# cbs228/sameold

Hardware: AMD Instinct MI355X
Metric: Msamples/s demodulated (batched 22.05 kHz channels) + % HBM roofline, 1/8 GPU (higher is better)
Workload: dtype f32

## Files before the change

sameold_amd/csrc/same_batch.cpp:

```cpp
#include <hip/hip_runtime.h>

#include <algorithm>
#include <chrono>
#include <cstdio>
#include <cstdlib>
#include <cstring>
#include <deque>
#include <new>
#include <string>
#include <type_traits>
#include <utility>
#include <vector>

#include "../../include/same_rx.h"
#include "same_config.h"
#include "same_device.h"
#include "same_harvest.h"
#include "same_hipmem.h"
#include "same_launch.h"
#include "same_resets.h"
#include "same_tp_plan.h"
#include "same_transport.h"

using same::fail;
static_assert(sizeof(same::cap::Span) == same::kSpanBytes, "same_tp_plan.h sizes the span list");

namespace {

#define HIP_TRY(expr)                                                                     \
    do {                                                                                   \
        hipError_t _e = (expr);                                                            \
        if (_e != hipSuccess)                                                              \
            return fail(SAME_EHIP, "%s failed: %s (%s:%d)", #expr, hipGetErrorString(_e),  \
                        __FILE__, __LINE__);                                               \
    } while (0)

}

struct same_batch {
    same_rx_builder builder{};
    same::Params P{};
    same::State S{};
    int device = 0;
    uint32_t flags = 0;
    uint64_t counter = 0;
    hipStream_t own_stream = nullptr;
    hipStream_t last_stream = nullptr;
    same::DevBuf<float4> d_taps;
    same::DevBuf<void> d_state_blob;
    struct Slot {
        same::DevBuf<same::DevEvent> d_events;
        uint32_t event_cap() const { return (uint32_t)d_events.size(); }
        same::DevBuf<uint32_t> d_sort;
        same::PinnedBuf<uint32_t> h_sort;
        same::DevBuf<same::DevEvent> d_sorted;
        uint32_t sort_bins = 0;
        same::DevBuf<uint8_t> d_bursts;
        uint32_t burst_cap() const { return (uint32_t)(d_bursts.size() / same::kBurstCap); }
        same::DevBuf<uint32_t> d_counters;
        same::MappedBuf<uint32_t> h_counters;
        same::Event ev_start, ev_stop, ev_done, ev_planned;
        same::Event ev_k0, ev_k1;
        bool have_k = false;
        bool timed = false;
        same::PinnedBuf<void> h_events, h_bursts;
        bool in_flight = false;
        uint64_t seq = 0;
        uint64_t end_counter = 0;
        bool chunked = false;
        same::ChunkGeom geom{};
        uint32_t columns(uint32_t n_channels) const { return chunked ? geom.n_chunks * n_channels : n_channels; }
        uint64_t end_blocks = 0;
        same::DevBuf<uint64_t> d_handover;
        same::PinnedBuf<uint64_t> h_handover;
        bool per_channel = false;
        same::TpGeomWords words;
        same::DevBuf<uint32_t> d_geom;
        same::PinnedBuf<uint32_t> h_geom;
        same::TpPlan plan{};
        uint64_t plan_counter0 = 0;
        bool plan_sorted = false, plan_lpt = false, plan_pairs = false;
        same::CoherentBuf<uint32_t> h_reset;
        same::CoherentBuf<uint32_t> h_counts;
        same::PinnedBuf<uint64_t> h_wake_up;
        bool dev_transport = false;
        same::CoherentBuf<same::DevMessage> h_near;
        uint32_t near_cap() const { return (uint32_t)h_near.size(); }
        same::DevBuf<same::DevMessage> d_msgs;
        uint32_t msg_cap() const { return (uint32_t)d_msgs.size(); }
        same::PinnedBuf<void> h_msgs;
        bool captured = false;
        same::DevBuf<same::cap::Span> d_spans;
        uint32_t span_cap() const { return (uint32_t)d_spans.size(); }
        same::DevBuf<float> d_pool;
        same::DevBuf<same::cap::Cursors> d_cap_cur;
        same::MappedBuf<same::cap::Cursors> h_cap_cur;
        same::PinnedBuf<void> h_spans, h_pool;
    } slot[2];
    struct TimePar {
        bool enabled = false;
        same::TpConfig cfg;
        uint32_t cap_columns = 0;
        uint32_t carved_columns = 0;
        int carved_family = -1;
        same::Params Pv{};
        same::State Sv{};
        same::DevBuf<void> blob;
        same::DevBuf<void> blob_fresh;
        size_t fresh_bytes = 0;
        same::DevBuf<same::StateArrayDesc> d_desc_in, d_desc_out;
        uint32_t n_desc = 0;
        same::DevBuf<uint32_t> d_final_col;
        same::DevBuf<float> d_energy;
        same::DevBuf<float> d_hist;
        same::Event ev_plan_prev; bool plan_recorded = false;
        uint32_t last_chunks = 1;
        bool last_per_channel = false;
        same::Family family = same::Family::kPipe;
    } tp;
    uint64_t launch_seq = 0;
    hipStream_t copy_stream = nullptr;
    struct Windowed {
        bool on = false;
        uint32_t window = 0;
        uint32_t fill = 0;
        same::DevBuf<void> d_buf;
        same::Event ev_buf;
        hipStream_t buf_stream = nullptr; bool buf_used = false;
        same::Event ev_read[2];
        uint64_t n_reads = 0;
        hipStream_t read_stream = nullptr;
    } inv;
    hipStream_t plan_stream = nullptr;
    float last_ms = 0.0f;
    bool overflowed = false;
    std::string record_path;
    bool kernel_fault = false;
    same::Request want;
    same::Mode mode;
    same::Choice plain;
    same::Params Pfm{};
    same::Family last_family = same::Family::kGeneric;
    bool sym_launched = false;
    bool debug = false;
    same::DevBuf<void> d_stage, d_stage2;
    same::DevBuf<void> d_upload;
    same::DevBuf<void> d_zero;
    same::Event ev_order;
    bool timing = false;
    bool have_timing = false;
    float last_demod_ms = 0.0f;
    same::PinnedBuf<uint64_t> h_wake;
    bool wake_ordered = false;
    std::vector<uint32_t> ragged_by;
    bool messages_only = false;
    bool dev_transport = false;
    bool last_dev_transport = false;
    same::DevBuf<void> d_thot, d_tcold;
    same::ResetLedger resets;
    std::vector<uint32_t> reset_list, reset_now, reset_cols;
    same::EventLog events;
    same::Replay replay{resets, events};
    struct Audio {
        size_t per_launch = 0;
        same::DevBuf<same::cap::Rec> d_rec;
        uint64_t flush_at = UINT64_MAX;
        same::AudioLog log;
    } audio;
};

namespace {

struct Carver {
    size_t off = 0;
    template <typename T> size_t take(size_t n)
    {
        off = (off + 255) & ~size_t(255);
        size_t o = off;
        off += n * sizeof(T);
        return o;
    }
};

#define SAME_STATE_ARRAYS(X, P)                                                                            \
    X(dc_ff_ring, float, (P).dc_len) X(dc_fb_ring, float, (P).dc_len)                                        \
    X(dc_sum0, float, 1) X(dc_sum1, float, 1) X(agc_gain, float, 1)                                          \
    X(win_ring, float, (P).win_ring)                                                                         \
    X(ted_clock, uint32_t, 1) X(until_next_ted, float, 1)                                                    \
    X(ted_h0, float, 1) X(ted_h1, float, 1) X(ted_h2, float, 1)                                              \
    X(period_avg, float, 1) X(period_inst, float, 1)                                                         \
    X(sq_data, uint32_t, 1) X(sq_power, float, 1) X(sq_phist, uint32_t, 1)                                   \
    X(sq_fill, uint32_t, 1) X(sq_clock, int32_t, 1) X(sq_symbols, uint64_t, 1)                               \
    X(sq_hist, float, same::kSquelchHist)                                                                    \
    X(eq_ffc, float, (P).eq_nff) X(eq_fbc, float, (P).eq_nfb)                                                \
    X(eq_ffw, float, (P).eq_nff) X(eq_fbw, float, (P).eq_nfb)                                                \
    X(eq_word, uint32_t, 1) X(eq_count, uint32_t, 1)                                                         \
    X(eq_snap_ffc, float, (P).eq_nff) X(eq_snap_fbc, float, (P).eq_nfb)                                      \
    X(eq_snap_ffw, float, (P).eq_nff) X(eq_snap_fbw, float, (P).eq_nfb)                                      \
    X(fr_word, uint32_t, 1) X(fr_count, uint32_t, 1) X(fr_invalid, uint32_t, 1) X(fr_len, uint32_t, 1)       \
    X(flags, uint32_t, 1)                                                                                    \
    X(tk_next, uint64_t, 1) X(tk_last, uint64_t, 1) X(tk_ring, uint64_t, same::kTickRing)                    \
    X(tk_n, uint32_t, 1) X(wake_sample, uint64_t, 1) X(wake_fired, uint64_t, 1)

size_t carve_state(const same::Params &P, char *base, same::State &S)
{
    const size_t C = P.n_channels;
    Carver cv;
#define CARVE(field, type, count) \
    do { size_t o = cv.take<type>(count); if (base) S.field = reinterpret_cast<type *>(base + o); } while (0)
#define CARVE_ROWS(field, type, rows) CARVE(field, type, (size_t)(rows) * C);
    SAME_STATE_ARRAYS(CARVE_ROWS, P)
#undef CARVE_ROWS
    CARVE(fr_msg, uint8_t, (size_t)same::kBurstCap * C);
    if (P.trace_cap) {
        CARVE(trace_n, uint32_t, C);
        CARVE(trace, float, (size_t)P.trace_cap * 4 * C);
        CARVE(trace_idx, uint64_t, (size_t)P.trace_cap * C);
    }
#undef CARVE
    return (cv.off + 255) & ~size_t(255);
}

void list_state_arrays(const same::Params &P, const same::State &src, const same::State &dst,
                       std::vector<same::StateArrayDesc> &out)
{
    out.clear();
#define DESC_ROWS(field, type, rows)                                                                     \
    out.push_back(same::StateArrayDesc{reinterpret_cast<char *>(src.field), reinterpret_cast<char *>(dst.field), \
                                       (uint32_t)(rows), (uint32_t)(sizeof(type) / 4)});
    SAME_STATE_ARRAYS(DESC_ROWS, P)
#undef DESC_ROWS
    static_assert(same::kBurstCap % 4 == 0, "framer rows are copied in words");
    out.push_back(same::StateArrayDesc{reinterpret_cast<char *>(src.fr_msg), reinterpret_cast<char *>(dst.fr_msg), 1u,
                                       (uint32_t)(same::kBurstCap / 4)});
}

void read_knobs(same_batch *rx)
{
    auto num = [](const char *name, int unset) { const char *e = std::getenv(name); return e ? std::atoi(e) : unset; };
    auto tri = [](const char *name) { const char *e = std::getenv(name); return e ? (std::atoi(e) ? 1 : -1) : 0; };
    rx->P.knob_pipe = tri("SAME_PIPE");
    rx->P.knob_pipe_lanes = num("SAME_PIPE_LANES", 0);
    rx->P.knob_pipe_split = tri("SAME_PIPE_SPLIT");
#ifdef SAME_PROFILE
    rx->P.knob_mirror = tri("SAME_MIRROR");
    rx->P.knob_pipe_share = tri("SAME_PIPE_SHARE");
    rx->P.knob_prio = num("SAME_PIPE_PRIO", 0);
#endif
    rx->P.knob_fast_dense = tri("SAME_FAST_DENSE");
    rx->P.knob_sym = tri("SAME_SYM");
    rx->want.sym_max_channels = (uint32_t)std::max(0, num("SAME_SYM_MAX", 1 << 30));
    rx->debug = rx->replay.debug = std::getenv("SAME_DEBUG") != nullptr;
    { const char *e = std::getenv("SAME_RECORD_HARVEST"); rx->record_path = e ? e : ""; }
    rx->replay.host_threads = std::max(0, num("SAME_HOST_THREADS", 0));
    rx->tp.cfg.sort_mode = num("SAME_TP_SORT", -1);
    rx->tp.cfg.knob_plan_stream = tri("SAME_TP_PLAN_STREAM");
    rx->tp.cfg.knob_prologue = tri("SAME_TP_PROLOGUE");
    rx->want.knob_relaxed = tri("SAME_RELAXED");
    { const char *e = std::getenv("SAME_RELAXED_KERNEL"); rx->P.knob_relaxed_kernel = !e ? 0 : (std::strcmp(e, "solo") == 0 ? 1 : (std::strcmp(e, "duo") == 0 ? 2 : 0)); }
    { const char *e = std::getenv("SAME_TP_KERNEL"); rx->want.knob_tp_kernel = !e ? 0 : (std::strcmp(e, "wave") == 0 ? 2 : (std::strcmp(e, "pipe") == 0 ? 1 : 0)); }
}

int ensure_output(same_batch *rx, same_batch::Slot &sl, size_t n_samples, same::Output &O, size_t n_columns = 0)
{
    const same::OutputCaps caps = same::output_caps(rx->P, n_samples, n_columns, rx->dev_transport, rx->audio.per_launch != 0, sl.near_cap(), sl.msg_cap());
    HIP_TRY(sl.d_events.ensure(caps.events));
    HIP_TRY(sl.d_bursts.ensure(caps.bursts * same::kBurstCap));
    if (caps.messages) HIP_TRY(sl.d_msgs.ensure(caps.messages));
    if (caps.near) HIP_TRY(sl.h_near.ensure(caps.near));
    if (caps.spans) HIP_TRY(sl.d_spans.ensure(caps.spans));
    HIP_TRY(sl.d_sorted.ensure(sl.d_events.size()));
    HIP_TRY(sl.d_sort.ensure(caps.sort_words));
    HIP_TRY(sl.h_sort.ensure(caps.bins + 1));
    sl.sort_bins = (uint32_t)caps.bins;
    O.events = sl.d_events; O.event_cap = sl.event_cap();
    O.bursts = sl.d_bursts; O.burst_cap = sl.burst_cap();
    O.n_events = sl.d_counters; O.n_bursts = sl.d_counters + 1; O.overflow = sl.d_counters + 2;
    return SAME_OK;
}

template <typename SampleT>
hipError_t launch_family(same::Family f, const same::Params &P, const same::State &S, const same::Output &O, const float4 *taps, const SampleT *x,
                         uint32_t n_blocks, uint64_t counter0, hipStream_t stream, const same::PipeChunks &pc = same::PipeChunks{})
{
    switch (f) {
    case same::Family::kSym: return same::launch_demod_sym(P, S, O, taps, x, n_blocks, counter0, stream, pc);
    case same::Family::kPipeFastmath: return same::launch_demod_pipe(P, S, O, taps, x, n_blocks, counter0, stream, pc, true);
    case same::Family::kPipe: return same::launch_demod_pipe(P, S, O, taps, x, n_blocks, counter0, stream, pc, false);
    case same::Family::kWaveRelaxed: return same::launch_demod_relaxed(P, S, O, taps, x, n_blocks, counter0, stream, pc);
    case same::Family::kFast: return same::launch_demod_fast(P, S, O, taps, x, n_blocks, counter0, stream);
    case same::Family::kGeneric: break;
    }
    return hipErrorInvalidValue;
}

void reset_channel_host(same_batch *rx, uint32_t c, uint64_t pos)
{
    rx->replay.reset_channel(c, pos);
    if (rx->h_wake) rx->h_wake[c] = 0;
}

int launch_pending_resets(same_batch *rx, same_batch::Slot &sl, hipStream_t stream)
{
    if (rx->resets.device.empty()) return SAME_OK;
    std::vector<uint32_t> &cols = rx->reset_cols;
    rx->resets.take_device(cols);
    const uint32_t n = (uint32_t)cols.size();
    if (n > sl.h_reset.size()) HIP_TRY(sl.h_reset.ensure(std::max<uint32_t>(256u, n + n / 2u)));
    std::memcpy(sl.h_reset, cols.data(), (size_t)n * sizeof(uint32_t));
    hipError_t e = same::launch_reset_columns(rx->P, rx->S, sl.h_reset.dev(), n, stream);
    if (e == hipSuccess && rx->dev_transport)
        e = same::launch_transport_reset(rx->d_thot, rx->d_tcold, rx->P.n_channels, sl.h_reset.dev(), n, 0, stream, rx->audio.d_rec);
    if (e != hipSuccess) return fail(SAME_EHIP, "channel reset launch failed: %s", hipGetErrorString(e));
    return SAME_OK;
}

int record_harvest(same_batch *rx, same_batch::Slot &sl, const same::HarvestInput &in, uint32_t n_events, uint32_t n_bursts, const char *path)
{
    if (sl.seq != 3u) return SAME_OK;
    const uint32_t n_ch = rx->P.n_channels, n_bins = sl.columns(n_ch);
    same::HarvestFileHeader h{};
    h.n_channels = n_ch; h.n_bins = n_bins; h.n_events = n_events; h.n_bursts = n_bursts;
    h.chunked = sl.chunked; h.per_channel = sl.per_channel; h.flags = rx->flags; h.input_rate = rx->P.input_rate; h.tp_enabled = rx->tp.enabled;
    h.geom = sl.geom; h.end_blocks = sl.end_blocks; h.end_counter = sl.end_counter;
    return same::write_harvest_file(path, h, in);
}

hipError_t grow_pinned(same::PinnedBuf<void> &b, size_t need)
{
    return need <= b.size() ? hipSuccess : b.ensure(need + need / 2 + 4096);
}

int harvest_audio(same_batch *rx, same_batch::Slot &sl)
{
    sl.captured = false;
    same_batch::Audio &A = rx->audio;
    const same::cap::Cursors cur = *sl.h_cap_cur.get();
    if (cur.overflow) rx->overflowed = true;
    const uint32_t n_spans = std::min(cur.n_spans, sl.span_cap());
    if (!n_spans) return SAME_OK;
    const size_t used = (size_t)std::min<unsigned long long>(cur.pool_used, (unsigned long long)A.per_launch);
    HIP_TRY(grow_pinned(sl.h_spans, (size_t)n_spans * sizeof(same::cap::Span)));
    HIP_TRY(hipMemcpyAsync(sl.h_spans, sl.d_spans, (size_t)n_spans * sizeof(same::cap::Span), hipMemcpyDeviceToHost, rx->copy_stream));
    if (used) {
        HIP_TRY(grow_pinned(sl.h_pool, used * sizeof(float)));
        HIP_TRY(hipMemcpyAsync(sl.h_pool, sl.d_pool, used * sizeof(float), hipMemcpyDeviceToHost, rx->copy_stream));
    }
    HIP_TRY(hipStreamSynchronize(rx->copy_stream));
    const same::cap::Span *sp = static_cast<const same::cap::Span *>(sl.h_spans.get());
    const float *pool = static_cast<const float *>(sl.h_pool.get());
    size_t n_samples = 0;
    if (const int arc = A.log.append_spans(sp, n_spans, pool, used, rx->resets, &n_samples)) return arc;
    if (rx->debug)
        std::fprintf(stderr, "[same] audio: %u chunks, %zu samples (pool %zu of %zu)%s\n", n_spans, n_samples, used, A.per_launch,
                     cur.overflow ? ", truncated" : "");
    return SAME_OK;
}

int harvest_messages(same_batch *rx, same_batch::Slot &sl, std::chrono::steady_clock::time_point t_begin,
                     std::chrono::steady_clock::time_point t_waited)
{
    const uint32_t n_msgs = std::min(sl.h_counters[3], sl.near_cap() + sl.msg_cap());
    const uint32_t n_near = std::min(n_msgs, sl.near_cap()), n_far = n_msgs - n_near;
    const size_t far_bytes = (size_t)n_far * sizeof(same::DevMessage);
    if (n_far) {
        HIP_TRY(grow_pinned(sl.h_msgs, far_bytes));
        HIP_TRY(hipMemcpyAsync(sl.h_msgs, sl.d_msgs, far_bytes, hipMemcpyDeviceToHost, rx->copy_stream));
        HIP_TRY(hipStreamSynchronize(rx->copy_stream));
    }
    auto t_copied = std::chrono::steady_clock::now();
    const same::DevMessage *far = static_cast<const same::DevMessage *>(sl.h_msgs.get());
    if (const int mrc = rx->replay.append_messages(sl.h_near.get(), n_near, far, n_far)) return mrc;
    if (sl.captured) {
        const int arc = harvest_audio(rx, sl);
        if (arc) return arc;
    }
    const int si = (int)(&sl - rx->slot);
    rx->resets.shift_due(si);
    rx->resets.done_shift(si);
    if (const int arc = rx->audio.log.end_reset(rx->resets.slot[si & 1].channels, rx->resets.rec_pos(si), rx->resets)) return arc;
    for (uint32_t c : rx->resets.host_due(si)) reset_channel_host(rx, c, rx->resets.rec_pos(si));
    rx->resets.done_host(si);
    if (rx->debug) {
        auto t_end = std::chrono::steady_clock::now();
        auto ms = [](auto a, auto b) { return std::chrono::duration<double, std::milli>(b - a).count(); };
        std::fprintf(stderr, "[same] harvest timing: wait %.2f ms, copy %.2f ms, %u messages queued in %.2f ms (transport layer on the device)\n",
                     ms(t_begin, t_waited), ms(t_waited, t_copied), n_msgs, ms(t_copied, t_end));
    }
    return SAME_OK;
}

int upload_wake_ordered(same_batch *rx, same_batch::Slot &sl)
{
    const uint32_t C = rx->P.n_channels;
    HIP_TRY(sl.h_wake_up.ensure(C));
    same_batch::Slot &other = rx->slot[(&sl - rx->slot) ^ 1];
    const int oi = (int)(&other - rx->slot);
    for (uint32_t c = 0; c < C; ++c) {
        const uint64_t w = rx->h_wake[c];
        sl.h_wake_up[c] = w && other.in_flight ? w + rx->resets.pending_shift(oi, c) : w;
    }
    if (other.in_flight) {
        HIP_TRY(hipMemcpyAsync(rx->S.wake_sample, sl.h_wake_up, (size_t)C * sizeof(uint64_t), hipMemcpyHostToDevice, rx->last_stream));
        HIP_TRY(hipEventRecord(other.ev_done, rx->last_stream));
    } else {
        HIP_TRY(hipMemcpyAsync(rx->S.wake_sample, sl.h_wake_up, (size_t)C * sizeof(uint64_t), hipMemcpyHostToDevice, rx->copy_stream));
        HIP_TRY(hipStreamSynchronize(rx->copy_stream));
    }
    return SAME_OK;
}

int harvest_slot(same_batch *rx, same_batch::Slot &sl)
{
    if (!sl.in_flight) return SAME_OK;
    const bool dbg = rx->debug;
    auto t_begin = std::chrono::steady_clock::now();
    HIP_TRY(hipEventSynchronize(sl.ev_done));
    sl.in_flight = false;
    if (sl.timed) {
        HIP_TRY(hipEventElapsedTime(&rx->last_ms, sl.ev_start, sl.ev_stop));
        rx->last_demod_ms = rx->last_ms;
        if (sl.have_k) HIP_TRY(hipEventElapsedTime(&rx->last_demod_ms, sl.ev_k0, sl.ev_k1));
        rx->have_timing = true;
    }
    auto t_waited = std::chrono::steady_clock::now();
    const uint32_t n_events = std::min(sl.h_counters[0], sl.event_cap());
    if (dbg)
        std::fprintf(stderr, "[same] harvest: %u device events (%u bursts), cap %u/%u\n", sl.h_counters[0],
                     sl.h_counters[1], sl.event_cap(), sl.burst_cap());
    const uint32_t n_bursts = std::min(sl.h_counters[1], sl.burst_cap());
    if (sl.h_counters[2] & (3u | same::kMessageLogOverflow)) rx->overflowed = true;
    if (sl.h_counters[2] & 4u) rx->kernel_fault = true;
    if (sl.dev_transport) return harvest_messages(rx, sl, t_begin, t_waited);
    const size_t ev_bytes = (size_t)n_events * sizeof(same::DevEvent), bu_bytes = (size_t)n_bursts * same::kBurstCap;
    HIP_TRY(grow_pinned(sl.h_events, ev_bytes));
    HIP_TRY(grow_pinned(sl.h_bursts, bu_bytes));
    const uint32_t n_bins = sl.columns(rx->P.n_channels);
    if (n_bins != sl.sort_bins) return fail(SAME_EINVAL, "internal: event sort made for %u columns, launch has %u", sl.sort_bins, n_bins);
    HIP_TRY(hipMemcpyAsync(sl.h_sort, sl.d_sort + n_bins, ((size_t)n_bins + 1) * sizeof(uint32_t), hipMemcpyDeviceToHost, rx->copy_stream));
    if (n_events) HIP_TRY(hipMemcpyAsync(sl.h_events, sl.d_sorted, ev_bytes, hipMemcpyDeviceToHost, rx->copy_stream));
    HIP_TRY(hipStreamSynchronize(rx->copy_stream));
    if (n_bursts) HIP_TRY(hipMemcpyAsync(sl.h_bursts, sl.d_bursts, bu_bytes, hipMemcpyDeviceToHost, rx->copy_stream));
    if (sl.chunked) {
        HIP_TRY(hipMemcpyAsync(sl.h_handover, sl.d_handover, (size_t)n_bins * sizeof(uint64_t), hipMemcpyDeviceToHost, rx->copy_stream));
        if (sl.per_channel)
            HIP_TRY(hipMemcpyAsync(sl.h_geom, sl.d_geom + sl.words.own_start, sl.words.harvest * sizeof(uint32_t), hipMemcpyDeviceToHost, rx->copy_stream));
    }
    if (n_bursts || sl.chunked) HIP_TRY(hipStreamSynchronize(rx->copy_stream));
    auto t_copied = std::chrono::steady_clock::now();
    const same::HarvestInput in{sl.h_sort, static_cast<same::DevEvent *>(sl.h_events.get()), static_cast<const uint8_t *>(sl.h_bursts.get()),
                                sl.h_handover, sl.h_geom};
    if (!rx->record_path.empty()) { const int rrc = record_harvest(rx, sl, in, n_events, n_bursts, rx->record_path.c_str()); if (rrc != SAME_OK) return rrc; }
    std::vector<uint32_t> rearm;
    same::HarvestTimes times;
    same::HarvestLaunch launch;
    launch.chunked = sl.chunked; launch.per_channel = sl.per_channel; launch.geom = sl.geom;
    launch.end_blocks = sl.end_blocks; launch.end_counter = sl.end_counter;
    int rc = rx->replay.replay(launch, in, n_events, n_bursts, rearm, times);
    if (rc) return rc;
    {
        const int si = (int)(&sl - rx->slot);
        const same::ResetLedger::SlotShift &sh = rx->resets.shift_due(si);
        if (!rx->replay.thot.empty())
            for (size_t i = 0; i < sh.channels.size(); ++i)
                if (rx->replay.tr(sh.channels[i]).shift_force_eom(sh.by[i])) rearm.push_back(sh.channels[i]);
        rx->resets.done_shift(si);
    }
    {
        const int si = (int)(&sl - rx->slot);
        const std::vector<uint32_t> &due = rx->resets.host_due(si);
        for (uint32_t c : due) reset_channel_host(rx, c, rx->resets.rec_pos(si));
        rx->resets.done_host(si);
    }
    if (!rearm.empty()) {
        if (!rx->h_wake) {
            HIP_TRY(rx->h_wake.ensure(rx->P.n_channels));
            std::memset(rx->h_wake, 0, (size_t)rx->P.n_channels * sizeof(uint64_t));
        }
        for (uint32_t c : rearm) rx->h_wake[c] = rx->replay.tr(c).force_eom_at();
        if (rx->wake_ordered) {
            int rc2 = upload_wake_ordered(rx, sl);
            if (rc2) return rc2;
        } else {
        HIP_TRY(hipMemcpyAsync(rx->S.wake_sample, rx->h_wake, (size_t)rx->P.n_channels * sizeof(uint64_t), hipMemcpyHostToDevice, rx->copy_stream));
        HIP_TRY(hipStreamSynchronize(rx->copy_stream));
        }
    }
    if (dbg) {
        auto t_end = std::chrono::steady_clock::now();
        auto ms = [](auto a, auto b) { return std::chrono::duration<double, std::milli>(b - a).count(); };
        std::fprintf(stderr, "[same] harvest timing: wait %.2f ms, copy %.2f ms, sort %.2f ms, replay on %u threads %.2f ms, "
                             "queue %.2f ms\n",
                     ms(t_begin, t_waited), ms(t_waited, t_copied), ms(t_copied, times.sorted), times.n_threads,
                     ms(times.sorted, times.replayed), ms(times.replayed, t_end));
    }
    return SAME_OK;
}

int harvest(same_batch *rx)
{
    same_batch::Slot *order[2] = {&rx->slot[0], &rx->slot[1]};
    if (order[0]->seq > order[1]->seq) std::swap(order[0], order[1]);
    for (same_batch::Slot *sl : order) {
        int rc = harvest_slot(rx, *sl);
        if (rc) return rc;
    }
    return SAME_OK;
}

int ensure_wide_state(same_batch *rx, uint32_t columns)
{
    same_batch::TimePar &tp = rx->tp;
    if (tp.carved_columns == columns && tp.carved_family == (int)tp.family) return SAME_OK;
    int rc = harvest(rx);
    if (rc) return rc;
    HIP_TRY(hipDeviceSynchronize());
    tp.Pv = same::wide_params(rx->P, columns, same::is_fastmath(tp.family), same::tp_more_than_one_round(columns));
    if (columns > tp.cap_columns) {
        tp.cap_columns = 0;
        HIP_TRY(tp.blob.reset());
        HIP_TRY(tp.blob_fresh.reset());
        const size_t bytes = carve_state(tp.Pv, nullptr, tp.Sv);
        HIP_TRY(tp.blob.ensure(bytes));
        HIP_TRY(hipMemset(tp.blob, 0, bytes));
        HIP_TRY(tp.blob_fresh.ensure(bytes));
        tp.cap_columns = columns;
    }
    const size_t blob_bytes = carve_state(tp.Pv, (char *)tp.blob.get(), tp.Sv);
    {
        same::State Sf{};
        carve_state(tp.Pv, (char *)tp.blob_fresh.get(), Sf);
        HIP_TRY(hipMemset(tp.blob_fresh, 0, blob_bytes));
        HIP_TRY(same::launch_init_state(tp.Pv, Sf, 0, nullptr, 0));
        HIP_TRY(hipDeviceSynchronize());
        tp.fresh_bytes = (size_t)(reinterpret_cast<char *>(tp.Sv.fr_msg) - static_cast<char *>(tp.blob.get()));
    }
    std::vector<same::StateArrayDesc> in, out;
    list_state_arrays(rx->P, rx->S, tp.Sv, in);
    list_state_arrays(rx->P, tp.Sv, rx->S, out);
    tp.n_desc = (uint32_t)in.size();
    HIP_TRY(tp.d_desc_in.ensure(in.size()));
    HIP_TRY(tp.d_desc_out.ensure(out.size()));
    HIP_TRY(tp.d_final_col.ensure(rx->P.n_channels));
    HIP_TRY(hipMemcpy(tp.d_desc_in, in.data(), in.size() * sizeof(same::StateArrayDesc), hipMemcpyHostToDevice));
    HIP_TRY(hipMemcpy(tp.d_desc_out, out.data(), out.size() * sizeof(same::StateArrayDesc), hipMemcpyHostToDevice));
    tp.carved_columns = columns;
    tp.carved_family = (int)tp.family;
    return SAME_OK;
}

struct Ragged {
    const uint32_t *counts = nullptr;
    uint32_t m = 0;
    uint32_t row_off = 0;
};

struct RaggedLaunch {
    uint32_t row0 = 0;
    size_t n_lock = 0;
};


int begin_launch(same_batch *rx, same_batch::Slot &sl, const same_batch::Slot &prev, hipStream_t stream)
{
    int rc = harvest_slot(rx, sl);
    if (rc) return rc;
    if (prev.in_flight && rx->last_stream != stream) HIP_TRY(hipStreamWaitEvent(stream, prev.ev_done, 0));
    return launch_pending_resets(rx, sl, stream);
}

int begin_timing(same_batch *rx, same_batch::Slot &sl, hipStream_t stream)
{
    sl.timed = rx->timing;
    if (sl.timed) HIP_TRY(hipEventRecord(sl.ev_start, stream));
    return SAME_OK;
}

int tp_start(same_batch *rx, same_batch::Slot &sl, uint32_t columns, const char *layout, hipStream_t stream, bool *sort_bins_empty)
{
    same_batch::TimePar &tp = rx->tp;
    const uint32_t C = rx->P.n_channels;
    *sort_bins_empty = false;
    if (tp.cfg.knob_prologue >= 0) {
        HIP_TRY(same::launch_tp_prologue(tp.blob, tp.blob_fresh, tp.fresh_bytes, sl.d_handover, sl.d_sort, columns, sl.d_counters, stream));
        *sort_bins_empty = sl.sort_bins == columns;
    } else {
        HIP_TRY(same::launch_counters(sl.d_counters, sl.h_counters.dev(), 0, stream));
        HIP_TRY(same::launch_init_state(tp.Pv, tp.Sv, 0, stream, C));
        HIP_TRY(same::launch_fill_u64(sl.d_handover, columns, same::kNoHandover, stream));
    }
    if (rx->debug) std::fprintf(stderr, "[same] time-parallel launch: %u columns (%s), start-up: %s\n", columns, layout,
                                tp.cfg.knob_prologue >= 0 ? "prologue kernel" : "separate launches");
    HIP_TRY(same::launch_copy_state_columns(tp.d_desc_in, tp.n_desc, C, columns, nullptr, C, stream));
    return SAME_OK;
}

template <typename SampleT>
int demod_tail(same_batch *rx, const same::Output &O, const SampleT *rows, size_t n, uint64_t counter0, hipStream_t stream)
{
    const hipError_t e = same::launch_demod(rx->P, rx->S, O, rx->d_taps, rows, (uint32_t)n, counter0, stream);
    if (e != hipSuccess) return fail(SAME_EHIP, "demod kernel launch failed: %s", hipGetErrorString(e));
    return SAME_OK;
}
int demod_tail_corner(same_batch *rx, const same::Output &O, const float *corner, size_t pitch, size_t r, uint64_t counter0, hipStream_t stream)
{
    const uint32_t C = rx->P.n_channels;
    HIP_TRY(rx->d_stage.ensure(r * C * sizeof(float)));
    HIP_TRY(rx->d_stage2.ensure(r * C * sizeof(float)));
    float *staged = static_cast<float *>(rx->d_stage.get()), *rows = static_cast<float *>(rx->d_stage2.get());
    HIP_TRY(hipMemcpy2DAsync(staged, r * sizeof(float), corner, pitch * sizeof(float), r * sizeof(float), C, hipMemcpyDeviceToDevice, stream));
    const hipError_t e = same::launch_transpose(staged, rows, C, (uint32_t)r, stream);
    if (e != hipSuccess) return fail(SAME_EHIP, "demod kernel launch failed: %s", hipGetErrorString(e));
    return demod_tail(rx, O, rows, r, counter0, stream);
}

int tp_plan_boundaries(same_batch *rx, same_batch::Slot &sl, const same::TpCut &cut, const same::TpNative &np, const float *d_x,
                       hipStream_t stream, same::PipeChunks &pc)
{
    same_batch::TimePar &tp = rx->tp;
    const same::TpGeomWords &w = np.words;
    same::TpPlan plan{};
    plan.channels = rx->P.n_channels; plan.n_chunks = cut.n_chunks; plan.block_len = cut.geom.block_len;
    plan.warmup_samples = np.warmup_samples; plan.whole_samples = np.whole_samples; plan.in_samples = np.in_samples;
    plan.scout_blocks = np.scout_blocks;
    sl.plan = plan; sl.plan_counter0 = rx->counter;
    sl.plan_sorted = np.sort_mode != 0; sl.plan_lpt = np.lpt; sl.plan_pairs = np.pair_groups;
    uint32_t *g = sl.d_geom;
    const bool side = same::tp_plan_beside(tp.cfg, stream == rx->own_stream);
    hipStream_t ps = side ? rx->plan_stream : stream;
    if (tp.plan_recorded) HIP_TRY(hipStreamWaitEvent(ps, tp.ev_plan_prev, 0));
    HIP_TRY(same::launch_tp_plan(d_x, plan, tp.d_energy, g + w.own_start, g + w.row0, g + w.nominal, g + w.perm, g + w.wg, np.sort_mode != 0, ps,
                                 np.lpt ? g + w.perm2 : nullptr, np.lpt ? g + w.wg2 : nullptr, np.pair_groups));
    HIP_TRY(tp.ev_plan_prev.ensure());
    HIP_TRY(hipEventRecord(tp.ev_plan_prev, ps));
    tp.plan_recorded = true;
    if (side) {
        HIP_TRY(hipEventRecord(sl.ev_planned, ps));
        HIP_TRY(hipStreamWaitEvent(stream, sl.ev_planned, 0));
    }
    pc.col_row0 = g + w.row0; pc.col_nominal = g + w.nominal;
    pc.wg_blocks = g + (np.lpt ? w.wg2 : w.wg); pc.col_perm = np.lpt ? g + w.perm2 : nullptr;
    pc.in_samples = np.in_samples; pc.whole_samples = np.whole_samples;
    pc.hist_scratch = np.need_hist ? tp.d_hist.get() : nullptr;
    return SAME_OK;
}

template <typename SampleT>
int launch_time_parallel(same_batch *rx, same_batch::Slot &sl, hipStream_t stream, const same::TpCut &cut, const same::TpNative *np,
                         const SampleT *x, size_t n_call, bool *sort_bins_empty)
{
    same_batch::TimePar &tp = rx->tp;
    const same::ChunkGeom &geom = cut.geom;
    const uint32_t C = rx->P.n_channels, columns = cut.n_chunks * C, fb = geom.block_len;
    const uint32_t total_blocks = (uint32_t)(n_call / fb);
    const size_t n_whole = (size_t)total_blocks * fb;
    tp.family = cut.choice.family;
    same::Output O{};
    int rc = ensure_wide_state(rx, columns);
    if (rc == SAME_OK) rc = ensure_output(rx, sl, same::tp_output_samples(np ? n_whole : n_call, cut.pc, fb), O, columns);
    if (rc) return rc;
    HIP_TRY(sl.d_handover.ensure(columns));
    HIP_TRY(sl.h_handover.ensure(columns));
    same::PipeChunks pc = cut.pc;
    pc.handover = sl.d_handover;
    if (np) {
        HIP_TRY(sl.d_geom.ensure(np->words.total));
        HIP_TRY(sl.h_geom.ensure(np->words.harvest));
        HIP_TRY(tp.d_energy.ensure(np->energy_floats));
        if (np->need_hist) HIP_TRY(tp.d_hist.ensure(np->hist_floats));
        sl.words = np->words;
    }
    rc = begin_timing(rx, sl, stream);
    if (rc) return rc;
    const float *xf = nullptr;
    if constexpr (std::is_same_v<SampleT, float>) xf = x;
    if (np && (rc = tp_plan_boundaries(rx, sl, cut, *np, xf, stream, pc)) != SAME_OK) return rc;
    rc = tp_start(rx, sl, columns, np ? "channel-major" : "time-major", stream, sort_bins_empty);
    if (rc) return rc;
    sl.have_k = np && sl.timed;
    if (sl.have_k) HIP_TRY(hipEventRecord(sl.ev_k0, stream));
    const hipError_t e = launch_family(tp.family, tp.Pv, tp.Sv, O, rx->d_taps, x, total_blocks, rx->counter, stream, pc);
    rx->last_family = tp.family;
    if (e != hipSuccess) return fail(SAME_EHIP, "time-parallel demod kernel launch failed: %s", hipGetErrorString(e));
    if (sl.have_k) HIP_TRY(hipEventRecord(sl.ev_k1, stream));
    if (np) HIP_TRY(same::launch_chunk_final_column_pc(sl.d_handover, sl.d_geom + np->words.own_start, C, geom.n_chunks, rx->counter, tp.d_final_col, stream));
    else HIP_TRY(same::launch_chunk_final_column(sl.d_handover, C, geom, tp.d_final_col, stream));
    HIP_TRY(same::launch_copy_state_columns(tp.d_desc_out, tp.n_desc, columns, C, tp.d_final_col, C, stream));
    if (n_whole < n_call) {
        rc = np ? demod_tail_corner(rx, O, xf + n_whole, n_call, n_call - n_whole, rx->counter + n_whole, stream)
                : demod_tail(rx, O, x + n_whole * C, n_call - n_whole, rx->counter + n_whole, stream);
        if (rc) return rc;
    }
    sl.chunked = true; sl.per_channel = np != nullptr;
    sl.geom = geom;
    sl.end_blocks = rx->counter + n_whole;
    tp.last_chunks = cut.n_chunks; tp.last_per_channel = sl.per_channel;
    return SAME_OK;
}

template <typename SampleT>
int end_launch(same_batch *rx, same_batch::Slot &sl, same_batch::Slot &prev, hipStream_t stream, const SampleT *rows, size_t n,
               bool sort_bins_empty, const RaggedLaunch *rl = nullptr)
{
    if (sl.timed) HIP_TRY(hipEventRecord(sl.ev_stop, stream));
    HIP_TRY(same::launch_event_sort(sl.d_events, sl.d_counters, sl.event_cap(), sl.sort_bins, sl.d_sort, sl.d_sort + sl.sort_bins,
                                    sl.d_sorted, stream, sort_bins_empty));
    sl.dev_transport = rx->dev_transport && !sl.chunked;
    rx->last_dev_transport = sl.dev_transport;
    if (sl.dev_transport) {
        same::TransportLaunch T{};
        T.n_channels = rx->P.n_channels; T.input_rate = rx->P.input_rate;
        T.first = sl.d_sort + sl.sort_bins; T.sorted = sl.d_sorted; T.counters = sl.d_counters;
        T.bursts = sl.d_bursts; T.burst_cap = sl.burst_cap();
        T.hot = rx->d_thot; T.cold = rx->d_tcold; T.wake_sample = rx->S.wake_sample;
        T.near = sl.h_near.dev(); T.near_cap = sl.near_cap();
        T.log = sl.d_msgs; T.log_cap = sl.msg_cap(); T.log_cursor = sl.d_counters + 3; T.overflow = sl.d_counters + 2;
        sl.captured = rx->audio.per_launch != 0;
        if (sl.captured) {
            same::cap::Launch &K = T.cap;
            const uint64_t fa = rx->audio.flush_at;
            K.start = rx->counter; K.n_rows = (uint32_t)n;
            K.flush_row = fa >= rx->counter + n ? same::cap::kNoFlush : (uint32_t)(fa > rx->counter ? fa - rx->counter : 0);
            K.rec = rx->audio.d_rec; K.spans = sl.d_spans; K.span_cap = sl.span_cap();
            K.n_spans = &sl.d_cap_cur->n_spans; K.pool_used = &sl.d_cap_cur->pool_used; K.pool_cap = rx->audio.per_launch;
            K.overflow = &sl.d_cap_cur->overflow;
        }
        if (rl && rl->n_lock < n)
            HIP_TRY(same::launch_transport_ragged(T, sl.h_counts.dev(), rl->row0, (uint32_t)n, stream));
        else
            HIP_TRY(same::launch_transport(T, stream));
        if (sl.captured) {
            const hipError_t e = same::launch_capture(sl.d_spans, sl.d_cap_cur, sl.span_cap(), sl.d_pool, rx->audio.per_launch, rows,
                                                      rx->P.n_channels, (uint32_t)n, sl.h_cap_cur.dev(), stream);
            if (e != hipSuccess) return fail(SAME_EHIP, "capture kernel launch failed: %s", hipGetErrorString(e));
        }
    }
    HIP_TRY(same::launch_counters(sl.d_counters, sl.h_counters.dev(), 1, stream));
    HIP_TRY(hipEventRecord(sl.ev_done, stream));
    sl.in_flight = true;
    sl.seq = ++rx->launch_seq;
    rx->last_stream = stream;
    if (rl) rx->resets.shift(rx->ragged_by.data(), rx->counter + n, (int)(&sl - rx->slot));
    rx->counter += n;
    sl.end_counter = rx->counter;
    return harvest_slot(rx, prev);
}

template <typename SampleT>
int process_time_major_launches(same_batch *rx, const SampleT *d_x, size_t n_samples, hipStream_t stream, const Ragged *rg = nullptr)
{
    const size_t kMaxChunk = same::max_launch_samples(rx->P.input_rate);
    size_t done = 0;
    while (done < n_samples) {
        const size_t n = std::min(kMaxChunk, n_samples - done);
        same_batch::Slot &sl = rx->slot[rx->launch_seq & 1];
        same_batch::Slot &prev = rx->slot[(rx->launch_seq & 1) ^ 1];
        int rc = begin_launch(rx, sl, prev, stream);
        if (rc) return rc;
        size_t n_lock = n;
        if (rg) {
            const size_t row0 = (size_t)rg->row_off + done;
            const uint32_t C = rx->P.n_channels;
            HIP_TRY(sl.h_counts.ensure(C));
            std::memcpy(sl.h_counts, rg->counts, (size_t)C * sizeof(uint32_t));
            rx->ragged_by.resize(C);
            n_lock = same::ragged_launch_split(rg->counts, C, rg->m, row0, n, rx->ragged_by.data());
        }
        const same::TpCut cut = rg ? same::TpCut{} : same::tp_uniform_cut(rx->P, rx->mode, rx->want, rx->tp.cfg, n, rx->counter);
        rx->tp.last_chunks = cut.n_chunks;
        sl.have_k = false;
        bool sort_bins_empty = false;
        if (cut.n_chunks > 1u) {
            rc = launch_time_parallel(rx, sl, stream, cut, nullptr, d_x + done * rx->P.n_channels, n, &sort_bins_empty);
            if (rc) return rc;
        } else {
        same::Output O{};
        sl.chunked = false; sl.per_channel = false;
        rc = ensure_output(rx, sl, n, O);
        if (rc) return rc;
        HIP_TRY(same::launch_counters(sl.d_counters, sl.h_counters.dev(), 0, stream));
        rc = begin_timing(rx, sl, stream);
        if (rc) return rc;
        const SampleT *xp = d_x + done * rx->P.n_channels;
        hipError_t e = hipSuccess;
        const same::Choice &plain = rx->plain;
        const size_t fb = plain.block_len;
        const size_t n_fast = fb ? (n_lock / fb) * fb : 0;
        if (n_fast) {
            e = launch_family(plain.family, same::is_fastmath(plain.family) ? rx->Pfm : rx->P, rx->S, O, rx->d_taps, xp, (uint32_t)(n_fast / fb), rx->counter, stream);
            if (e != hipSuccess) return fail(SAME_EHIP, "%s launch failed: %s", same::family_name(plain.family, rx->P.block_len), hipGetErrorString(e));
            rx->sym_launched |= plain.family == same::Family::kSym;
        }
        rx->last_family = plain.family == same::Family::kSym && !rx->sym_launched ? same::Family::kPipeFastmath : plain.family;
        if (n_fast < n_lock &&
            (rc = demod_tail(rx, O, xp + n_fast * rx->P.n_channels, n_lock - n_fast, rx->counter + n_fast, stream)) != SAME_OK) return rc;
        if (n_lock < n) {
            e = same::launch_demod_ragged(rx->P, rx->S, O, rx->d_taps, xp + n_lock * rx->P.n_channels, (uint32_t)(n - n_lock), sl.h_counts.dev(),
                                          (uint32_t)(rg->row_off + done + n_lock), rx->counter + n_lock, stream);
            if (e != hipSuccess) return fail(SAME_EHIP, "ragged demod kernel launch failed: %s", hipGetErrorString(e));
        }
        }
        const RaggedLaunch rl{rg ? (uint32_t)(rg->row_off + done) : 0u, n_lock};
        rc = end_launch(rx, sl, prev, stream, d_x + done * rx->P.n_channels, n, sort_bins_empty, rg ? &rl : nullptr);
        if (rc) return rc;
        done += n;
    }
    return SAME_OK;
}

constexpr uint32_t kInvWindow = 18432;
constexpr uint32_t kInvWindowTimeParallel = 73728;
static int inv_buffer_wait(same_batch *rx, hipStream_t stream)
{
    same_batch::Windowed &iv = rx->inv;
    if (iv.buf_used && iv.buf_stream != stream) HIP_TRY(hipStreamWaitEvent(stream, iv.ev_buf, 0));
    return SAME_OK;
}
static int inv_buffer_done(same_batch *rx, hipStream_t stream)
{
    same_batch::Windowed &iv = rx->inv;
    HIP_TRY(iv.ev_buf.ensure());
    HIP_TRY(hipEventRecord(iv.ev_buf, stream));
    iv.buf_stream = stream; iv.buf_used = true;
    return SAME_OK;
}
static int inv_copy(const float *d_x, float *dst, size_t n, hipStream_t stream)
{
    HIP_TRY(hipMemcpyAsync(dst, d_x, n * sizeof(float), hipMemcpyDeviceToDevice, stream));
    return SAME_OK;
}
static int inv_copy(const int16_t *d_x, float *dst, size_t n, hipStream_t stream)
{
    const hipError_t e = same::launch_cast_i16_f32(d_x, dst, n, stream);
    if (e != hipSuccess) return fail(SAME_EHIP, "cast launch failed: %s", hipGetErrorString(e));
    return SAME_OK;
}
template <typename SampleT>
static int inv_append(same_batch *rx, const SampleT *d_x, size_t n, hipStream_t stream)
{
    same_batch::Windowed &iv = rx->inv;
    const size_t C = rx->P.n_channels;
    HIP_TRY(iv.d_buf.ensure((size_t)iv.window * C * sizeof(float)));
    int rc = inv_buffer_wait(rx, stream);
    if (rc) return rc;
    rc = inv_copy(d_x, static_cast<float *>(iv.d_buf.get()) + (size_t)iv.fill * C, n * C, stream);
    if (rc) return rc;
    iv.fill += (uint32_t)n;
    return inv_buffer_done(rx, stream);
}
static int inv_launch_waiting(same_batch *rx, hipStream_t stream)
{
    same_batch::Windowed &iv = rx->inv;
    if (!iv.fill) return SAME_OK;
    int rc = inv_buffer_wait(rx, stream);
    if (rc) return rc;
    const uint32_t n = iv.fill;
    iv.fill = 0;
// ... 145 lines not shown
template <typename SampleT>
int process_host_any(same_batch *rx, const SampleT *h_x, size_t n_samples, uint32_t layout)
{
    if (!rx || (!h_x && n_samples)) return fail(SAME_EINVAL, "null argument");
    if (n_samples == 0) return SAME_OK;
    HIP_TRY(hipSetDevice(rx->device));
    return upload_in_slabs(rx, h_x, n_samples, n_samples, layout, [&](const SampleT *d_in, size_t n, size_t) {
        return process_device_any(rx, d_in, n, layout, SAME_STREAM_OWN);
    });
}

int ragged_check(same_batch *rx, size_t n_rows, const uint32_t *counts, uint32_t layout, uint32_t *m_out, uint32_t *M_out)
{
    if (!rx) return fail(SAME_EINVAL, "null handle");
    if (!counts) return fail(SAME_EINVAL, "null counts");
    if (layout != SAME_LAYOUT_TIME_MAJOR && layout != SAME_LAYOUT_CHANNEL_MAJOR) return fail(SAME_EINVAL, "unknown layout %u", layout);
    if (rx->tp.enabled) return fail(SAME_EINVAL, "ragged calls: a SAME_BATCH_TIME_PARALLEL batch plans its cuts over one common row range");
    if (rx->inv.on) return fail(SAME_EINVAL, "ragged calls: SAME_BATCH_CALL_INVARIANT windows begin at positions of one common stream");
    if (rx->P.trace_cap) return fail(SAME_EINVAL, "ragged calls: SAME_BATCH_TRACE_SYMBOLS records batch sample positions");
    if (n_rows > 0xffffffffull) return fail(SAME_EINVAL, "ragged calls: n_rows beyond 2^32 - 1");
    uint32_t m = UINT32_MAX, M = 0;
    for (uint32_t c = 0; c < rx->P.n_channels; ++c) {
        if (counts[c] > n_rows) return fail(SAME_EINVAL, "counts[%u] = %u exceeds n_rows = %zu; nothing was consumed", c, counts[c], n_rows);
        m = std::min(m, counts[c]); M = std::max(M, counts[c]);
    }
    *m_out = m; *M_out = M;
    return SAME_OK;
}

template <typename SampleT>
int process_ragged_on(same_batch *rx, const SampleT *d_x, size_t pitch, size_t n_buf, size_t row_base, const uint32_t *counts,
                      uint32_t m, uint32_t M, uint32_t layout, hipStream_t stream)
{
    const size_t n_p = std::min<size_t>(M, row_base + n_buf) - row_base;
    Ragged rg; rg.counts = counts; rg.m = m;
    if (layout == SAME_LAYOUT_TIME_MAJOR) {
        if (m == M) return process_time_major_launches(rx, d_x, n_p, stream);
        rg.row_off = (uint32_t)row_base;
        return process_time_major_launches(rx, d_x, n_p, stream, &rg);
    }
    return transpose_in_slabs(rx, d_x, pitch, n_p, stream, [&](const SampleT *rows, size_t n, size_t t0) {
        if (m == M) return process_time_major_launches(rx, rows, n, stream);
        rg.row_off = (uint32_t)(row_base + t0);
        return process_time_major_launches(rx, rows, n, stream, &rg);
    });
}

template <typename SampleT>
int process_ragged_device(same_batch *rx, const SampleT *d_x, size_t n_rows, const uint32_t *counts, uint32_t layout, void *hip_stream)
{
    uint32_t m = 0, M = 0;
    int rc = ragged_check(rx, n_rows, counts, layout, &m, &M);
    if (rc) return rc;
    if (M == 0) return SAME_OK;
    if (!d_x) return fail(SAME_EINVAL, "null argument");
    if (m == M && M == n_rows) return process_device_any(rx, d_x, n_rows, layout, hip_stream);
    HIP_TRY(hipSetDevice(rx->device));
    hipStream_t stream = hip_stream == SAME_STREAM_OWN ? rx->own_stream : (hipStream_t)hip_stream;
    if (m != M) rx->wake_ordered = true;
    return process_ragged_on(rx, d_x, n_rows, n_rows, 0, counts, m, M, layout, stream);
}

template <typename SampleT>
int process_ragged_host(same_batch *rx, const SampleT *h_x, size_t n_rows, const uint32_t *counts, uint32_t layout)
{
    uint32_t m = 0, M = 0;
    int rc = ragged_check(rx, n_rows, counts, layout, &m, &M);
    if (rc) return rc;
    if (M == 0) return SAME_OK;
    if (!h_x) return fail(SAME_EINVAL, "null argument");
    if (m == M && M == n_rows) return process_host_any(rx, h_x, n_rows, layout);
    HIP_TRY(hipSetDevice(rx->device));
    if (m != M) rx->wake_ordered = true;
    rc = harvest(rx);
    if (rc) return rc;
    return upload_in_slabs(rx, h_x, n_rows, M, layout, [&](const SampleT *d_in, size_t n, size_t t0) {
        return process_ragged_on(rx, d_in, n, n, t0, counts, m, M, layout, rx->own_stream);
    });
}

}

extern "C" {

const char *same_last_error(void) { return same::last_error(); }

#ifndef SAME_SOURCE_HASH
#define SAME_SOURCE_HASH "unknown"
#endif
const char *same_rx_source_hash(void) { return "SAME_SOURCE_HASH=" SAME_SOURCE_HASH; }

int same_batch_new(const same_rx_builder *b, uint32_t n_channels, int device, uint32_t flags,
                   same_batch **out)
{
    if (!b || !out || n_channels == 0) return fail(SAME_EINVAL, "null builder/out or zero channels");
    *out = nullptr;
    int ndev = 0;
    if (hipGetDeviceCount(&ndev) != hipSuccess || ndev <= 0)
        return fail(SAME_ENODEVICE, "no HIP device visible (this library has no CPU path)");
    if (device < 0 || device >= ndev) return fail(SAME_ENODEVICE, "device %d out of range (%d visible)", device, ndev);
    same_batch *rx = new (std::nothrow) same_batch;
    if (!rx) return fail(SAME_ENOMEM, "out of memory");
    rx->builder = *b;
    rx->device = device;
    rx->flags = flags;
    rx->inv.on = (flags & SAME_BATCH_CALL_INVARIANT) != 0;
    rx->inv.window = (flags & SAME_BATCH_TIME_PARALLEL) ? kInvWindowTimeParallel : kInvWindow;
    if (const char *e = std::getenv("SAME_INV_WINDOW")) { const long v = std::atol(e); if (v >= 64 && v <= (1 << 22)) rx->inv.window = (uint32_t)v; }
    std::vector<float> taps;
    int rc = same::derive_params(*b, n_channels, rx->P, taps);
    if (rc) { delete rx; return fail(rc, "builder rejected (code %d)", rc); }
    read_knobs(rx);
    rx->P.trace_cap = (flags & SAME_BATCH_TRACE_SYMBOLS) ? 4096u : 0u;
    if ((flags & SAME_BATCH_TIME_PARALLEL) && (flags & SAME_BATCH_TRACE_SYMBOLS)) {
        delete rx;
        return fail(SAME_EINVAL, "SAME_BATCH_TIME_PARALLEL cannot record a symbol trace");
    }
    if ((flags & SAME_BATCH_MESSAGES_ONLY) && (flags & SAME_BATCH_LINK_ONLY)) {
        delete rx;
        return fail(SAME_EINVAL, "SAME_BATCH_MESSAGES_ONLY needs the transport layer that SAME_BATCH_LINK_ONLY skips");
    }
    rx->tp.enabled = (flags & SAME_BATCH_TIME_PARALLEL) != 0;
    rx->messages_only = (flags & SAME_BATCH_MESSAGES_ONLY) != 0;
    rx->dev_transport = rx->messages_only && !rx->tp.enabled;
    rx->P.ticks = ((flags & SAME_BATCH_LINK_ONLY) || rx->tp.enabled) ? 0u : 1u;
    rx->P.tick_interburst = (uint32_t)same::max_interburst_symbols();
    rx->P.tick_history = (uint32_t)same::max_history_duration();

    auto cleanup = [&](int code) { same_batch_free(rx); return code; };
#define TRY_OR_CLEAN(expr)                                                                     \
    do {                                                                                       \
        hipError_t _e = (expr);                                                                \
        if (_e != hipSuccess)                                                                  \
            return cleanup(fail(SAME_EHIP, "%s failed: %s", #expr, hipGetErrorString(_e)));    \
    } while (0)
    TRY_OR_CLEAN(hipSetDevice(device));
    hipDeviceProp_t prop;
    TRY_OR_CLEAN(hipGetDeviceProperties(&prop, device));
    if (std::strncmp(prop.gcnArchName, "gfx950", 6) != 0)
        return cleanup(fail(SAME_ENODEVICE, "device %d is %s; this build carries gfx950 code only", device, prop.gcnArchName));
    rx->want.relaxed = (flags & SAME_BATCH_RELAXED) != 0;
    rx->want.time_parallel = rx->tp.enabled;
    rx->want.generic = (flags & SAME_BATCH_GENERIC_KERNEL) != 0;
    rx->mode = same::select_mode(rx->P, rx->want);
    rx->plain = same::select_plain(rx->P, rx->mode, rx->want);
    rx->Pfm = same::fm_params(rx->P);
    rx->last_family = same::strict_family(rx->P, rx->mode);
    if (same::demod_lds_bytes(rx->P) > 160 * 1024)
        return cleanup(fail(SAME_EINVAL, "configuration needs %zu bytes of LDS per wavefront (limit 160 KiB)", same::demod_lds_bytes(rx->P)));
    TRY_OR_CLEAN(hipStreamCreateWithFlags(&rx->own_stream, hipStreamNonBlocking));
    TRY_OR_CLEAN(hipStreamCreateWithFlags(&rx->copy_stream, hipStreamNonBlocking));
    TRY_OR_CLEAN(hipStreamCreateWithFlags(&rx->plan_stream, hipStreamNonBlocking));
    TRY_OR_CLEAN(rx->ev_order.ensure());
    for (auto &sl : rx->slot) {
        TRY_OR_CLEAN(sl.ev_start.ensure(hipEventDefault));
        TRY_OR_CLEAN(sl.ev_stop.ensure(hipEventDefault));
        TRY_OR_CLEAN(sl.ev_k0.ensure(hipEventDefault));
        TRY_OR_CLEAN(sl.ev_k1.ensure(hipEventDefault));
        TRY_OR_CLEAN(sl.ev_done.ensure());
        TRY_OR_CLEAN(sl.ev_planned.ensure());
        TRY_OR_CLEAN(sl.d_counters.ensure(4));
        TRY_OR_CLEAN(sl.h_counters.ensure(4));
    }
    static_assert(sizeof(float4) == 4 * sizeof(float), "the taps are uploaded in fours");
    TRY_OR_CLEAN(rx->d_taps.ensure(taps.size() / 4));
    TRY_OR_CLEAN(hipMemcpy(rx->d_taps, taps.data(), taps.size() * sizeof(float), hipMemcpyHostToDevice));
    const size_t state_bytes = carve_state(rx->P, nullptr, rx->S);
    TRY_OR_CLEAN(rx->d_state_blob.ensure(state_bytes));
    TRY_OR_CLEAN(hipMemset(rx->d_state_blob, 0, state_bytes));
    carve_state(rx->P, (char *)rx->d_state_blob.get(), rx->S);
    TRY_OR_CLEAN(same::launch_init_state(rx->P, rx->S, 0, rx->own_stream));
    if (rx->dev_transport) {
        TRY_OR_CLEAN(rx->d_thot.ensure((size_t)n_channels * same::transport_hot_bytes()));
        TRY_OR_CLEAN(rx->d_tcold.ensure((size_t)n_channels * same::transport_cold_bytes()));
        TRY_OR_CLEAN(hipMemsetAsync(rx->d_tcold, 0, (size_t)n_channels * same::transport_cold_bytes(), rx->own_stream));
        TRY_OR_CLEAN(same::launch_transport_reset(rx->d_thot, rx->d_tcold, n_channels, nullptr, 0, 1, rx->own_stream));
    }
    TRY_OR_CLEAN(hipStreamSynchronize(rx->own_stream));
#undef TRY_OR_CLEAN
    rx->replay.link_only = (flags & SAME_BATCH_LINK_ONLY) != 0;
    rx->replay.messages_only = rx->messages_only;
    rx->replay.time_parallel = rx->tp.enabled;
    rx->replay.init(n_channels, rx->P.input_rate, !(flags & SAME_BATCH_LINK_ONLY) && !rx->dev_transport);
    rx->resets.init(n_channels);
    *out = rx;
    return SAME_OK;
}

void same_batch_free(same_batch *rx)
{
    if (!rx) return;
    (void)hipSetDevice(rx->device);
    if (rx->last_stream) (void)hipStreamSynchronize(rx->last_stream);
    const hipStream_t streams[3] = {rx->copy_stream, rx->plan_stream, rx->own_stream};
    delete rx;
    for (hipStream_t st : streams)
        if (st) (void)hipStreamDestroy(st);
}

int same_batch_reset(same_batch *rx)
{
    if (!rx) return fail(SAME_EINVAL, "null handle");
    HIP_TRY(hipSetDevice(rx->device));
    int rc = harvest(rx);
    if (rc) return rc;
    hipError_t e = same::launch_init_state(rx->P, rx->S, 1, rx->own_stream);
    if (e == hipSuccess && rx->dev_transport)
        e = same::launch_transport_reset(rx->d_thot, rx->d_tcold, rx->P.n_channels, nullptr, 0, 0, rx->own_stream, rx->audio.d_rec);
    if (e != hipSuccess) return fail(SAME_EHIP, "reset launch failed: %s", hipGetErrorString(e));
    HIP_TRY(hipStreamSynchronize(rx->own_stream));
    rx->counter = 0;
    rx->inv.fill = 0;
    rx->events.clear();
    rx->replay.reset();
    if (rx->h_wake) std::memset(rx->h_wake, 0, (size_t)rx->P.n_channels * sizeof(uint64_t));
    rx->resets.clear();
    rx->overflowed = false;
    rx->kernel_fault = false;
    rx->audio.log.clear();
    rx->audio.flush_at = UINT64_MAX;
    return SAME_OK;
}

int same_batch_reset_channels(same_batch *rx, const uint32_t *channels, size_t n)
{
    if (!rx) return fail(SAME_EINVAL, "null handle");
    if (n && !channels) return fail(SAME_EINVAL, "null channel list");
    if (!same::ResetLedger::normalise(channels, n, rx->P.n_channels, rx->reset_list))
        return fail(SAME_EINVAL, "a channel of the list is out of range (the batch has %u); nothing was reset", rx->P.n_channels);
    if (rx->reset_list.empty()) return SAME_OK;
    HIP_TRY(hipSetDevice(rx->device));
    if (rx->inv.on && rx->inv.fill) {
        const int rc = inv_launch_waiting(rx, rx->own_stream);
        if (rc) return rc;
    }
    int newest = -1;
    for (int s = 0; s < 2; ++s)
        if (rx->slot[s].in_flight && (newest < 0 || rx->slot[s].seq > rx->slot[newest].seq)) newest = s;
    if (newest < 0) {
        const int arc = rx->audio.log.end_reset(rx->reset_list, rx->counter, rx->resets);
        if (arc) return arc;
    }
    rx->resets.request(rx->reset_list, rx->counter, newest, rx->reset_now);
    for (uint32_t c : rx->reset_now) reset_channel_host(rx, c, rx->counter);
    return SAME_OK;
}

uint64_t same_batch_channel_input_sample_counter(const same_batch *rx, uint32_t channel)
{
    if (!rx || channel >= rx->P.n_channels) return 0;
    return rx->counter + rx->inv.fill - rx->resets.api_base[channel];
}

uint32_t same_batch_input_rate(const same_batch *rx) { return rx ? rx->P.input_rate : 0; }
uint32_t same_batch_n_channels(const same_batch *rx) { return rx ? rx->P.n_channels : 0; }
uint64_t same_batch_input_sample_counter(const same_batch *rx) { return rx ? rx->counter + rx->inv.fill : 0; }
int same_batch_device(const same_batch *rx) { return rx ? rx->device : -1; }

int same_batch_process_device(same_batch *rx, const float *d_x, size_t n_samples, uint32_t layout, void *hip_stream)
{ return process_device_any<float>(rx, d_x, n_samples, layout, hip_stream); }
int same_batch_process_device_i16(same_batch *rx, const int16_t *d_x, size_t n_samples, uint32_t layout, void *hip_stream)
{ return process_device_any<int16_t>(rx, d_x, n_samples, layout, hip_stream); }
int same_batch_process_host(same_batch *rx, const float *h_x, size_t n_samples, uint32_t layout)
{ return process_host_any<float>(rx, h_x, n_samples, layout); }
int same_batch_process_host_i16(same_batch *rx, const int16_t *h_x, size_t n_samples, uint32_t layout)
{ return process_host_any<int16_t>(rx, h_x, n_samples, layout); }

int same_batch_process_device_ragged(same_batch *rx, const float *d_x, size_t n_rows, const uint32_t *counts, uint32_t layout, void *hip_stream)
{ return process_ragged_device<float>(rx, d_x, n_rows, counts, layout, hip_stream); }
int same_batch_process_device_ragged_i16(same_batch *rx, const int16_t *d_x, size_t n_rows, const uint32_t *counts, uint32_t layout,
                                         void *hip_stream)
{ return process_ragged_device<int16_t>(rx, d_x, n_rows, counts, layout, hip_stream); }
int same_batch_process_host_ragged(same_batch *rx, const float *h_x, size_t n_rows, const uint32_t *counts, uint32_t layout)
{ return process_ragged_host<float>(rx, h_x, n_rows, counts, layout); }
int same_batch_process_host_ragged_i16(same_batch *rx, const int16_t *h_x, size_t n_rows, const uint32_t *counts, uint32_t layout)
{ return process_ragged_host<int16_t>(rx, h_x, n_rows, counts, layout); }

int same_batch_flush(same_batch *rx)
{
    if (!rx) return fail(SAME_EINVAL, "null handle");
    HIP_TRY(hipSetDevice(rx->device));
    const size_t n = (size_t)rx->P.input_rate * 4;
    const size_t slab = std::max<size_t>(1, std::min<size_t>(n, ((size_t)256 << 20) / ((size_t)rx->P.n_channels * sizeof(float))));
    if (slab * rx->P.n_channels * sizeof(float) > rx->d_zero.size()) {
        HIP_TRY(rx->d_zero.ensure(slab * rx->P.n_channels * sizeof(float)));
        HIP_TRY(hipMemset(rx->d_zero, 0, rx->d_zero.size()));
    }
    int rc = SAME_OK;
    rx->audio.flush_at = rx->counter + rx->inv.fill;
    for (size_t t0 = 0; t0 < n && rc == SAME_OK; t0 += slab) {
        rc = process_device_any<float>(rx, static_cast<const float *>(rx->d_zero.get()), std::min(slab, n - t0), SAME_LAYOUT_TIME_MAJOR, SAME_STREAM_OWN);
        if (rc == SAME_OK) rc = harvest(rx);
    }
    if (rc == SAME_OK && rx->inv.on) {
        rc = inv_launch_waiting(rx, rx->own_stream);
        if (rc == SAME_OK) rc = harvest(rx);
    }
    rx->audio.flush_at = UINT64_MAX;
    return rc;
}

int same_batch_set_call_window(same_batch *rx, uint32_t samples)
{
    if (!rx) return fail(SAME_EINVAL, "null handle");
    if (!rx->inv.on) return fail(SAME_EINVAL, "the batch was not made with SAME_BATCH_CALL_INVARIANT");
    if (samples < 64u || samples > (1u << 22)) return fail(SAME_EINVAL, "window of %u samples (64 .. 4 194 304)", samples);
    if (rx->counter || rx->inv.fill) return fail(SAME_EINVAL, "the window is set before the first sample (or right behind a reset)");
    rx->inv.window = samples;
    return SAME_OK;
}

int same_batch_order_after(same_batch *rx, void *producer_stream)
{
    if (!rx) return fail(SAME_EINVAL, "null handle");
    if (producer_stream == SAME_STREAM_OWN) return SAME_OK;
    HIP_TRY(hipSetDevice(rx->device));
    HIP_TRY(hipEventRecord(rx->ev_order, (hipStream_t)producer_stream));
    HIP_TRY(hipStreamWaitEvent(rx->own_stream, rx->ev_order, 0));
    HIP_TRY(hipStreamWaitEvent(rx->plan_stream, rx->ev_order, 0));
    return SAME_OK;
}

int same_batch_sync(same_batch *rx)
{
    if (!rx) return fail(SAME_EINVAL, "null handle");
    HIP_TRY(hipSetDevice(rx->device));
    int rc = harvest(rx);
    if (rc == SAME_OK && rx->inv.on) rc = inv_reads_wait(rx);
    if (rc) return rc;
    if (rx->kernel_fault) return fail(SAME_EKERNEL, "a demodulation kernel's wavefronts lost step (internal hand-over timed out)");
    if (rx->overflowed) return fail(SAME_EOVERFLOW, "event/burst pool overflow");
    return SAME_OK;
}

size_t same_batch_pending_events(same_batch *rx)
{
    if (!rx) return 0;
    return rx->events.pending();
}

int same_batch_poll_events(same_batch *rx, same_rx_event *out, size_t cap, size_t *n_out, size_t *n_left)
{
    if (!rx || (!out && cap)) return fail(SAME_EINVAL, "null argument");
    return rx->events.poll(rx->replay.workers, out, cap, n_out, n_left);
}

int same_batch_peek_events(same_batch *rx, const same_rx_event **events, size_t *n)
{
    if (!rx || !events || !n) return fail(SAME_EINVAL, "null argument");
    return rx->events.peek(rx->replay.workers, events, n);
}

int same_batch_drop_events(same_batch *rx, size_t n)
{
    if (!rx) return fail(SAME_EINVAL, "null argument");
    return rx->events.drop(n);
}

int same_batch_set_audio_capture(same_batch *rx, size_t samples_per_launch)
{
    if (!rx) return fail(SAME_EINVAL, "null handle");
    if (!rx->messages_only) return fail(SAME_EINVAL, "audio capture needs SAME_BATCH_MESSAGES_ONLY (the transport layer on the device)");
    if (rx->tp.enabled) return fail(SAME_EINVAL, "audio capture is not available in SAME_BATCH_TIME_PARALLEL batches");
    if (rx->counter || rx->inv.fill) return fail(SAME_EINVAL, "audio capture is set before the first sample (or right behind a reset)");
    HIP_TRY(hipSetDevice(rx->device));
    int rc = harvest(rx);
    if (rc) return rc;
    same_batch::Audio &A = rx->audio;
    auto release = [&]() {
        for (same_batch::Slot &sl : rx->slot) { (void)sl.d_pool.reset(); (void)sl.d_spans.reset(); }
        (void)A.d_rec.reset();
        A.per_launch = 0;
        A.log.open.clear();
    };
    release();
    if (!samples_per_launch) return SAME_OK;
    if (samples_per_launch > ((size_t)1 << 40)) return fail(SAME_EINVAL, "%zu samples per launch", samples_per_launch);
    auto oom = [&](const char *what) {
        (void)hipGetLastError();
        release();
        return fail(SAME_ENOMEM, "audio capture: %s (%zu samples per launch)", what, samples_per_launch);
    };
    for (same_batch::Slot &sl : rx->slot) {
        if (sl.d_pool.ensure(samples_per_launch) != hipSuccess) return oom("sample pool");
        if (!sl.d_cap_cur) {
            if (sl.d_cap_cur.ensure(1) != hipSuccess) return oom("cursors");
            HIP_TRY(hipMemset(sl.d_cap_cur, 0, sizeof(same::cap::Cursors)));
            if (sl.h_cap_cur.ensure(1) != hipSuccess) return oom("cursors");
        }
    }
    if (A.d_rec.ensure(rx->P.n_channels) != hipSuccess) return oom("capture records");
    HIP_TRY(hipMemset(A.d_rec, 0, (size_t)rx->P.n_channels * sizeof(same::cap::Rec)));
    A.log.open.assign(rx->P.n_channels, 0);
    A.per_launch = samples_per_launch;
    return SAME_OK;
}

int same_batch_peek_audio(same_batch *rx, const same_audio_chunk **chunks, size_t *n)
{
    if (!rx || !chunks || !n) return fail(SAME_EINVAL, "null argument");
    return rx->audio.log.peek(chunks, n);
}

int same_batch_drop_audio(same_batch *rx, size_t n)
{
    if (!rx) return fail(SAME_EINVAL, "null argument");
    return rx->audio.log.drop(n);
}

int same_batch_pack_bursts(same_batch *rx, uint32_t first_channel, uint8_t *out, size_t cap, size_t *n_records)
{
    if (!rx || !n_records) return fail(SAME_EINVAL, "null argument");
    return rx->events.pack_bursts(rx->replay.workers, first_channel, out, cap, n_records);
}

int same_batch_read_trace(same_batch *rx, uint32_t channel, same_symbol_trace *out, size_t cap, size_t *n_out)
{
    if (!rx || !n_out) return fail(SAME_EINVAL, "null argument");
    if (!rx->P.trace_cap) return fail(SAME_EINVAL, "batch was not created with SAME_BATCH_TRACE_SYMBOLS");
    if (channel >= rx->P.n_channels) return fail(SAME_EINVAL, "channel out of range");
    HIP_TRY(hipSetDevice(rx->device));
    int rc = harvest(rx);
    if (rc) return rc;
    uint32_t n = 0;
    HIP_TRY(hipMemcpy(&n, rx->S.trace_n + channel, sizeof(n), hipMemcpyDeviceToHost));
    n = std::min(n, rx->P.trace_cap);
    n = (uint32_t)std::min<size_t>(n, cap);
    std::vector<float> f((size_t)n * 4);
    std::vector<uint64_t> idx(n);
    if (n) {
        HIP_TRY(hipMemcpy(f.data(), rx->S.trace + (size_t)channel * rx->P.trace_cap * 4, f.size() * sizeof(float), hipMemcpyDeviceToHost));
        HIP_TRY(hipMemcpy(idx.data(), rx->S.trace_idx + (size_t)channel * rx->P.trace_cap, n * sizeof(uint64_t), hipMemcpyDeviceToHost));
    }
    for (uint32_t i = 0; i < n; ++i) {
        out[i].sample_counter = idx[i];
        out[i].zero = f[4 * i]; out[i].sym = f[4 * i + 1]; out[i].err = f[4 * i + 2];
        out[i].samples_until_next_ted = f[4 * i + 3];
    }
    *n_out = n;
    return SAME_OK;
}

void same_batch_set_kernel_timing(same_batch *rx, int enable) { if (rx) { rx->timing = enable != 0; rx->have_timing = false; } }
int same_batch_last_kernel_ms(same_batch *rx, float *ms)
{
    if (!rx || !ms) return fail(SAME_EINVAL, "null argument");
    if (!rx->have_timing) return fail(SAME_EINVAL, "no timed launch yet");
    *ms = rx->last_ms;
    return SAME_OK;
}
int same_batch_last_demod_kernel_ms(same_batch *rx, float *ms)
{
    if (!rx || !ms) return fail(SAME_EINVAL, "null argument");
    if (!rx->have_timing) return fail(SAME_EINVAL, "no timed launch yet");
    *ms = rx->last_demod_ms;
    return SAME_OK;
}
int same_batch_time_parallel_config(same_batch *rx, uint32_t max_chunks, uint32_t min_own_samples, uint32_t warmup_samples)
{
    if (!rx) return fail(SAME_EINVAL, "null handle");
    if (!rx->tp.enabled) return fail(SAME_EINVAL, "batch was not created with SAME_BATCH_TIME_PARALLEL");
    rx->tp.cfg.max_chunks = max_chunks; rx->tp.cfg.min_own = min_own_samples; rx->tp.cfg.warmup = warmup_samples;
    return SAME_OK;
}
uint32_t same_batch_time_parallel_chunks(const same_batch *rx) { return rx ? rx->tp.last_chunks : 0; }
int same_batch_transport_on_device(const same_batch *rx) { return rx && rx->last_dev_transport ? 1 : 0; }
int same_batch_time_parallel_per_channel(const same_batch *rx) { return rx && rx->tp.last_chunks > 1u && rx->tp.last_per_channel ? 1 : 0; }

int same_batch_debug_tp_plan(same_batch *rx, same_tp_plan_info *info, float *energy, size_t energy_cap, uint32_t *geom,
                             size_t geom_cap, uint64_t *handover, size_t handover_cap, uint32_t *final_col, size_t final_col_cap)
{
    if (!rx || !info) return fail(SAME_EINVAL, "null argument");
// ... 172 lines not shown
```

sameold_amd/csrc/same_device.h:

```cpp
#pragma once

#include <stddef.h>
#include <stdint.h>

namespace same {

constexpr int kWave = 64;
constexpr int kMaxEqTaps = 16;
constexpr int kBurstCap = 288;
constexpr int kSquelchHist = 64;
constexpr int kMaxTaps = 512;

struct Params {
    uint32_t n_channels;
    uint32_t input_rate;
    uint32_t dc_len;
    float dc_inv_len;
    float dc_k;
    float agc_bw, agc_min, agc_max, agc_gain0;
    uint32_t ntaps;
    uint32_t win_ring;
    float samples_per_ted, period_min, period_max;
    float alpha_unlocked, beta_unlocked, alpha_locked, beta_locked;
    uint32_t sync_word, sq_max_errors;
    float sq_power_open, sq_power_close, sq_bw;
    uint32_t eq_nff, eq_nfb;
    float eq_relaxation, eq_regularization;
    uint32_t fr_max_prefix_errors, fr_max_invalid;
    uint32_t block_len;
    uint32_t trace_cap;
    uint32_t ticks;
    uint32_t tick_interburst;
    uint32_t tick_history;
    int32_t knob_pipe;
    int32_t knob_pipe_lanes;
    int32_t knob_pipe_split;
    int32_t knob_mirror;
    int32_t knob_fast_dense;
    int32_t knob_pipe_share;
    int32_t knob_relaxed_kernel;
    int32_t knob_sym;
    int32_t knob_prio;
};

enum : uint32_t {
    F_AGC_LOCKED = 1u << 0,
    F_TED_PHASE = 1u << 1,
    F_BW_LOCKED = 1u << 2,
    F_SQ_LOCK = 1u << 3,
    F_EQ_MODE_SHIFT = 4,
    F_EQ_MODE_MASK = 3u << 4,
    F_FR_STATE_SHIFT = 6,
    F_FR_STATE_MASK = 3u << 6,
    F_LINK_SHIFT = 8,
    F_LINK_MASK = 3u << 8,
    F_TICK_AGAIN = 1u << 10,
    F_EQ_BITS_SHIFT = 16,
    F_EQ_BITS_MASK = 0xffu << 16,
};
constexpr int kTickRing = 8;

struct State {
    float *dc_ff_ring;
    float *dc_fb_ring;
    float *dc_sum0, *dc_sum1;
    float *agc_gain;
    float *win_ring;
    uint32_t *ted_clock;
    float *until_next_ted;
    float *ted_h0, *ted_h1, *ted_h2;
    float *period_avg, *period_inst;
    uint32_t *sq_data;
    float *sq_power;
    uint32_t *sq_phist;
    uint32_t *sq_fill;
    int32_t *sq_clock;
    uint64_t *sq_symbols;
    float *sq_hist;
    float *eq_ffc, *eq_fbc;
    float *eq_ffw, *eq_fbw;
    uint32_t *eq_word, *eq_count;
    float *eq_snap_ffc, *eq_snap_fbc, *eq_snap_ffw, *eq_snap_fbw;
    uint32_t *fr_word, *fr_count, *fr_invalid, *fr_len;
    uint8_t *fr_msg;
    uint32_t *flags;
    uint64_t *tk_next;
    uint64_t *tk_last;
    uint64_t *tk_ring;
    uint32_t *tk_n;
    uint64_t *wake_sample;
    uint64_t *wake_fired;
    uint32_t *trace_n;
    float *trace;
    uint64_t *trace_idx;
};

struct PipeChunks {
    uint32_t n_chunks;
    uint32_t in_channels;
    uint32_t stride_blocks;
    uint32_t nominal_blocks;
    uint64_t *handover;
    const uint32_t *col_row0;
    const uint32_t *col_nominal;
    const uint32_t *wg_blocks;
    const uint32_t *col_perm;
    float *hist_scratch;
    uint64_t in_samples;
    uint32_t whole_samples;
};

struct ChunkGeom {
    uint64_t counter0;
    uint32_t n_chunks, block_len, stride_blocks, warmup_blocks;
#if defined(__HIPCC__)
    __host__ __device__
#endif
    uint32_t owner_of(uint64_t h) const
    {
        const uint64_t blocks = (h - counter0) / block_len;
        if (blocks < warmup_blocks) return 0u;
        const uint64_t k = (blocks - warmup_blocks) / stride_blocks;
        return k >= n_chunks ? n_chunks - 1u : (uint32_t)k;
    }
#if defined(__HIPCC__)
    __host__ __device__
#endif
    uint64_t own_start(uint32_t k) const
    { return k == 0u ? counter0 : counter0 + ((uint64_t)k * stride_blocks + warmup_blocks) * block_len; }
};
constexpr uint64_t kNoHandover = ~0ull;

struct StateArrayDesc { char *src; char *dst; uint32_t rows; uint32_t elem_words; };

constexpr uint32_t kDevEventNone = 0xffffffffu;
struct DevEvent {
    uint32_t channel;
    uint32_t kind;
    uint64_t sample_counter;
    uint64_t symbol_count;
    uint32_t burst_len;
    uint32_t burst_slot;
};

constexpr uint32_t kDevMessageText = 272;
struct DevMessage {
    uint32_t channel;
    uint32_t kind;
    uint64_t sample_counter;
    uint64_t symbol_count;
    uint32_t len, aux, aux2;
    uint32_t seq;
    uint8_t text[kDevMessageText];
};

struct Output {
    DevEvent *events;
    uint32_t *n_events;
    uint32_t event_cap;
    uint8_t *bursts;
    uint32_t *n_bursts;
    uint32_t burst_cap;
    uint32_t *overflow;
};

}
```

sameold_amd/csrc/same_kernels.hip:

```cpp
#include <hip/hip_runtime.h>

#include <algorithm>

#include "same_dev_common.h"
#include "same_device.h"
#include "same_launch.h"
#include "same_tp_plan.h"

namespace same {

template <int B, typename SampleT>
__global__ __launch_bounds__(kWave) void demod_kernel(Params P, State S, Output O,
                                                      const float4 *__restrict__ taps,
                                                      const SampleT *__restrict__ x,
                                                      uint32_t n_samples, uint64_t counter0)
{
    extern __shared__ float lds[];
    const uint32_t lane = threadIdx.x;
    const uint32_t C = P.n_channels;
    const uint32_t c_raw = blockIdx.x * kWave + lane;
    if (c_raw >= C) return;
    const uint32_t c = c_raw;
    const uint32_t DL = P.dc_len;
    float *ff = lds;
// ... 553 lines not shown
        return n;
    };
    const bool forced = plan(NB - 1, false, false) > K;
    int lo = (NB + K - 1) / K, hi = NB;
    while (lo < hi) {
        const int step = (hi - lo + (int)kWave - 1) / (int)kWave;
        const int cand = lo + step * (int)lane;
        const bool ok = cand >= hi || plan(cand, false, forced) <= K;
        const unsigned long long okm = __builtin_amdgcn_ballot_w64(ok);
        if (okm == 0ull) { lo += step * ((int)kWave - 1) + 1; continue; }
        const int first = __builtin_ctzll(okm);
        hi = min(lo + step * first, hi);
        if (first > 0) lo += step * (first - 1) + 1;
    }
    int used = 0;
    if (lane == 0) used = plan(lo, true, forced);
    used = __shfl(used, 0);
    __syncthreads();
    auto own = [&](int k) __attribute__((always_inline)) -> uint32_t {
        const int i = k < used ? k : used - 1;
        uint32_t p = (k >= 1 && i >= 1) ? (uint32_t)cut[i] * kScoutBlock : 0u;
        return p - p % kB;
    };
    for (int k = (int)lane; k < K; k += (int)kWave) {
        const uint32_t p = own(k);
        const uint32_t r = (k == 0 || p < g.warmup_samples) ? 0u : p - g.warmup_samples;
        const size_t v = (size_t)k * g.channels + c;
        own_start[v] = p;
        row0[v] = r;
        nominal[v] = k + 1 < K ? (own(k + 1) - r + kB - 1u) / kB : 0xffffffffu;
    }
}
constexpr uint32_t kSortBuckets = 4096, kSortBucketBlocks = 4;
__device__ __forceinline__ void tp_sort_key(const TpPlan &g, const uint32_t *row0, const uint32_t *nominal, uint32_t v,
                                            uint32_t *group, uint32_t *bucket)
{
    const uint32_t chunk = v / g.channels;
    const uint32_t avail = (g.whole_samples - row0[v]) / g.block_len;
    *group = chunk + 1u == g.n_chunks ? 0u : (chunk == 0u ? 1u : 2u);
    const uint32_t len = *group == 0u ? avail : min(nominal[v], avail);
    *bucket = kSortBuckets - 1u - min(len / kSortBucketBlocks, kSortBuckets - 1u);
}
constexpr uint32_t kSortThreads = 1024;
__global__ __launch_bounds__(kSortThreads) void tp_sort_kernel(TpPlan g, const uint32_t *__restrict__ row0, const uint32_t *__restrict__ nominal,
                                                                uint32_t *__restrict__ perm)
{
    __shared__ uint32_t hist[3u * kSortBuckets];
    __shared__ uint32_t wave_sum[kSortThreads / kWave];
    const uint32_t tid = threadIdx.x, lane = tid & (kWave - 1u), wave = tid / kWave, n = g.n_chunks * g.channels;
    for (uint32_t i = tid; i < 3u * kSortBuckets; i += kSortThreads) hist[i] = 0u;
    __syncthreads();
    for (uint32_t v = tid; v < n; v += kSortThreads) {
        uint32_t grp, b;
        tp_sort_key(g, row0, nominal, v, &grp, &b);
        if (grp != 0u) atomicAdd(&hist[grp * kSortBuckets + b], 1u);
    }
    __syncthreads();
    constexpr uint32_t PER = kSortBuckets / kSortThreads;
    static_assert(PER * kSortThreads == kSortBuckets, "buckets per thread");
    const uint32_t base[3] = {0u, g.channels, 2u * g.channels};
    for (uint32_t grp = 0; grp < 3u; ++grp) {
        uint32_t *h = hist + grp * kSortBuckets + tid * PER;
        uint32_t mine = 0;
        for (uint32_t i = 0; i < PER; ++i) mine += h[i];
        uint32_t incl = mine;
        for (int off = 1; off < (int)kWave; off <<= 1) { const uint32_t t = (uint32_t)__shfl_up((int)incl, off); if ((int)lane >= off) incl += t; }
        if (lane == kWave - 1u) wave_sum[wave] = incl;
        __syncthreads();
        uint32_t before = base[grp] + incl - mine;
        for (uint32_t w = 0; w < wave; ++w) before += wave_sum[w];
        for (uint32_t i = 0; i < PER; ++i) { const uint32_t c = h[i]; h[i] = before; before += c; }
        __syncthreads();
    }
    for (uint32_t v = tid; v < n; v += kSortThreads) {
        uint32_t grp, b;
        tp_sort_key(g, row0, nominal, v, &grp, &b);
        if (grp == 0u) perm[v - (g.n_chunks - 1u) * g.channels] = v;
        else perm[atomicAdd(&hist[grp * kSortBuckets + b], 1u)] = v;
    }
}
__global__ void tp_iota_kernel(uint32_t *perm, uint32_t n)
{
    const uint32_t i = blockIdx.x * blockDim.x + threadIdx.x;
    if (i < n) perm[i] = i;
}
__global__ void tp_align_kernel(TpPlan g, const uint32_t *__restrict__ perm, uint32_t *__restrict__ row0, const uint32_t *__restrict__ nominal,
                                uint32_t *__restrict__ wg_blocks, uint32_t *__restrict__ wg_len)
{
    const uint32_t v = perm[blockIdx.x * kWave + threadIdx.x];
    const uint32_t chunk = v / g.channels;
    uint32_t avail = (g.whole_samples - row0[v]) / g.block_len;
    uint32_t m = avail;
    for (int off = 32; off > 0; off >>= 1) m = max(m, (uint32_t)__shfl_xor((int)m, off));
    if (chunk + 1u == g.n_chunks) row0[v] = g.whole_samples - m * g.block_len;
    if (threadIdx.x == 0) wg_blocks[blockIdx.x] = m;
    if (wg_len) {
        uint32_t len = chunk + 1u == g.n_chunks ? m : min(nominal[v], avail);
        for (int off = 32; off > 0; off >>= 1) len = max(len, (uint32_t)__shfl_xor((int)len, off));
        if (threadIdx.x == 0) wg_len[blockIdx.x] = len;
    }
}
__global__ void tp_wg_order_kernel(uint32_t n_wg, const uint32_t *__restrict__ perm, const uint32_t *__restrict__ wg_blocks,
                                   const uint32_t *__restrict__ wg_len, uint32_t *__restrict__ perm_out, uint32_t *__restrict__ wg_blocks_out,
                                   uint32_t pairs)
{
    const uint32_t w = blockIdx.x, lane = threadIdx.x;
    const uint32_t mine = wg_len[w];
    uint32_t rank = 0;
    for (uint32_t j = lane; j < n_wg; j += kWave) { const uint32_t b = wg_len[j]; rank += (b > mine || (b == mine && j < w)) ? 1u : 0u; }
    for (int off = 32; off > 0; off >>= 1) rank += (uint32_t)__shfl_xor((int)rank, off);
    const uint32_t pos = (pairs && (n_wg & 1u) == 0u) ? (rank < n_wg / 2u ? 2u * rank : 2u * (n_wg - 1u - rank) + 1u) : rank;
    perm_out[pos * kWave + lane] = perm[w * kWave + lane];
    if (lane == 0) wg_blocks_out[pos] = wg_blocks[w];
}
hipError_t launch_tp_plan(const float *x, const TpPlan &g, float *energy, uint32_t *own_start, uint32_t *row0,
                          uint32_t *nominal, uint32_t *perm, uint32_t *wg_blocks, bool sorted, hipStream_t stream,
                          uint32_t *perm_out, uint32_t *wg_blocks_out, bool pairs)
{
    const size_t n = (size_t)g.channels * g.scout_blocks;
    const uint32_t columns = g.n_chunks * g.channels;
    hipLaunchKernelGGL(tp_scout_kernel, dim3((unsigned)((4 * n + 255) / 256)), dim3(256), 0, stream, x, g, energy);
    hipLaunchKernelGGL(tp_boundaries_kernel, dim3(g.channels), dim3(kWave), (size_t)g.scout_blocks * 8 + 64 * sizeof(int), stream, energy, g, own_start, row0, nominal);
    if (sorted) {
        hipLaunchKernelGGL(tp_sort_kernel, dim3(1), dim3(kSortThreads), 0, stream, g, row0, nominal, perm);
    } else {
        hipLaunchKernelGGL(tp_iota_kernel, dim3((columns + 255) / 256), dim3(256), 0, stream, perm, columns);
    }
    uint32_t *wg_len = perm_out ? wg_blocks_out + columns / kWave : nullptr;
    hipLaunchKernelGGL(tp_align_kernel, dim3(columns / kWave), dim3(kWave), 0, stream, g, perm, row0, nominal, wg_blocks, wg_len);
    if (perm_out)
        hipLaunchKernelGGL(tp_wg_order_kernel, dim3(columns / kWave), dim3(kWave), 0, stream, columns / kWave, perm, wg_blocks, wg_len,
                           perm_out, wg_blocks_out, pairs ? 1u : 0u);
    return hipGetLastError();
}

__global__ __launch_bounds__(256) void tp_prologue_kernel(uint4 *__restrict__ dst, const uint4 *__restrict__ src, size_t n16,
                                                          uint64_t *__restrict__ handover, uint32_t *__restrict__ sort_cnt, uint32_t n_cols,
                                                          uint32_t *__restrict__ counters)
{
    const size_t t = (size_t)blockIdx.x * blockDim.x + threadIdx.x, stride = (size_t)gridDim.x * blockDim.x;
    for (size_t i = t; i < n16; i += stride) dst[i] = src[i];
    for (size_t i = t; i < n_cols; i += stride) { handover[i] = kNoHandover; if (sort_cnt) sort_cnt[i] = 0u; }
    if (t < 3 && counters) counters[t] = 0u;
}
hipError_t launch_tp_prologue(void *blob, const void *fresh, size_t bytes, uint64_t *handover, uint32_t *sort_cnt, uint32_t n_cols,
                              uint32_t *counters, hipStream_t stream)
{
    const size_t n16 = bytes / 16;
    const unsigned grid = (unsigned)std::min<size_t>((n16 + 255) / 256, 256 * 16);
    hipLaunchKernelGGL(tp_prologue_kernel, dim3(grid ? grid : 1u), dim3(256), 0, stream, reinterpret_cast<uint4 *>(blob),
                       reinterpret_cast<const uint4 *>(fresh), n16, handover, sort_cnt, n_cols, counters);
    return hipGetLastError();
}
__global__ void cast_i16_f32_kernel(const int16_t *__restrict__ in, float *__restrict__ out, size_t n)
{
    for (size_t i = (size_t)blockIdx.x * blockDim.x + threadIdx.x; i < n; i += (size_t)gridDim.x * blockDim.x) out[i] = (float)in[i];
}
hipError_t launch_cast_i16_f32(const int16_t *in, float *out, size_t n, hipStream_t stream)
{
    if (!n) return hipSuccess;
    hipLaunchKernelGGL(cast_i16_f32_kernel, dim3((unsigned)std::min<size_t>((n + 255) / 256, 65536)), dim3(256), 0, stream, in, out, n);
    return hipGetLastError();
}
__global__ void fill_u64_kernel(uint64_t *p, size_t n, uint64_t v)
{
    const size_t i = (size_t)blockIdx.x * blockDim.x + threadIdx.x;
    if (i < n) p[i] = v;
}
hipError_t launch_fill_u64(uint64_t *p, size_t n, uint64_t v, hipStream_t stream)
{
    hipLaunchKernelGGL(fill_u64_kernel, dim3((unsigned)((n + 255) / 256)), dim3(256), 0, stream, p, n, v);
    return hipGetLastError();
}

hipError_t launch_transpose(const float *in, float *out, uint32_t n_channels, uint32_t n_samples,
                            hipStream_t stream)
{
    dim3 grid((n_samples + 63) / 64, (n_channels + 63) / 64);
    hipLaunchKernelGGL(transpose_to_time_major<float>, grid, dim3(256), 0, stream, in, out, n_channels, n_samples);
    return hipGetLastError();
}
hipError_t launch_transpose(const int16_t *in, int16_t *out, uint32_t n_channels, uint32_t n_samples,
                            hipStream_t stream)
{
    dim3 grid((n_samples + 63) / 64, (n_channels + 63) / 64);
    hipLaunchKernelGGL(transpose_to_time_major<int16_t>, grid, dim3(256), 0, stream, in, out, n_channels, n_samples);
    return hipGetLastError();
}

}
```

sameold_amd/csrc/same_kernels_sym.hip:

```cpp
#include <hip/hip_runtime.h>

#include <cmath>
#include <cstdlib>
#include <mutex>
#include <set>
#include <type_traits>
#include <utility>

#include "same_dev_common.h"
#include "same_device.h"
#include "same_fast_common.h"
#include "same_launch.h"
#include "same_pipe_common.h"
#include "same_profile.h"
#include "same_relaxed_common.h"

namespace same {

constexpr int kSymSub = 36;
constexpr uint32_t kSymDrain = 5u;
constexpr uint32_t kSymOffMask = 255u;
template <int NT> struct SymGeom;
template <> struct SymGeom<42> { static constexpr int DCL = 16, NSUB = 1, HALVES = 2; };
template <> struct SymGeom<92> { static constexpr int DCL = 35, NSUB = 2, HALVES = 1; };
// ... 705 lines not shown
            for (int i = 0; i < 16; ++i) samples[i] = *hptr((head + (uint32_t)i) & 63u);
            uint32_t tb = 0u;
#pragma unroll 1
            for (int b = 0; b < 8; ++b) tb |= eq_step_masked(P, train, samples[2 * b], samples[2 * b + 1]) << b;
            byte = train ? tb : byte;
        }
        const bool snap = ready & ((L.flags & F_SQ_LOCK) == 0u);
        if (__builtin_amdgcn_ballot_w64(snap) != 0ull) {
#pragma unroll
            for (int i = 0; i < NFF; ++i) { sffc[i] = snap ? ffc[i] : sffc[i]; sffw[i] = snap ? ffw[i] : sffw[i]; }
#pragma unroll
            for (int i = 0; i < NFB; ++i) { sfbc[i] = snap ? fbc[i] : sfbc[i]; sfbw[i] = snap ? fbw[i] : sfbw[i]; }
        }
        if (__builtin_expect(__builtin_amdgcn_ballot_w64(drop) != 0ull, 0)) end_masked(drop);
        const uint32_t after = L.flags & (F_AGC_LOCKED | F_BW_LOCKED);
        *fb = (valid & ((after != before) | drop)) ? (FB_VALID | ((after & F_AGC_LOCKED) ? FB_AGC : 0u) | ((after & F_BW_LOCKED) ? FB_BW : 0u) | (drop ? FB_END : 0u) | (off << 8)) : 0u;
        return valid ? (YM_VALID | (ready ? YM_READY : 0u) | (adjusted ? YM_ADJUSTED : 0u) | (reading ? YM_READING : 0u) | (drop ? YM_DROP : 0u) |
                        (byte << YM_BYTE_SHIFT) | (off << YM_OFF_SHIFT)) : 0u;
    }
    __device__ __forceinline__ uint32_t symbol(const Params &P, float zero, float sym, uint32_t off, uint32_t *fb)
    {
        const uint32_t before = L.flags & (F_AGC_LOCKED | F_BW_LOCKED);
        const uint32_t slot = (2u * nsym) & 63u;
        const float eq_in0 = nxt0, eq_in1 = nxt1;
        {
            float *pn = hptr((slot + 18u) & 63u), *pw = hptr(slot);
            nxt0 = pn[0]; nxt1 = *reinterpret_cast<float *>(reinterpret_cast<char *>(pn) + hrow4);
            pw[0] = zero; *reinterpret_cast<float *>(reinterpret_cast<char *>(pw) + hrow4) = sym;
        }
        const uint32_t fill = min(64u, L.sq_fill + 2u);
        L.sq_fill = fill;
        L.sq_data = (L.sq_data >> 1) | ((sym >= 0.0f) ? 0x80000000u : 0u);
        const uint32_t nerr = __popc(P.sync_word ^ L.sq_data);
        const float pwr = fmaxf(__builtin_fmaf(__builtin_fmaf(sym, sym, -L.sq_power), P.sq_bw, L.sq_power), 0.0f);
        L.sq_power = pwr;
        L.sq_phist = (L.sq_phist << 1) | ((pwr >= P.sq_power_close) ? 1u : 0u);
        nsym += 1u;
        const int32_t clock_before = L.sq_clock;
        const bool full = fill >= 64u;
        const bool locked = (L.flags & F_SQ_LOCK) != 0u;
        const bool sync_now = full & !locked & (nerr <= P.sq_max_errors) & (pwr >= P.sq_power_open);
        const bool adjusted = sync_now & (clock_before != 0);
        const bool drop = full & !sync_now & (clock_before >= 0) & ((L.sq_phist & 0x80000000u) == 0u);
        int32_t clk = sync_now ? 0 : clock_before;
        clk = drop ? -1 : clk;
        const bool ready = full & (clk == 0);
        const bool reading = full & (clk > 0);
        clk = ready ? 1 : (reading ? ((clk + 1) & 7) : clk);
        L.sq_clock = clk;
        if ((clock_before >= 0) & !adjusted & (ready | reading)) {
            const uint32_t j = (uint32_t)(clock_before + 7) & 7u;
            const uint32_t ebit = eq_symbol_relaxed<NFF, NFB>(P, L, ffc, ffw, fbc, fbw, eq_in0, eq_in1);
            uint32_t bits = (j == 0u) ? 0u : ((L.flags & F_EQ_BITS_MASK) >> F_EQ_BITS_SHIFT);
            bits |= ebit << j;
            L.flags = (L.flags & ~F_EQ_BITS_MASK) | (bits << F_EQ_BITS_SHIFT);
        }
        uint32_t byte = (L.flags & F_EQ_BITS_MASK) >> F_EQ_BITS_SHIFT;
        if (ready & adjusted) {
            if (clock_before >= 0) {
#pragma unroll
                for (int i = 0; i < NFF; ++i) { ffc[i] = sffc[i]; ffw[i] = sffw[i]; }
#pragma unroll
                for (int i = 0; i < NFB; ++i) { fbc[i] = sfbc[i]; fbw[i] = sfbw[i]; }
            }
            L.flags |= F_AGC_LOCKED | F_BW_LOCKED;
            L.flags = (L.flags & ~F_EQ_MODE_MASK) | (2u << F_EQ_MODE_SHIFT);
            L.eq_word = P.sync_word; L.eq_count = 0;
            const uint32_t head = (2u * nsym) & 63u;
            float samples[16];
#pragma unroll
            for (int i = 0; i < 16; ++i) samples[i] = *hptr((head + (uint32_t)i) & 63u);
            byte = 0u;
#pragma unroll 1
            for (int b = 0; b < 8; ++b) byte |= eq_symbol_relaxed<NFF, NFB>(P, L, ffc, ffw, fbc, fbw, samples[2 * b], samples[2 * b + 1]) << b;
        }
        if (ready & !(L.flags & F_SQ_LOCK)) {
#pragma unroll
            for (int i = 0; i < NFF; ++i) { sffc[i] = ffc[i]; sffw[i] = ffw[i]; }
#pragma unroll
            for (int i = 0; i < NFB; ++i) { sfbc[i] = fbc[i]; sfbw[i] = fbw[i]; }
        }
        if (drop) end();
        const uint32_t after = L.flags & (F_AGC_LOCKED | F_BW_LOCKED);
        *fb = (after != before || drop) ? (FB_VALID | ((after & F_AGC_LOCKED) ? FB_AGC : 0u) | ((after & F_BW_LOCKED) ? FB_BW : 0u) | (drop ? FB_END : 0u) | (off << 8)) : 0u;
        return YM_VALID | (ready ? YM_READY : 0u) | (adjusted ? YM_ADJUSTED : 0u) | (reading ? YM_READING : 0u) | (drop ? YM_DROP : 0u) |
               (byte << YM_BYTE_SHIFT) | (off << YM_OFF_SHIFT);
    }
};

struct SymFramer { uint32_t st, last, word, count, invalid, len; };
__device__ __forceinline__ uint32_t sym_framer_step(const Params &P, SymFramer &F, uint8_t *row, uint32_t m, uint32_t *burst_len, uint32_t *fb2, bool *emit)
{
    const bool valid = (m & YM_VALID) != 0u, ready = (m & YM_READY) != 0u, reading = (m & YM_READING) != 0u;
    const uint32_t byte = (m >> YM_BYTE_SHIFT) & 0xffu;
    const bool restart = (m & (YM_READY | YM_ADJUSTED)) == (YM_READY | YM_ADJUSTED);
    const uint32_t st = F.st;
    const bool burst_at_restart = restart & (st == 2u);
    const uint32_t st1 = restart ? 1u : st;
    const uint32_t word0 = restart ? 0u : F.word, count0 = restart ? 0u : F.count;
    const bool searching = ready & (st1 == 1u), rd = ready & (st1 == 2u);
    const uint32_t word = (word0 << 8) | byte, count = count0 + 1u;
    const uint32_t e0 = __popc(word ^ 0x5a435a43u);
    const uint32_t e1 = __popc(word ^ 0x4e4e4e4eu);
    const bool found = searching & (min(e0, e1) <= P.fr_max_prefix_errors);
    const bool give_up = searching & !found & (count > 21u);
    const uint32_t invalid = F.invalid + (is_allowed_byte(byte) ? 0u : 1u);
    const bool over = rd & (invalid > P.fr_max_invalid);
    const bool keep = rd & !over;
    F.word = searching ? word : word0;
    F.count = searching ? count : count0;
    F.invalid = found ? 0u : (rd ? invalid : F.invalid);
    if (found) *reinterpret_cast<uint32_t *>(row) = __builtin_bswap32(word);
    if (keep && F.len < (uint32_t)kBurstCap) row[F.len] = (uint8_t)byte;
    const bool was_reading_burst = valid & !ready & !reading & (st == 2u);
    *burst_len = (over | burst_at_restart | was_reading_burst) ? F.len : 0u;
    F.len = found ? 4u : (keep ? F.len + 1u : F.len);
    const uint32_t nst = found ? 2u : ((give_up | over) ? 0u : st1);
    const uint32_t link_ready = restart ? (burst_at_restart ? 3u : 1u) : (over ? 3u : nst);
    const uint32_t link_quiet = reading ? st : (st == 2u ? 3u : 0u);
    const uint32_t link = ready ? link_ready : link_quiet;
    F.st = ready ? nst : ((valid & !reading) ? 0u : st);
    const uint32_t fb_end = FB_VALID | FB_END | (((m >> YM_OFF_SHIFT) & kSymOffMask) << 8);
    *fb2 = ready ? (link == 2u ? (uint32_t)FB_SQLOCK : ((link == 0u || link == 3u) ? fb_end : 0u)) : 0u;
    *emit = valid & ((link != F.last) | (link == 3u));
    F.last = *emit ? link : F.last;
    return link;
}

#ifndef SYM_PRIOS
#define SYM_PRIOS 0x0031322
#endif
constexpr int sym_prio_of(int k) { return (int)((SYM_PRIOS >> (4 * (6 - k))) & 3); }
#ifndef SYM_PRIOS_HI
#define SYM_PRIOS_HI 0x3321200
#endif
template <int NT> constexpr int sym_prio(int k) { return NT == 42 ? sym_prio_of(k) : (int)((SYM_PRIOS_HI >> (4 * (6 - k))) & 3); }
template <int PRIO> __device__ __forceinline__ void sym_setprio(const Params &P)
{
#ifdef SAME_PROFILE
    const uint32_t variant = ((uint32_t)P.knob_prio >> 12) & 3u;
    if (variant == 1u) return;
    if (variant == 2u) { __builtin_amdgcn_s_setprio(PRIO >= 2 ? 3 : 0); return; }
#else
    (void)P;
#endif
    __builtin_amdgcn_s_setprio(PRIO);
}

__device__ __forceinline__ float sym_next_fire(float s)
{
    return fmaxf(floorf(s - 0.5f) + 1.0f, 1.0f);
}

struct SymKernArgs { Params P; State S; Output O; const float4 *taps; const void *x; uint32_t n_blocks; uint64_t counter0; PipeChunks K; };
typedef const __attribute__((address_space(4))) char *sym_kernarg_ptr;
template <typename T> __device__ __forceinline__ T sym_fresh_arg(sym_kernarg_ptr ka, size_t off)
{
    uint64_t p = (uint64_t)(uintptr_t)ka + off;
    asm volatile("" : "+s"(p));
    T r;
    __builtin_memcpy(&r, reinterpret_cast<const __attribute__((address_space(4))) void *>(p), sizeof(T));
    return r;
}

constexpr int kSymRoles = 6;
template <int NT, int NFF, int NFB, typename SampleT, int CMODE>
__global__ __launch_bounds__(SymGeom<NT>::HALVES * kSymRoles * kWave, NT == 42 ? 3 : 2) void demod_sym_kernel(Params P, State S_arg_, Output O_arg_, const float4 *__restrict__ taps,
                                                                         const SampleT *__restrict__ x, uint32_t n_blocks, uint64_t counter0,
                                                                         PipeChunks K)
{
    (void)S_arg_; (void)O_arg_;
    const sym_kernarg_ptr ka = (sym_kernarg_ptr)__builtin_amdgcn_kernarg_segment_ptr();
    auto fresh_state = [&]() __attribute__((always_inline)) -> State { return sym_fresh_arg<State>(ka, offsetof(SymKernArgs, S)); };
    auto fresh_output = [&]() __attribute__((always_inline)) -> Output { return sym_fresh_arg<Output>(ka, offsetof(SymKernArgs, O)); };
    using LY = SymLayout<NT>;
    constexpr int kB = LY::B, RING = LY::RING, kSB = LY::SB, kNSUB = LY::NSUB;
    constexpr uint32_t kSymHalves = (uint32_t)LY::HALVES;
    constexpr uint32_t LP = kWave;
    static_assert(CMODE == 0 || std::is_same<SampleT, float>::value, "channel-major streams are f32");
    if constexpr (CMODE == 0) { K.col_row0 = nullptr; K.col_perm = nullptr; }
    extern __shared__ float lds_all[];
    const uint32_t lane = threadIdx.x & (kWave - 1u);
    const uint32_t wave = (uint32_t)__builtin_amdgcn_readfirstlane((int)(threadIdx.x >> 6));
    constexpr uint64_t kDeal0 = 0xdcba98543210ull;
#ifdef SAME_PROFILE
    const uint32_t deal = ((uint32_t)P.knob_prio >> 14) & 3u;
    constexpr uint64_t kDeal1 = 0x805d192ab3c4ull;
    constexpr uint64_t kDeal2 = 0x08d591a2b3c4ull;
    constexpr uint64_t kDeal3 = 0x2ad51908b3c4ull;
    const uint64_t tbl = deal == 0u ? kDeal0 : (deal == 1u ? kDeal1 : (deal == 2u ? kDeal2 : kDeal3));
#else
    constexpr uint64_t tbl = kDeal0;
#endif
    const uint32_t hr = LY::HALVES == 2 ? (uint32_t)(tbl >> (4u * wave)) & 15u : wave;
    const uint32_t half = LY::HALVES == 2 ? hr >> 3 : 0u;
    const uint32_t role = hr & 7u;
    const uint32_t C = P.n_channels;
    const uint32_t vwg = blockIdx.x * kSymHalves + half;
    if (vwg * kWave >= C) return;
    float *lds = lds_all + half * (uint32_t)(LY::lds_bytes / sizeof(float));
    const uint32_t c = (K.n_chunks > 1u && K.col_perm) ? K.col_perm[vwg * kWave + lane] : vwg * kWave + lane;
    uint32_t cin = c, Cin = C, n_nominal = n_blocks;
    bool may_leave = false;
    int32_t row_l = 0;
    const SampleT *xl = nullptr;
    uint32_t avail_l = 0;
    if (K.n_chunks > 1u) {
        Cin = K.in_channels;
        if (K.col_row0) {
            const uint32_t chunk_l = c / Cin;
            cin = c - chunk_l * Cin;
            may_leave = (uint32_t)__builtin_amdgcn_readfirstlane((int)chunk_l) + 1u < K.n_chunks;
            const uint32_t row_abs = K.col_row0[c];
            xl = x + (size_t)cin * K.in_samples + row_abs;
            avail_l = (K.whole_samples - row_abs) / (uint32_t)kSB;
            n_blocks = K.wg_blocks[vwg];
            n_nominal = may_leave ? K.col_nominal[c] : n_blocks;
            const uint32_t row_first = (uint32_t)__builtin_amdgcn_readfirstlane((int)row_abs);
            counter0 += (uint64_t)row_first;
            row_l = (int32_t)(row_abs - row_first);
        } else {
            const uint32_t wgs = K.in_channels / kWave;
            const uint32_t chunk = (uint32_t)__builtin_amdgcn_readfirstlane((int)(vwg / wgs));
            cin = (vwg - chunk * wgs) * kWave + lane;
            may_leave = chunk + 1u < K.n_chunks;
            const uint32_t first_block = chunk * K.stride_blocks;
            x += (size_t)first_block * kB * Cin;
            counter0 += (uint64_t)first_block * kB;
            n_blocks -= first_block;
            n_nominal = may_leave ? K.nominal_blocks : n_blocks;
        }
    }
    lds_u32 *mail = (lds_u32 *)(lds + LY::tap_floats);
    lds_u32 *symbox = mail;
    lds_u32 *ybox = symbox + 2u * LY::sym_words;
    lds_u32 *fb1box = ybox + 2u * kWave;
    lds_u32 *fb2box = fb1box + 2u * LY::fb_words;
    lds_u32 *iobox = fb2box + 2u * LY::fb_words;
    lds_u32 *phasebox = iobox + 2u * LY::io_words;
    lds_u32 *againbox = phasebox + kWave;
    lds_u32 *flagbox = againbox + kWave;
    lds_u32 *posbox = flagbox + kWave;
    lds_u32 *sabox = posbox + 2u * kWave;
    lds_u32 *tkbox = sabox + kWave;
    lds_u32 *donebox = tkbox + kIoRingWords;
    lds_u32 *chunkbox = fb1box + kWave + 2u;
    lds_u32 *seqbox = fb1box + kWave + 4u;
    static_assert((size_t)(2u * LY::sym_words + 2u * kWave + 4u * LY::fb_words + 2u * LY::io_words + 3u * kWave + 2u * kWave + kWave + kIoRingWords + kWave + kWave) <= LY::mail_words, "mailboxes");
    float *wring = lds + LY::tap_floats + LY::mail_words;
    float *wcol = wring + lane;
    const uint64_t counter1 = counter0 + (uint64_t)n_blocks * kB;
    const uint32_t last_e_step = n_blocks + kSymDrain;
    const uint32_t last_y1_step = last_e_step + 1u, last_y2_step = last_e_step + 2u, last_a_step = last_e_step + 3u;
    const uint32_t n_steps = last_e_step + 4u;
    auto sym_index = [&](uint32_t s_e, uint32_t off) __attribute__((always_inline)) -> int64_t {
        const int64_t base = s_e <= n_blocks ? (int64_t)s_e - 2 : (int64_t)n_blocks - 3;
        return (int64_t)kB * base + (int64_t)off;
    };
    lds_u32 *prog = donebox + kWave;
    lds_u32 *pos2box = prog + kWave + (SYM_TL_WORDS + 63u) / 64u * 64u;
    lds_u32 *partbox = pos2box + 2u * kWave;
#ifdef SAME_SYM_TL
    lds_u32 *tlbox = prog + kWave;
#endif
    const uint32_t prog_idx = lane < (uint32_t)kSymRoles ? lane : 0u;
    uint32_t *const err_flags = fresh_output().n_events + 2;
    uint32_t spin_limit = 1u << 22;
    auto gave_up = [&]() __attribute__((always_inline)) -> bool { return spin_limit != (1u << 22); };
    constexpr bool kPeek = NT != 42;
    uint32_t seen = 0u;
    auto peek = [&]() __attribute__((always_inline)) { if constexpr (kPeek) seen = prog[prog_idx]; };
    auto wait_for = [&](uint32_t s, uint32_t deps, uint32_t *w_y1, uint32_t *w_y2, auto nap_) __attribute__((always_inline)) {
        constexpr int NAP = decltype(nap_)::value;
        uint32_t v = seen, spins = 0;
        if constexpr (!kPeek) v = prog[prog_idx];
        for (;;) {
            const uint32_t ok = (uint32_t)__builtin_amdgcn_ballot_w64(v >= (s << 16));
            if ((ok & deps) == deps) break;
            if (!kPeek || spins != 0u) __builtin_amdgcn_s_sleep(NAP);
            if (++spins > spin_limit) { if (lane == 0u) atomicOr(err_flags, 4u); spin_limit = 8u; break; }
            v = prog[prog_idx];
        }
        if constexpr (kPeek) seen = v;
        asm volatile("" ::: "memory");
        *w_y1 = (uint32_t)__builtin_amdgcn_readlane((int)v, 4);
        *w_y2 = (uint32_t)__builtin_amdgcn_readlane((int)v, 5);
    };
    constexpr std::integral_constant<int, 1> kNapShort{};
    constexpr std::integral_constant<int, 4> kNapLong{};
    auto flags_of_last = [&](uint32_t w, uint32_t s) __attribute__((always_inline)) -> uint32_t { return s == 0u ? 0u : (w >> (8u * ((s - 1u) & 1u))) & 0xffu; };
    auto publish = [&](uint32_t s, uint32_t flags, uint32_t flags_before) __attribute__((always_inline)) {
        asm volatile("" ::: "memory");
        if (lane == 0u) prog[role] = ((s + 1u) << 16) | (flags << (8u * (s & 1u))) | (flags_before << (8u * ((s + 1u) & 1u)));
    };
    enum : uint32_t { R_S = 1u, R_T = 2u, R_A = 4u, R_E = 8u, R_Y1 = 16u, R_Y2 = 32u };
    enum : uint32_t { Y1F_ANY = 1u, Y2F_END = 1u, Y2F_LEAVE = 2u, Y2F_LOCK = 4u };
    constexpr uint32_t kDepsS = R_T | R_A | R_E | R_Y1 | R_Y2;
    if (role == 0u && lane < (uint32_t)kSymRoles) prog[lane] = 0u;

    if (role == 0u) {
        sym_setprio<sym_prio<NT>(0)>(P);
        SymAgc<NT> M;
        { const State S = fresh_state(); M.load(P, S, c, C, counter0, wcol); }
        lds_barrier();
        P3_T0();
        uint32_t stop_at = 0xffffffffu;
        bool left = false;
        for (uint32_t s = 0; s < n_steps; ++s) {
            uint32_t w1, w2;
            SYM_TRACE(0, s, 0);
            wait_for(s, kDepsS, &w1, &w2, kNapLong);
            SYM_TRACE(0, s, 1);
            P3_LAP(p3_wait);
            const uint32_t f1 = flags_of_last(w1, s), f2 = flags_of_last(w2, s);
            if (f2 & Y2F_LEAVE) stop_at = s;
            if ((f2 & Y2F_END) && s >= 1u) {
                if (fb2box[((s - 1u) & 1u) * LY::fb_words + lane] & FB_VALID) M.locked = false;
            }
            if ((f1 & Y1F_ANY) && s >= 1u) {
                const uint32_t v = fb1box[((s - 1u) & 1u) * LY::fb_words + lane];
                if (v & FB_VALID) {
                    const bool new_locked = (v & FB_AGC) != 0u;
                    if (new_locked && !M.locked) {
                        const int64_t idx = sym_index(s - 2u, v >> 8);
                        const uint32_t b = (uint32_t)(idx / kB);
                        M.gain = M.gain_at(P, wcol, b, (int)(idx - (int64_t)b * kB));
                    }
                    M.locked = new_locked;
                }
                P3_LAP(p3_fb);
            }
            if (s < n_blocks && !PROF_SKIP(P, 64)) M.block(P, wcol, s);
            SYM_TRACE(0, s, 2);
            peek();
            publish(s, 0u, 0u);
            P3_LAP(p3_work);
            if (s == stop_at) { left = true; break; }
        }
        SYM_REPORT(0);
        if (left || gave_up()) return;
        { const State S = fresh_state(); M.store(P, S, c, C, counter1, wcol); }
    } else if (role == 1u) {
        sym_setprio<sym_prio<NT>(1)>(P);
        if constexpr (NT != 42) {
            static_assert(CMODE == 0 && kNSUB == 2, "time-major rows, two sub-blocks a step");
            SymDcRot<SampleT, NT> D;
            const uint32_t n_sub = n_blocks * (uint32_t)kNSUB;
            { const State S = fresh_state(); D.load(S, x, c, C, cin, Cin, counter0, n_sub); }
            donebox[lane] = 0u;
            D.template sub<0>(P, wcol, x, 0u, n_sub, cin, Cin);
            D.template sub<1>(P, wcol, x, 1u, n_sub, cin, Cin);
            lds_barrier();
            P3_T0();
            uint32_t stop_at = 0xffffffffu;
            auto step = [&](uint32_t s, auto ph_) __attribute__((always_inline)) -> bool {
                constexpr int PH = 2 * decltype(ph_)::value;
                uint32_t w1, w2;
                SYM_TRACE(1, s, 0);
                wait_for(s, R_A | R_E, &w1, &w2, kNapLong);
                SYM_TRACE(1, s, 1);
                P3_LAP(p3_wait);
                if (s + 1u < n_blocks && !PROF_SKIP(P, 128)) {
                    D.template sub<PH>(P, wcol, x, 2u * (s + 1u), n_sub, cin, Cin);
                    D.template sub<PH + 1>(P, wcol, x, 2u * (s + 1u) + 1u, n_sub, cin, Cin);
                }
                if (may_leave) {
                    wait_for(s, R_Y2, &w1, &w2, kNapLong);
                    if (flags_of_last(w2, s) & Y2F_LEAVE) stop_at = s;
                }
                SYM_TRACE(1, s, 2);
                peek();
                publish(s, 0u, 0u);
                P3_LAP(p3_work);
                return s == stop_at;
            };
            bool left = false;
            for (uint32_t s = 0; s < n_steps && !left; s += 3u) {
                left = step(s, std::integral_constant<int, 1>{});
                if (!left && s + 1u < n_steps) left = step(s + 1u, std::integral_constant<int, 2>{});
                if (!left && s + 2u < n_steps) left = step(s + 2u, std::integral_constant<int, 0>{});
            }
            SYM_REPORT(1);
            if (left || gave_up()) return;
            { const State S = fresh_state(); D.store(S, c, C, counter1, n_sub - 1u); }
            return;
        } else {
        using Dc = SymDc<SampleT, CMODE, NT>;
        Dc D;
        D.xl = xl; D.avail = avail_l;
        const uint32_t n_sub = n_blocks * (uint32_t)kNSUB;
        { const State S = fresh_state(); D.load(S, x, c, C, cin, Cin, counter0, n_sub); }
        donebox[lane] = 0u;
        auto sub_tm = [&](uint32_t q, auto pb_) __attribute__((always_inline)) {
            typename Dc::Pairs X;
            if constexpr (decltype(pb_)::value == 0) { D.request(D.xb, x, q + 1u, n_sub, cin, Cin); D.template take<0>(D.xa, X); }
            else { D.request(D.xa, x, q + 1u, n_sub, cin, Cin); D.template take<0>(D.xb, X); }
            D.block(P, wcol, X, q);
        };
        {
            if constexpr (CMODE == 1) {
                typename Dc::Pairs X0;
                D.request(D.xb, x, 1u, n_sub, cin, Cin);
                D.template take<9>(D.xa, X0);
                D.block(P, wcol, X0, 0u);
                D.request(D.xa, x, 2u, n_sub, cin, Cin);
            } else {
                sub_tm(0u, std::integral_constant<int, 0>{});
                if constexpr (kNSUB == 2) sub_tm(1u, std::integral_constant<int, 1>{});
            }
        }
        lds_barrier();
        P3_T0();
        uint32_t stop_at = 0xffffffffu;
        auto step = [&](uint32_t s, auto buf) __attribute__((always_inline)) -> bool {
            constexpr int BUF = decltype(buf)::value;
            uint32_t w1, w2;
            SYM_TRACE(1, s, 0);
            wait_for(s, R_A | R_E, &w1, &w2, kNapLong);
            SYM_TRACE(1, s, 1);
            P3_LAP(p3_wait);
            if constexpr (CMODE == 1) D.done = donebox[lane] != 0u;
            if (s + 1u < n_blocks && !PROF_SKIP(P, 128)) {
                if constexpr (CMODE == 1) {
                    typename Dc::Pairs X;
                    if constexpr (BUF == 0) { D.template take<9>(D.xa, X); D.block(P, wcol, X, s + 1u); D.request(D.xa, x, s + 3u, n_sub, cin, Cin); }
                    else { D.template take<9>(D.xb, X); D.block(P, wcol, X, s + 1u); D.request(D.xb, x, s + 3u, n_sub, cin, Cin); }
                } else if constexpr (kNSUB == 1) {
                    sub_tm(s + 1u, buf);
                } else {
                    sub_tm(2u * (s + 1u), std::integral_constant<int, 0>{});
                    sub_tm(2u * (s + 1u) + 1u, std::integral_constant<int, 1>{});
                }
            }
            if (may_leave) {
                wait_for(s, R_Y2, &w1, &w2, kNapLong);
                if (flags_of_last(w2, s) & Y2F_LEAVE) stop_at = s;
            }
            SYM_TRACE(1, s, 2);
            peek();
            publish(s, 0u, 0u);
            P3_LAP(p3_work);
            return s == stop_at;
        };
        bool left = false;
        for (uint32_t s = 0; s < n_steps && !left; s += 2u) {
            left = step(s, std::integral_constant<int, 1>{});
            if (!left && s + 1u < n_steps) left = step(s + 1u, std::integral_constant<int, 0>{});
        }
        SYM_REPORT(1);
        if (left || gave_up()) return;
        { const State S = fresh_state(); D.store(S, c, C, counter1); }
        }
    } else if (role == 2u) {
        sym_setprio<sym_prio<NT>(2)>(P);
        const uint32_t wcol_lds = lds_addr(wcol);
        std::conditional_t<NT == 42, SymTaps<42>, SymHalfTaps<NT, 0, NT / 4>> TP;
        TP.load(taps);
        Lane L;
        IoCtxLds X;
        X.chunk = chunkbox;
        if (lane == 0u) { chunkbox[0] = 0u; chunkbox[1] = kEvChunk; seqbox[0] = 0u; }
        X.pending_slot = 0xffffffffu;
        X.tk = tkbox + lane;
        {
            const State S = fresh_state();
            lane_load(L, S, c);
            X.ring_load(P, S, c);
        }
        const State Snone{};
        Output O{};
        { const Output Of = fresh_output(); O.events = Of.events; O.n_events = Of.n_events; O.event_cap = Of.event_cap; }
        lds_barrier();
        P3_T0();
        uint32_t stop_at = 0xffffffffu;
        bool left = false;
        for (uint32_t s = 0; s < n_steps; ++s) {
            uint32_t w1, w2;
            SYM_TRACE(2, s, 0);
            wait_for(s, R_S | R_E, &w1, &w2, kNapShort);
            SYM_TRACE(2, s, 1);
            P3_LAP(p3_wait);
            if (s >= 1u && s <= last_e_step) {
                const uint32_t n1 = posbox[(s & 1u) * kWave + lane];
                if constexpr (NT == 42) {
                    if (__builtin_amdgcn_ballot_w64(n1 != 0xffffffffu) != 0ull) {
                        const float sa1 = PROF_SKIP(P, 256) ? 0.0f : TP.template demod<RING>(wcol_lds, n1 == 0xffffffffu ? 0 : (int)n1);
                        sabox[lane] = __float_as_uint(sa1);
                        if (lane == 0u) seqbox[0] = 2u * s + 1u;
                    }
                } else {
                    const uint32_t n2 = pos2box[(s & 1u) * kWave + lane];
                    if (__builtin_amdgcn_ballot_w64(n2 != 0xffffffffu) != 0ull) {
                        float2v r2 = {0.0f, 0.0f}, i2 = {0.0f, 0.0f}, r1 = {0.0f, 0.0f}, i1 = {0.0f, 0.0f};
                        if (!PROF_SKIP(P, 256)) {
                            TP.template partial<RING>(wcol_lds, n2 == 0xffffffffu ? 0 : (int)n2, r2, i2);
                            if (__builtin_amdgcn_ballot_w64(n1 != 0xffffffffu) != 0ull) TP.template partial<RING>(wcol_lds, n1 == 0xffffffffu ? 0 : (int)n1, r1, i1);
                        }
                        lds_u32 *pb = partbox + lane;
                        pb[0] = __float_as_uint(r2.x); pb[kWave] = __float_as_uint(r2.y); pb[2 * kWave] = __float_as_uint(i2.x); pb[3 * kWave] = __float_as_uint(i2.y);
                        pb[4 * kWave] = __float_as_uint(r1.x); pb[5 * kWave] = __float_as_uint(r1.y); pb[6 * kWave] = __float_as_uint(i1.x); pb[7 * kWave] = __float_as_uint(i1.y);
                        if (lane == 0u) seqbox[0] = 2u * s + 1u;
                    }
                }
            }
            SYM_TRACE(2, s, 3);
            sym_setprio<sym_prio<NT>(3)>(P);
            wait_for(s, R_Y2, &w1, &w2, kNapLong);
            if (flags_of_last(w2, s) & Y2F_LEAVE) stop_at = s;
            if (s >= 4u && s <= last_a_step && !PROF_SKIP(P, 8)) {
                const lds_u32 *io = iobox + ((s - 1u) & 1u) * LY::io_words + lane;
                const uint32_t io0 = io[0];
                if (io0 & 1u) {
                    L.sq_symbols += 1;
                    const uint32_t link = (io0 >> 1) & 3u, off = (io0 >> 4) & kSymOffMask;
                    const bool burst = (io0 & 8u) != 0u && link == 3u;
                    uint32_t burst_len = 0;
                    if (burst) { X.pending_slot = io[kWave]; burst_len = io[2 * kWave]; }
                    const uint64_t counter = counter0 + (int64_t)row_l + (uint64_t)sym_index(s - 3u, off) + 1u;
                    symbol_io(P, L, Snone, O, X, c, link, (io0 & 8u) != 0u, counter, burst_len);
                }
            }
            if (s + 1u == n_steps) againbox[lane] = L.flags & F_TICK_AGAIN;
            SYM_TRACE(2, s, 2);
            peek();
            publish(s, 0u, 0u);
            sym_setprio<sym_prio<NT>(2)>(P);
            P3_LAP(p3_work);
            if (s == stop_at) { left = true; break; }
        }
        SYM_REPORT(2);
        X.retire(O, lane, kWave);
        if (left || gave_up()) return;
        {
            const State S = fresh_state();
            S.tk_next[c] = L.tk_next; S.tk_last[c] = L.tk_last; S.wake_fired[c] = L.wake_fired;
            X.ring_store(P, S, c);
        }
    } else if (role == 3u) {
        sym_setprio<sym_prio<NT>(4)>(P);
        const uint32_t wcol_lds = lds_addr(wcol);
        std::conditional_t<NT == 42, SymTaps<42>, SymHalfTaps<NT, NT / 4, NT / 2>> TP;
        TP.load(taps);
        Lane L;
        { const State S = fresh_state(); lane_load(L, S, c); }
        const float inv_spt = 1.0f / P.samples_per_ted;
        int cstar = next_fire_count(L.until_next_ted, L.ted_clock);
        int rel = cstar - (int)L.ted_clock - 1;
        float cstar_f = (float)cstar;
        SYM_T_DECL();
        bool pl_typeA = false, pl_ready = false, pl_single = false;
        int pl_p2 = 0;
        uint32_t pl_n2 = 0, pl_n1 = 0xffffffffu;
        float pl_rem1 = 0.0f, pl_instA = 0.0f, pl_c2 = 0.0f;
        auto plan = [&](uint32_t s) __attribute__((always_inline)) {
            pl_single = s > n_blocks;
            const uint32_t wb = (min(s, n_blocks) % (uint32_t)LY::NBLK) * (uint32_t)kB;
            pl_typeA = !pl_single && (L.flags & F_TED_PHASE) != 0u;
            pl_rem1 = L.until_next_ted - cstar_f;
            pl_instA = L.period_inst + __builtin_amdgcn_fmed3f(pl_rem1, -0.5f, 0.5f);
            pl_c2 = sym_next_fire(pl_instA);
            pl_p2 = pl_typeA ? rel + (int)pl_c2 : rel;
            pl_ready = pl_p2 < 0 && s >= 1u && s <= last_e_step;
            auto slot = [&](int p) __attribute__((always_inline)) { int n = (int)wb + p; n += n < 0 ? RING : 0; return (uint32_t)n; };
            pl_n2 = pl_ready ? slot(pl_p2) : 0u;
            pl_n1 = (pl_ready && pl_typeA) ? slot(rel) : 0xffffffffu;
            posbox[(s & 1u) * kWave + lane] = pl_n1;
            if constexpr (NT != 42) pos2box[(s & 1u) * kWave + lane] = pl_ready ? pl_n2 : 0xffffffffu;
        };
        float sa1 = 0.0f, sa2 = 0.0f;
        auto filters = [&](uint32_t seq) __attribute__((always_inline)) {
            sa1 = 0.0f; sa2 = 0.0f;
            if (__builtin_amdgcn_ballot_w64(pl_ready) != 0ull) {
                SYM_T_BEGIN();
                SYM_TCOUNT(20, 1);
                auto wait_for_a = [&]() __attribute__((always_inline)) {
                    uint32_t spins = 0;
                    while ((int32_t)(seqbox[0] - seq) < 0) {
                        __builtin_amdgcn_s_sleep(1);
                        if (++spins > spin_limit) { if (lane == 0u) atomicOr(err_flags, 4u); spin_limit = 8u; break; }
                    }
                    asm volatile("" ::: "memory");
                };
                if constexpr (NT == 42) {
                    sa2 = PROF_SKIP(P, 512) ? 0.0f : TP.template demod<RING>(wcol_lds, (int)pl_n2);
                    SYM_T_LAP(22);
                    if (__builtin_amdgcn_ballot_w64(pl_ready && pl_typeA) != 0ull) {
                        wait_for_a();
                        sa1 = __uint_as_float(sabox[lane]);
                    }
                } else {
                    float2v r2 = {0.0f, 0.0f}, i2 = {0.0f, 0.0f}, r1 = {0.0f, 0.0f}, i1 = {0.0f, 0.0f};
                    const bool any_a = __builtin_amdgcn_ballot_w64(pl_n1 != 0xffffffffu) != 0ull;
                    if (!PROF_SKIP(P, 512)) {
                        TP.template partial<RING>(wcol_lds, (int)pl_n2, r2, i2);
                        if (any_a) TP.template partial<RING>(wcol_lds, pl_n1 == 0xffffffffu ? 0 : (int)pl_n1, r1, i1);
                    }
                    SYM_T_LAP(22);
                    wait_for_a();
                    const lds_u32 *pb = partbox + lane;
                    r2 += float2v{__uint_as_float(pb[0]), __uint_as_float(pb[kWave])}; i2 += float2v{__uint_as_float(pb[2 * kWave]), __uint_as_float(pb[3 * kWave])};
                    sa2 = sym_soft_sample(r2, i2);
                    if (any_a) {
                        r1 += float2v{__uint_as_float(pb[4 * kWave]), __uint_as_float(pb[5 * kWave])}; i1 += float2v{__uint_as_float(pb[6 * kWave]), __uint_as_float(pb[7 * kWave])};
                        sa1 = sym_soft_sample(r1, i1);
                    }
                }
                SYM_T_LAP(24);
            }
        };
        auto work = [&](uint32_t s) __attribute__((always_inline)) {
            SYM_T_BEGIN();
            const bool rdy = pl_ready, tA = pl_typeA;
            const float p1 = tA ? L.h2 : L.h1, p2 = tA ? sa1 : L.h2;
            const float inst_pre = tA ? pl_instA : L.period_inst;
            const float rem = tA ? pl_instA - pl_c2 : pl_rem1;
            const uint32_t flags_new = tA ? L.flags : (L.flags ^ F_TED_PHASE);
            const bool have = (flags_new & F_TED_PHASE) != 0u;
            const float dsg = rs_signum(p1) - rs_signum(sa2);
            const float te = p2 * dsg;
            const float offset = __builtin_amdgcn_fmed3f(rem, -0.5f, 0.5f);
            const float e = __builtin_amdgcn_fmed3f(__builtin_fmaf(-offset, inv_spt, te), -1.0f, 1.0f);
            const bool bw_locked = (L.flags & F_BW_LOCKED) != 0u;
            const float alpha = bw_locked ? P.alpha_locked : P.alpha_unlocked;
            const float beta = bw_locked ? P.beta_locked : P.beta_unlocked;
            const float avg1 = __builtin_amdgcn_fmed3f(__builtin_fmaf(beta, e, L.period_avg), P.period_min, P.period_max);
            float inst1 = __builtin_fmaf(alpha, e, avg1) + offset;
            inst1 = (inst1 < 0.0f) ? avg1 : inst1;
            const float inst_new = have ? inst1 : inst_pre + offset;
            const float cs = sym_next_fire(inst_new);
            const bool take = rdy & have;
            L.h0 = rdy ? p1 : L.h0; L.h1 = rdy ? p2 : L.h1; L.h2 = rdy ? sa2 : L.h2;
            L.flags = rdy ? flags_new : L.flags;
            L.period_avg = take ? avg1 : L.period_avg;
            L.period_inst = rdy ? inst_new : L.period_inst; L.until_next_ted = rdy ? inst_new : L.until_next_ted;
            cstar_f = rdy ? cs : cstar_f;
            rel = rdy ? pl_p2 + (int)cs : rel;
            const uint32_t hdr = take ? (1u | ((uint32_t)(pl_p2 + (pl_single ? 3 * kB : 2 * kB)) << 8)) : 0u;
            SYM_T_LAP(23);
            lds_u32 *sb = symbox + (s & 1u) * LY::sym_words + lane;
            sb[0] = hdr;
            sb[kWave] = __float_as_uint(p2); sb[2 * kWave] = __float_as_uint(sa2);
            if (P.trace_cap) { sb[3 * kWave] = __float_as_uint(te); sb[4 * kWave] = __float_as_uint(inst_new); }
        };
        auto late = [&](uint32_t v) __attribute__((always_inline)) {
            if (v & FB_VALID) {
                L.flags = (L.flags & ~F_BW_LOCKED) | ((v & FB_BW) ? F_BW_LOCKED : 0u);
                if (v & FB_END) {
                    L.flags &= ~F_TED_PHASE;
                    L.h0 = 0.0f; L.h1 = 0.0f; L.h2 = 0.0f;
                    L.period_avg = P.samples_per_ted; L.period_inst = P.samples_per_ted;
                }
            }
        };
        plan(0u);
        lds_barrier();
        P3_T0();
        uint32_t stop_at = 0xffffffffu;
        bool left = false;
        for (uint32_t s = 0; s < n_steps; ++s) {
            uint32_t w1, w2;
            SYM_TRACE(3, s, 0);
            wait_for(s, R_S, &w1, &w2, kNapShort);
            SYM_TRACE(3, s, 1);
            P3_LAP(p3_wait);
            if (!PROF_SKIP(P, 32)) filters(2u * s + 1u);
            wait_for(s, R_A | R_Y1 | R_Y2, &w1, &w2, kNapShort);
            SYM_TRACE(3, s, 3);
            const uint32_t f1 = flags_of_last(w1, s), f2 = flags_of_last(w2, s);
            if (f2 & Y2F_LEAVE) stop_at = s;
            uint32_t late1 = 0u, late2 = 0u;
            if ((f1 & Y1F_ANY) && s >= 1u) late1 = fb1box[((s - 1u) & 1u) * LY::fb_words + lane];
            if ((f2 & Y2F_END) && s >= 1u) late2 = fb2box[((s - 1u) & 1u) * LY::fb_words + lane];
            if (!PROF_SKIP(P, 32)) {
                work(s);
                if (__builtin_amdgcn_ballot_w64(((late1 | late2) & FB_VALID) != 0u) != 0ull) { late(late2); late(late1); }
                if (s + 1u <= n_blocks) rel -= kB;
                plan(s + 1u);
            }
            if (s + 1u == n_steps) phasebox[lane] = L.flags & F_TED_PHASE;
            SYM_TRACE(3, s, 2);
            peek();
            publish(s, 0u, 0u);
            P3_LAP(p3_work);
            if (s == stop_at) { left = true; break; }
        }
        SYM_REPORT(3);
        SYM_T_REPORT();
        if (left || gave_up()) return;
        L.ted_clock = (uint32_t)((int)cstar_f - rel - 1);
        {
            const State S = fresh_state();
            S.until_next_ted[c] = L.until_next_ted; S.ted_clock[c] = L.ted_clock;
            S.ted_h0[c] = L.h0; S.ted_h1[c] = L.h1; S.ted_h2[c] = L.h2;
            S.period_avg[c] = L.period_avg; S.period_inst[c] = L.period_inst;
        }
    } else if (role == 4u) {
        sym_setprio<sym_prio<NT>(5)>(P);
        SymSquelch<NFF, NFB> Q;
        uint64_t symbols0;
        const bool hist_copy = K.n_chunks > 1u && K.col_perm != nullptr && K.hist_scratch != nullptr;
        {
            const State S = fresh_state();
            lane_load(Q.L, S, c);
            symbols0 = Q.L.sq_symbols;
            Q.nsym = (uint32_t)symbols0;
            Q.hbase = reinterpret_cast<char *>(hist_copy ? K.hist_scratch : S.sq_hist);
            Q.hcol4 = (hist_copy ? vwg * kWave + lane : c) * 4u;
            Q.hrow4 = C * 4u;
            if (hist_copy) {
#pragma unroll 4
                for (int i = 0; i < kSquelchHist; ++i) *Q.hptr((uint32_t)i) = S.sq_hist[(size_t)i * C + c];
            }
#pragma unroll
            for (int i = 0; i < NFF; ++i) {
                Q.ffc[i] = S.eq_ffc[i * C + c]; Q.ffw[i] = S.eq_ffw[i * C + c];
                Q.sffc[i] = S.eq_snap_ffc[i * C + c]; Q.sffw[i] = S.eq_snap_ffw[i * C + c];
            }
#pragma unroll
            for (int i = 0; i < NFB; ++i) {
                Q.fbc[i] = S.eq_fbc[i * C + c]; Q.fbw[i] = S.eq_fbw[i * C + c];
                Q.sfbc[i] = S.eq_snap_fbc[i * C + c]; Q.sfbw[i] = S.eq_snap_fbw[i * C + c];
            }
            const uint32_t pslot = (2u * Q.nsym) & 63u;
            Q.nxt0 = *Q.hptr((pslot + 16u) & 63u); Q.nxt1 = *Q.hptr((pslot + 17u) & 63u);
        }
        lds_barrier();
        P3_T0();
        uint32_t stop_at = 0xffffffffu, flags_before = 0u, last_msg = 0u;
        bool left = false;
        for (uint32_t s = 0; s < n_steps; ++s) {
            uint32_t w1, w2;
            SYM_TRACE(4, s, 0);
            wait_for(s, R_E | R_Y2 | R_S, &w1, &w2, kNapShort);
            SYM_TRACE(4, s, 1);
            P3_LAP(p3_wait);
            const uint32_t f2 = flags_of_last(w2, s);
            if (f2 & Y2F_LEAVE) stop_at = s;
            if ((f2 & (Y2F_END | Y2F_LOCK)) && s >= 1u) {
                const uint32_t from_y2 = fb2box[((s - 1u) & 1u) * LY::fb_words + lane];
                const bool superseded = (last_msg & (YM_DROP | YM_ADJUSTED)) != 0u;
#ifdef SYM_Y1_SELECT
                Q.L.flags |= ((from_y2 & FB_SQLOCK) && !superseded) ? (uint32_t)F_SQ_LOCK : 0u;
                const bool y2_end = (from_y2 & FB_END) && !superseded;
                if (__builtin_expect(__builtin_amdgcn_ballot_w64(y2_end) != 0ull, 0)) Q.end_masked(y2_end);
#else
                if ((from_y2 & FB_SQLOCK) && !superseded) Q.L.flags |= F_SQ_LOCK;
                if ((from_y2 & FB_END) && !superseded) Q.end();
#endif
            }
            last_msg = 0u;
            uint32_t flags = 0u;
            if (s >= 2u && s <= last_y1_step) {
                const lds_u32 *sb = symbox + ((s - 1u) & 1u) * LY::sym_words + lane;
                const uint32_t hdr = sb[0], zero_w = sb[kWave], sym_w = sb[2 * kWave];
                uint32_t msg = 0u, fbv = 0u;
#ifdef SYM_Y1_SELECT
                {
                    const bool valid = (hdr & 1u) && !PROF_SKIP(P, 16);
                    const uint32_t off = hdr >> 8;
                    const float zero = __uint_as_float(zero_w), sym = __uint_as_float(sym_w);
                    if (P.trace_cap && valid) {
                        const State S = fresh_state();
                        const uint64_t counter = counter0 + (int64_t)row_l + (uint64_t)sym_index(s - 1u, off) + 1u;
                        const uint32_t n = S.trace_n[c];
                        if (n < P.trace_cap) {
                            float *t = S.trace + ((size_t)c * P.trace_cap + n) * 4;
                            t[0] = zero; t[1] = sym; t[2] = __uint_as_float(sb[3 * kWave]); t[3] = __uint_as_float(sb[4 * kWave]);
                            S.trace_idx[(size_t)c * P.trace_cap + n] = counter;
                        }
                        S.trace_n[c] = n + 1;
                    }
                    msg = Q.symbol_masked(P, valid, zero, sym, off, &fbv);
                }
#else
                if ((hdr & 1u) && !PROF_SKIP(P, 16)) {
                    const uint32_t off = hdr >> 8;
                    const float zero = __uint_as_float(zero_w), sym = __uint_as_float(sym_w);
                    if (P.trace_cap) {
                        const State S = fresh_state();
                        const uint64_t counter = counter0 + (int64_t)row_l + (uint64_t)sym_index(s - 1u, off) + 1u;
                        const uint32_t n = S.trace_n[c];
                        if (n < P.trace_cap) {
                            float *t = S.trace + ((size_t)c * P.trace_cap + n) * 4;
                            t[0] = zero; t[1] = sym; t[2] = __uint_as_float(sb[3 * kWave]); t[3] = __uint_as_float(sb[4 * kWave]);
                            S.trace_idx[(size_t)c * P.trace_cap + n] = counter;
                        }
                        S.trace_n[c] = n + 1;
                    }
                    msg = Q.symbol(P, zero, sym, off, &fbv);
                }
#endif
                ybox[(s & 1u) * kWave + lane] = msg;
                last_msg = msg;
                if (__builtin_amdgcn_ballot_w64(fbv != 0u) != 0ull) {
                    uint32_t u1, u2;
                    wait_for(s, R_S, &u1, &u2, kNapLong);
                    fb1box[(s & 1u) * LY::fb_words + lane] = fbv; flags = Y1F_ANY;
                }
            }
            if (s + 1u == n_steps) flagbox[lane] = Q.L.flags & (F_AGC_LOCKED | F_BW_LOCKED | F_SQ_LOCK | F_EQ_MODE_MASK | F_EQ_BITS_MASK);
            SYM_TRACE(4, s, 2);
            peek();
            publish(s, flags, flags_before);
            flags_before = flags;
            P3_LAP(p3_work);
            if (s == stop_at) { left = true; break; }
        }
        SYM_REPORT(4);
        if (left || gave_up()) return;
        const State S = fresh_state();
        S.sq_data[c] = Q.L.sq_data; S.sq_power[c] = Q.L.sq_power; S.sq_phist[c] = Q.L.sq_phist;
        S.sq_fill[c] = Q.L.sq_fill; S.sq_clock[c] = Q.L.sq_clock; S.sq_symbols[c] = symbols0 + (uint64_t)(Q.nsym - (uint32_t)symbols0);
        S.eq_word[c] = Q.L.eq_word; S.eq_count[c] = Q.L.eq_count;
        if (hist_copy) {
#pragma unroll 4
            for (int i = 0; i < kSquelchHist; ++i) S.sq_hist[(size_t)i * C + c] = *Q.hptr((uint32_t)i);
        }
#pragma unroll
        for (int i = 0; i < NFF; ++i) {
            S.eq_ffc[i * C + c] = Q.ffc[i]; S.eq_ffw[i * C + c] = Q.ffw[i];
            S.eq_snap_ffc[i * C + c] = Q.sffc[i]; S.eq_snap_ffw[i * C + c] = Q.sffw[i];
        }
#pragma unroll
        for (int i = 0; i < NFB; ++i) {
            S.eq_fbc[i * C + c] = Q.fbc[i]; S.eq_fbw[i * C + c] = Q.fbw[i];
            S.eq_snap_fbc[i * C + c] = Q.sfbc[i]; S.eq_snap_fbw[i * C + c] = Q.sfbw[i];
        }
    } else {
        sym_setprio<sym_prio<NT>(6)>(P);
        Lane L;
        SymFramer F;
        uint8_t *fr_rows;
        { const State S0 = fresh_state(); lane_load(L, S0, c); fr_rows = S0.fr_msg; }
        F.st = fr_state(L); F.last = (L.flags & F_LINK_MASK) >> F_LINK_SHIFT;
        F.word = L.fr_word; F.count = L.fr_count; F.invalid = L.fr_invalid; F.len = L.fr_len;
        uint8_t *const row = fr_rows + (size_t)c * kBurstCap;
        Output O{};
        { const Output Of = fresh_output(); O.n_events = Of.n_events; O.bursts = Of.bursts; O.burst_cap = Of.burst_cap; }
        lds_barrier();
        P3_T0();
        uint32_t stop_at = 0xffffffffu, flags_before = 0u;
        bool left = false, lane_done = false, leave_posted = false;
        for (uint32_t s = 0; s < n_steps; ++s) {
            uint32_t w1, w2;
            SYM_TRACE(5, s, 0);
            wait_for(s, R_Y1 | R_S | R_T | R_A | R_E, &w1, &w2, kNapShort);
            SYM_TRACE(5, s, 1);
            P3_LAP(p3_wait);
            uint32_t flags = 0u;
            if (s >= 3u && s <= last_y2_step) {
                const uint32_t m = PROF_SKIP(P, 1024) ? 0u : ybox[((s - 1u) & 1u) * kWave + lane];
                uint32_t fbv = 0, burst_len = 0, io1 = 0xffffffffu;
                bool emit = false;
                const uint32_t link = sym_framer_step(P, F, row, m, &burst_len, &fbv, &emit);
                const bool want_slot = emit & (link == 3u);
                const uint32_t io0 = (m & YM_VALID) ? (1u | (link << 1) | (emit ? 8u : 0u) | (((m >> YM_OFF_SHIFT) & kSymOffMask) << 4)) : 0u;
                uint64_t pend = __builtin_amdgcn_ballot_w64(want_slot);
                lds_u32 *io = iobox + (s & 1u) * LY::io_words + lane;
                if (pend != 0ull) {
                    const uint32_t n_new = (uint32_t)__popcll(pend);
                    uint32_t base = 0;
                    if (lane == 0u) base = atomicAdd(O.n_events + 1, n_new);
                    base = (uint32_t)__builtin_amdgcn_readfirstlane((int)base);
                    uint32_t k = 0;
                    while (pend != 0ull) {
                        const int j = __builtin_ctzll(pend);
                        pend &= pend - 1ull;
                        const uint32_t b = base + k++;
                        const uint32_t cj = (uint32_t)__builtin_amdgcn_readlane((int)c, j);
                        if (b < O.burst_cap) {
                            const uint32_t *src = reinterpret_cast<const uint32_t *>(fr_rows + (size_t)cj * kBurstCap);
                            uint32_t *dst = reinterpret_cast<uint32_t *>(O.bursts + (size_t)b * kBurstCap);
                            constexpr uint32_t kWords = (uint32_t)kBurstCap / 4u, kPer = (kWords + kWave - 1u) / kWave;
                            uint32_t t[kPer];
#pragma unroll
                            for (uint32_t i = 0; i < kPer; ++i) { const uint32_t w = lane + i * kWave; t[i] = w < kWords ? src[w] : 0u; }
#pragma unroll
                            for (uint32_t i = 0; i < kPer; ++i) { const uint32_t w = lane + i * kWave; if (w < kWords) dst[w] = t[i]; }
                            if ((int)lane == j) io1 = b;
                        } else {
                            if (lane == 0u) atomicOr(O.n_events + 2, 2u);
                            if ((int)lane == j) io1 = 0xffffffffu;
                        }
                    }
                    io[kWave] = io1; io[2 * kWave] = burst_len;
                }
                io[0] = io0;
                const bool any_end = __builtin_amdgcn_ballot_w64((fbv & FB_VALID) != 0u) != 0ull;
                const bool any_lock = __builtin_amdgcn_ballot_w64((fbv & FB_SQLOCK) != 0u) != 0ull;
                if (any_end || any_lock) fb2box[(s & 1u) * LY::fb_words + lane] = fbv;
                flags = (any_end ? Y2F_END : 0u) | (any_lock ? Y2F_LOCK : 0u);
                if (may_leave && !leave_posted) {
                    const uint32_t blk = min(s - 3u, n_blocks - 1u);
                    if (!lane_done && blk + 1u >= n_nominal && F.last == 0u && (xl == nullptr || blk < avail_l)) {
                        lane_done = true;
                        K.handover[c] = counter0 + (int64_t)row_l + (uint64_t)(blk + 1u) * kB;
                        donebox[lane] = 1u;
                    }
                    if (__builtin_amdgcn_ballot_w64(!lane_done) == 0ull) { flags |= Y2F_LEAVE; leave_posted = true; stop_at = s + 1u; }
                }
            }
            SYM_TRACE(5, s, 2);
            peek();
            publish(s, flags, flags_before);
            flags_before = flags;
            P3_LAP(p3_work);
            if (s == stop_at) { left = true; break; }
        }
        SYM_REPORT(5);
        SYM_COUNT(18, 1);
        SYM_COUNT(19, left ? stop_at + 1u : n_steps);
        if (left || gave_up()) return;
        uint32_t w1, w2;
        wait_for(n_steps, R_A | R_E | R_Y1, &w1, &w2, kNapShort);
        if (gave_up()) return;
        const uint32_t flags_out = (F.st << F_FR_STATE_SHIFT) | (F.last << F_LINK_SHIFT) | (phasebox[lane] & F_TED_PHASE) | (againbox[lane] & F_TICK_AGAIN) | flagbox[lane];
        const State S1 = fresh_state();
        S1.fr_word[c] = F.word; S1.fr_count[c] = F.count; S1.fr_invalid[c] = F.invalid;
        S1.fr_len[c] = F.len; S1.flags[c] = flags_out;
    }
}

#if !defined(SAME_PROFILE) && !defined(SAME_SYM_TL)
#define SYM_SPLIT_TU 1
#endif
static_assert(SymLayout<42>::B == kSymStep22 && SymLayout<92>::B == kSymStepHi && SymLayout<84>::B == kSymStepHi && SymLayout<42>::NBLK == kSymRingSteps &&
              SymLayout<92>::NBLK == kSymRingSteps, "same_select.h decides with these steps and this ring");

template <int NT, int NFF, int NFB, typename SampleT>
static hipError_t launch_sym_one(const Params &P, const State &S, const Output &O, const float4 *taps, const SampleT *x,
                                 uint32_t n_blocks, uint64_t counter0, hipStream_t stream, const PipeChunks &K)
{
    constexpr uint32_t kSymHalves = (uint32_t)SymLayout<NT>::HALVES;
    constexpr size_t lds = (size_t)kSymHalves * SymLayout<NT>::lds_bytes;
    static_assert(lds <= 160u * 1024u, "one workgroup per CU");
    const bool cm = K.n_chunks > 1u && K.col_row0 != nullptr;
    if (cm && (!std::is_same<SampleT, float>::value || NT != 42)) return hipErrorInvalidValue;
    if (K.n_chunks > 1u && (K.in_channels % kWave) != 0u) return hipErrorInvalidValue;
    if (n_blocks == 0u) return hipSuccess;
    auto go = [&](auto kernel) -> hipError_t {
        if (lds > 64u * 1024u) {
            static std::mutex mu;
            static std::set<std::pair<const void *, int>> opted_in;
            int dev = 0;
            if (hipGetDevice(&dev) != hipSuccess) return hipErrorInvalidDevice;
            const std::pair<const void *, int> key(reinterpret_cast<const void *>(kernel), dev);
            std::lock_guard<std::mutex> lock(mu);
            if (opted_in.find(key) == opted_in.end()) {
                const hipError_t e = hipFuncSetAttribute(key.first, hipFuncAttributeMaxDynamicSharedMemorySize, (int)lds);
                if (e != hipSuccess) return e;
                opted_in.insert(key);
            }
        }
        hipLaunchKernelGGL(kernel, dim3((P.n_channels / kWave + kSymHalves - 1u) / kSymHalves), dim3(kSymHalves * kSymRoles * kWave), lds, stream, P, S, O, taps, x, n_blocks, counter0, K);
        return hipGetLastError();
    };
    if constexpr (std::is_same<SampleT, float>::value && NT == 42) {
        if (cm) return go(demod_sym_kernel<NT, NFF, NFB, float, 1>);
    }
    return go(demod_sym_kernel<NT, NFF, NFB, SampleT, 0>);
}

template <typename SampleT>
static hipError_t launch_sym_hi_t(const Params &P, const State &S, const Output &O, const float4 *taps, const SampleT *x,
                                  uint32_t n_blocks, uint64_t counter0, hipStream_t stream, const PipeChunks &K)
{
    const bool eq = P.eq_nff == 6u && P.eq_nfb == 4u;
    if (standard_rate_taps(P) == 92u)
        return eq ? launch_sym_one<92, 6, 4, SampleT>(P, S, O, taps, x, n_blocks, counter0, stream, K) : launch_sym_one<92, 1, 1, SampleT>(P, S, O, taps, x, n_blocks, counter0, stream, K);
    return eq ? launch_sym_one<84, 6, 4, SampleT>(P, S, O, taps, x, n_blocks, counter0, stream, K) : launch_sym_one<84, 1, 1, SampleT>(P, S, O, taps, x, n_blocks, counter0, stream, K);
}
#if defined(SYM_TU_HI)
#if defined(SYM_SPLIT_TU)
hipError_t launch_demod_sym_hi(const Params &P, const State &S, const Output &O, const float4 *taps, const float *x,
                               uint32_t n_blocks, uint64_t counter0, hipStream_t stream, const PipeChunks &K)
{ return launch_sym_hi_t<float>(P, S, O, taps, x, n_blocks, counter0, stream, K); }
hipError_t launch_demod_sym_hi(const Params &P, const State &S, const Output &O, const float4 *taps, const int16_t *x,
                               uint32_t n_blocks, uint64_t counter0, hipStream_t stream, const PipeChunks &K)
{ return launch_sym_hi_t<int16_t>(P, S, O, taps, x, n_blocks, counter0, stream, K); }
#endif
#else
#if defined(SYM_SPLIT_TU)
hipError_t launch_demod_sym_hi(const Params &P, const State &S, const Output &O, const float4 *taps, const float *x,
                               uint32_t n_blocks, uint64_t counter0, hipStream_t stream, const PipeChunks &K);
hipError_t launch_demod_sym_hi(const Params &P, const State &S, const Output &O, const float4 *taps, const int16_t *x,
                               uint32_t n_blocks, uint64_t counter0, hipStream_t stream, const PipeChunks &K);
#else
template <typename SampleT>
static hipError_t launch_demod_sym_hi(const Params &P, const State &S, const Output &O, const float4 *taps, const SampleT *x,
                                      uint32_t n_blocks, uint64_t counter0, hipStream_t stream, const PipeChunks &K)
{ return launch_sym_hi_t<SampleT>(P, S, O, taps, x, n_blocks, counter0, stream, K); }
#endif
template <typename SampleT>
static hipError_t launch_sym_t(const Params &P, const State &S, const Output &O, const float4 *taps, const SampleT *x,
                               uint32_t n_blocks, uint64_t counter0, hipStream_t stream, const PipeChunks &K)
{
    if (!sym_kernel_supported(P)) return hipErrorInvalidValue;
    const bool eq = P.eq_nff == 6u && P.eq_nfb == 4u;
    if (standard_rate_taps(P) == 42u)
        return eq ? launch_sym_one<42, 6, 4, SampleT>(P, S, O, taps, x, n_blocks, counter0, stream, K) : launch_sym_one<42, 1, 1, SampleT>(P, S, O, taps, x, n_blocks, counter0, stream, K);
    return launch_demod_sym_hi(P, S, O, taps, x, n_blocks, counter0, stream, K);
}
hipError_t launch_demod_sym(const Params &P, const State &S, const Output &O, const float4 *taps, const float *x,
                            uint32_t n_blocks, uint64_t counter0, hipStream_t stream, const PipeChunks &K)
{ return launch_sym_t<float>(P, S, O, taps, x, n_blocks, counter0, stream, K); }
hipError_t launch_demod_sym(const Params &P, const State &S, const Output &O, const float4 *taps, const int16_t *x,
                            uint32_t n_blocks, uint64_t counter0, hipStream_t stream, const PipeChunks &K)
{ return launch_sym_t<int16_t>(P, S, O, taps, x, n_blocks, counter0, stream, K); }
#endif

}

#if !defined(SYM_TU_HI)
SYM_PROFILE_EXPORTS()
#endif
```

sameold_amd/csrc/same_launch.h:

```cpp
#pragma once

#include <hip/hip_runtime.h>

#include "same_capture_dev.h"
#include "same_device.h"
#include "same_select.h"

namespace same {

hipError_t launch_demod(const Params &P, const State &S, const Output &O, const float4 *taps,
                        const float *x, uint32_t n_samples, uint64_t counter0, hipStream_t stream);
hipError_t launch_demod(const Params &P, const State &S, const Output &O, const float4 *taps,
                        const int16_t *x, uint32_t n_samples, uint64_t counter0, hipStream_t stream);
hipError_t launch_demod_ragged(const Params &P, const State &S, const Output &O, const float4 *taps, const float *x,
                               uint32_t n_rows, const uint32_t *counts, uint32_t row_sub, uint64_t counter0, hipStream_t stream);
hipError_t launch_demod_ragged(const Params &P, const State &S, const Output &O, const float4 *taps, const int16_t *x,
                               uint32_t n_rows, const uint32_t *counts, uint32_t row_sub, uint64_t counter0, hipStream_t stream);
hipError_t launch_demod_pipe(const Params &P, const State &S, const Output &O, const float4 *taps,
                             const float *x, uint32_t n_blocks, uint64_t counter0, hipStream_t stream,
                             const PipeChunks &chunks = PipeChunks{}, bool relaxed = false);
hipError_t launch_demod_pipe(const Params &P, const State &S, const Output &O, const float4 *taps,
                             const int16_t *x, uint32_t n_blocks, uint64_t counter0, hipStream_t stream,
                             const PipeChunks &chunks = PipeChunks{}, bool relaxed = false);
hipError_t launch_demod_sym(const Params &P, const State &S, const Output &O, const float4 *taps,
                            const float *x, uint32_t n_blocks, uint64_t counter0, hipStream_t stream,
                            const PipeChunks &chunks = PipeChunks{});
hipError_t launch_demod_sym(const Params &P, const State &S, const Output &O, const float4 *taps,
                            const int16_t *x, uint32_t n_blocks, uint64_t counter0, hipStream_t stream,
                            const PipeChunks &chunks = PipeChunks{});
hipError_t launch_demod_relaxed(const Params &P, const State &S, const Output &O, const float4 *taps,
                                const float *x, uint32_t n_blocks, uint64_t counter0, hipStream_t stream,
                                const PipeChunks &chunks = PipeChunks{});
hipError_t launch_demod_relaxed(const Params &P, const State &S, const Output &O, const float4 *taps,
                                const int16_t *x, uint32_t n_blocks, uint64_t counter0, hipStream_t stream,
                                const PipeChunks &chunks = PipeChunks{});
hipError_t launch_demod_fast(const Params &P, const State &S, const Output &O, const float4 *taps,
                             const float *x, uint32_t n_blocks, uint64_t counter0, hipStream_t stream);
hipError_t launch_demod_fast(const Params &P, const State &S, const Output &O, const float4 *taps,
                             const int16_t *x, uint32_t n_blocks, uint64_t counter0, hipStream_t stream);
hipError_t launch_counters(uint32_t *dev, uint32_t *host_mapped, int publish, hipStream_t stream);
hipError_t launch_event_sort(const DevEvent *ev, const uint32_t *counters, uint32_t cap, uint32_t n_bins, uint32_t *cnt, uint32_t *first,
                             DevEvent *sorted, hipStream_t stream, bool cnt_is_zero = false);
hipError_t launch_init_state(const Params &P, const State &S, int is_reset, hipStream_t stream, uint32_t first_col = 0);
hipError_t launch_reset_columns(const Params &P, const State &S, const uint32_t *cols, uint32_t n, hipStream_t stream);
hipError_t launch_copy_state_columns(const StateArrayDesc *desc, uint32_t n_desc, uint32_t src_channels,
                                     uint32_t dst_channels, const uint32_t *src_col, uint32_t n_cols, hipStream_t stream,
                                     uint32_t src_base = 0);
hipError_t launch_chunk_final_column(const uint64_t *handover, uint32_t in_channels, ChunkGeom g, uint32_t *final_col,
                                     hipStream_t stream);
hipError_t launch_chunk_final_column_pc(const uint64_t *handover, const uint32_t *own_start, uint32_t in_channels, uint32_t n_chunks,
                                        uint64_t counter0, uint32_t *final_col, hipStream_t stream);
hipError_t launch_fill_u64(uint64_t *p, size_t n, uint64_t v, hipStream_t stream);
hipError_t launch_cast_i16_f32(const int16_t *in, float *out, size_t n, hipStream_t stream);
hipError_t launch_tp_prologue(void *blob, const void *fresh, size_t bytes, uint64_t *handover, uint32_t *sort_cnt, uint32_t n_cols,
                              uint32_t *counters, hipStream_t stream);
struct TpPlan {
    uint32_t channels, n_chunks, block_len, warmup_samples, whole_samples;
    uint64_t in_samples;
    uint32_t scout_blocks;
};
hipError_t launch_tp_plan(const float *x, const TpPlan &g, float *energy, uint32_t *own_start, uint32_t *row0,
                          uint32_t *nominal, uint32_t *perm, uint32_t *wg_blocks, bool sorted, hipStream_t stream,
                          uint32_t *perm_out = nullptr, uint32_t *wg_blocks_out = nullptr, bool pairs = false);
hipError_t launch_transpose(const float *in, float *out, uint32_t n_channels, uint32_t n_samples,
                            hipStream_t stream);
hipError_t launch_transpose(const int16_t *in, int16_t *out, uint32_t n_channels, uint32_t n_samples,
                            hipStream_t stream);

constexpr uint32_t kMessageLogOverflow = 8u;
struct TransportLaunch {
    uint32_t n_channels, input_rate;
    const uint32_t *first;
    DevEvent *sorted;
    const uint32_t *counters;
    const uint8_t *bursts; uint32_t burst_cap;
    void *hot, *cold;
    uint64_t *wake_sample;
    DevMessage *near; uint32_t near_cap;
    DevMessage *log; uint32_t log_cap;
    uint32_t *log_cursor, *overflow;
    cap::Launch cap;
};
size_t transport_hot_bytes();
size_t transport_cold_bytes();
hipError_t launch_transport(const TransportLaunch &T, hipStream_t stream);
hipError_t launch_transport_ragged(const TransportLaunch &T, const uint32_t *counts, uint32_t row_sub, uint32_t n_rows, hipStream_t stream);
hipError_t launch_transport_reset(void *hot, void *cold, uint32_t n_channels, const uint32_t *cols, uint32_t n, int fresh,
                                  hipStream_t stream, void *capture_rec = nullptr);
hipError_t launch_capture(const cap::Span *spans, cap::Cursors *cur, uint32_t span_cap, float *pool, uint64_t pool_cap,
                          const float *x, uint32_t n_channels, uint32_t n_rows, cap::Cursors *host, hipStream_t stream);
hipError_t launch_capture(const cap::Span *spans, cap::Cursors *cur, uint32_t span_cap, float *pool, uint64_t pool_cap,
                          const int16_t *x, uint32_t n_channels, uint32_t n_rows, cap::Cursors *host, hipStream_t stream);

struct SynthParams {
    uint32_t n_channels;
    uint32_t input_rate;
    uint64_t seed;
    float noise_sigma;
    uint32_t flags;
};
hipError_t launch_synth(const SynthParams &sp, float *x, size_t n_samples, hipStream_t stream);
struct TrialParams {
    uint32_t n_trials;
    uint32_t first_trial;
    uint32_t input_rate;
    uint32_t n_grid;
    uint64_t seed;
    float ebn0_db_lo, ebn0_db_step;
};
hipError_t launch_trials(const TrialParams &tp, float *x, size_t n_samples, hipStream_t stream);
uint32_t synth_payload(uint64_t seed, uint32_t channel, uint8_t *out, uint32_t cap);

}
```

sameold_amd/csrc/same_pipe_common.h:

```cpp
#pragma once

#include <hip/hip_runtime.h>

#include "same_dev_common.h"
#include "same_device.h"

namespace same {

typedef volatile __attribute__((address_space(3))) uint32_t lds_u32;

__device__ __forceinline__ void lds_barrier()
{
    asm volatile("s_waitcnt lgkmcnt(0)\n\ts_barrier" ::: "memory");
}

__device__ __forceinline__ uint32_t burst_to_pool(const State &S, const Output &O, uint32_t c)
{
    const uint32_t b = atomicAdd(O.n_events + 1, 1u);
    if (b >= O.burst_cap) { atomicOr(O.n_events + 2, 2u); return 0xffffffffu; }
    copy_burst_row(O.bursts + (size_t)b * kBurstCap, S.fr_msg + (size_t)c * kBurstCap);
    return b;
}

constexpr uint32_t kEvChunk = 64;
struct IoCtx : TickRingGlobal {
    lds_u32 *chunk;
    uint32_t pending_slot;
    __device__ __forceinline__ void mark(int) const {}
    __device__ __forceinline__ void emit(const Params &P, const State &S, const Output &O, uint32_t c, uint32_t kind,
                                         uint64_t sample_counter, uint64_t symbols, uint32_t burst_len)
    {
        const uint64_t act = __builtin_amdgcn_ballot_w64(true);
        const uint32_t n = (uint32_t)__popcll(act);
        const uint32_t rank = __builtin_amdgcn_mbcnt_hi((uint32_t)(act >> 32), __builtin_amdgcn_mbcnt_lo((uint32_t)act, 0u));
        uint32_t base = chunk[0], used = chunk[1];
        if (used + n > kEvChunk) {
            for (uint32_t i = used + rank; i < kEvChunk; i += n)
                if (base + i < O.event_cap) { O.events[base + i].channel = 0; O.events[base + i].kind = kDevEventNone; }
            uint32_t nb = 0;
            if (rank == 0u) nb = atomicAdd(O.n_events, kEvChunk);
            base = (uint32_t)__builtin_amdgcn_readfirstlane((int)nb);
            used = 0;
        }
        const uint32_t e = base + used + rank;
        chunk[0] = base; chunk[1] = used + n;
        if (e < O.event_cap) {
            DevEvent ev;
            ev.channel = c; ev.kind = kind; ev.sample_counter = sample_counter;
            ev.symbol_count = symbols; ev.burst_len = burst_len;
            ev.burst_slot = kind == 3u ? pending_slot : 0xffffffffu;
            O.events[e] = ev;
        } else {
            atomicOr(O.n_events + 2, 1u);
        }
    }
    __device__ __forceinline__ void retire(const Output &O, uint32_t lane, uint32_t lanes)
    {
        const uint32_t base = chunk[0], used = chunk[1];
        for (uint32_t i = used + lane; i < kEvChunk; i += lanes)
            if (base + i < O.event_cap) { O.events[base + i].channel = 0; O.events[base + i].kind = kDevEventNone; }
    }
};

constexpr uint32_t kIoRingWords = (2u * (uint32_t)kTickRing + 1u) * kWave;
struct IoCtxLds : IoCtx {
    lds_u32 *tk;
    __device__ __forceinline__ uint32_t tk_count(const State &, uint32_t) const { return tk[2 * kTickRing * kWave]; }
    __device__ __forceinline__ void tk_set_count(const State &, uint32_t, uint32_t n) const { tk[2 * kTickRing * kWave] = n; }
    __device__ __forceinline__ uint64_t tk_at(const State &, uint32_t, uint32_t, uint32_t i) const
    {
        return (uint64_t)tk[2u * i * kWave] | ((uint64_t)tk[(2u * i + 1u) * kWave] << 32);
    }
    __device__ __forceinline__ void tk_set(const State &, uint32_t, uint32_t, uint32_t i, uint64_t v) const
    {
        tk[2u * i * kWave] = (uint32_t)v; tk[(2u * i + 1u) * kWave] = (uint32_t)(v >> 32);
    }
    __device__ __forceinline__ void ring_load(const Params &P, const State &S, uint32_t c)
    {
        if (!P.ticks) return;
        const TickRingGlobal G;
#pragma unroll
        for (uint32_t i = 0; i < (uint32_t)kTickRing; ++i) tk_set(S, P.n_channels, c, i, G.tk_at(S, P.n_channels, c, i));
        tk_set_count(S, c, G.tk_count(S, c));
    }
    __device__ __forceinline__ void ring_store(const Params &P, const State &S, uint32_t c) const
    {
        if (!P.ticks) return;
        const TickRingGlobal G;
#pragma unroll
        for (uint32_t i = 0; i < (uint32_t)kTickRing; ++i) G.tk_set(S, P.n_channels, c, i, tk_at(S, P.n_channels, c, i));
        G.tk_set_count(S, c, tk_count(S, c));
    }
};

}
```

sameold_amd/csrc/same_tp_plan.h:

```cpp
#pragma once

#include <stddef.h>
#include <stdint.h>

#include "same_config.h"
#include "same_device.h"
#include "same_select.h"

namespace same {

#ifndef SAME_SCOUT_BLOCK
#define SAME_SCOUT_BLOCK 256
#endif
constexpr uint32_t kScoutBlock = SAME_SCOUT_BLOCK;
constexpr uint32_t kScanThreads = 1024;
inline uint32_t event_sort_extra_words(uint32_t n_bins) { return (n_bins + kScanThreads - 1u) / kScanThreads; }

constexpr size_t kMaxLaunchSamples = (size_t)1 << 22;
inline size_t max_launch_samples(uint32_t input_rate) { return kMaxLaunchSamples < (size_t)input_rate * 45 ? kMaxLaunchSamples : (size_t)input_rate * 45; }

struct TpConfig {
    uint32_t max_chunks = 0, min_own = 0, warmup = 0;
    int sort_mode = -1;
    int knob_plan_stream = 0;
    int knob_prologue = 0;
};

struct TpCut {
    uint32_t n_chunks = 1;
    Choice choice;
    ChunkGeom geom{};
    PipeChunks pc{};
};
TpCut tp_uniform_cut(const Params &P, const Mode &m, const Request &rq, const TpConfig &cfg, size_t n, uint64_t counter0,
                     uint32_t column_cap = kTpColumnCap, bool channel_major = false);

TpCut tp_native_cut(const Params &P, const Mode &m, const Request &rq, const TpConfig &cfg, size_t n_call, uint64_t counter0);
struct TpGeomWords {
    size_t own_start = 0, row0 = 0, nominal = 0, perm = 0, wg = 0, wg2 = 0, perm2 = 0;
    size_t total = 0;
    size_t harvest = 0;
};
struct TpNative {
    bool qualifies = false;
    uint32_t whole_samples = 0;
    uint32_t warmup_samples = 0, scout_blocks = 0;
    uint64_t in_samples = 0;
    int sort_mode = 0;
    bool pair_groups = false;
    bool lpt = false;
    bool need_hist = false;
    size_t hist_floats = 0, energy_floats = 0;
    TpGeomWords words;
};
TpNative tp_native_plan(const Params &P, const TpConfig &cfg, const TpCut &cut, size_t n_call, uintptr_t base);
inline bool tp_plan_beside(const TpConfig &cfg, bool own_stream) { return own_stream && cfg.knob_plan_stream >= 0; }

constexpr size_t kSpanBytes = 32;
struct OutputCaps {
    size_t events = 0, bursts = 0;
    size_t messages = 0, near = 0, spans = 0;
    size_t bins = 0, sort_words = 0;
};
OutputCaps output_caps(const Params &P, size_t n_samples, size_t n_columns, bool dev_transport, bool audio, size_t near_cap, size_t msg_cap);
inline size_t tp_output_samples(size_t n, const PipeChunks &pc, uint32_t block_len)
{
    const size_t m = 3 * (size_t)pc.nominal_blocks * block_len + 65536;
    return n < m ? n : m;
}

}
```

Measured before the change: 468,900.

## Overlap fresh time-parallel chunks with previous launch via double-buffered state and self-start

Double-buffers the time-parallel state blob and descriptors per slot. A slim prologue replaces the full blob copy, and the sym kernel loads its own start state directly. Chunks that start from fresh state are launched on a side stream so they can run alongside the previous launch's tail, while the chunk that continues from carried state waits on the main stream. Timing is adjusted to measure from the previous launch's stop event. This adds stream and event complexity and doubles state memory, and the timing change could also alter how throughput is reported.

```diff
diff --git a/sameold_amd/csrc/same_batch.cpp b/sameold_amd/csrc/same_batch.cpp
--- a/sameold_amd/csrc/same_batch.cpp
+++ b/sameold_amd/csrc/same_batch.cpp
@@ -62,6 +62,9 @@
         same::Event ev_start, ev_stop, ev_done, ev_planned;
         same::Event ev_k0, ev_k1;
         bool have_k = false;
+        same::Event ev_prologue, ev_fresh;
+        bool overlapped = false;
+        int stop_idx = 0, prev_stop = -1;
         bool timed = false;
         same::PinnedBuf<void> h_events, h_bursts;
         bool in_flight = false;
@@ -104,11 +107,12 @@
         uint32_t carved_columns = 0;
         int carved_family = -1;
         same::Params Pv{};
-        same::State Sv{};
-        same::DevBuf<void> blob;
+        same::State Sv[2]{};
+        same::State Sf{};
+        same::DevBuf<void> blob[2];
         same::DevBuf<void> blob_fresh;
         size_t fresh_bytes = 0;
-        same::DevBuf<same::StateArrayDesc> d_desc_in, d_desc_out;
+        same::DevBuf<same::StateArrayDesc> d_desc_in[2], d_desc_out[2];
         uint32_t n_desc = 0;
         same::DevBuf<uint32_t> d_final_col;
         same::DevBuf<float> d_energy;
@@ -133,6 +137,7 @@
     } inv;
     hipStream_t plan_stream = nullptr;
     float last_ms = 0.0f;
+    same::Event ev_stops[4];
     bool overflowed = false;
     std::string record_path;
     bool kernel_fault = false;
@@ -147,6 +152,7 @@
     same::DevBuf<void> d_upload;
     same::DevBuf<void> d_zero;
     same::Event ev_order;
+    bool order_recorded = false;
     bool timing = false;
     bool have_timing = false;
     float last_demod_ms = 0.0f;
@@ -256,6 +262,7 @@
     rx->tp.cfg.sort_mode = num("SAME_TP_SORT", -1);
     rx->tp.cfg.knob_plan_stream = tri("SAME_TP_PLAN_STREAM");
     rx->tp.cfg.knob_prologue = tri("SAME_TP_PROLOGUE");
+    rx->tp.cfg.overlap = std::min(2, std::max(0, num("SAME_TP_OVERLAP", 2)));
     rx->want.knob_relaxed = tri("SAME_RELAXED");
     { const char *e = std::getenv("SAME_RELAXED_KERNEL"); rx->P.knob_relaxed_kernel = !e ? 0 : (std::strcmp(e, "solo") == 0 ? 1 : (std::strcmp(e, "duo") == 0 ? 2 : 0)); }
     { const char *e = std::getenv("SAME_TP_KERNEL"); rx->want.knob_tp_kernel = !e ? 0 : (std::strcmp(e, "wave") == 0 ? 2 : (std::strcmp(e, "pipe") == 0 ? 1 : 0)); }
@@ -421,6 +428,17 @@
         HIP_TRY(hipEventElapsedTime(&rx->last_ms, sl.ev_start, sl.ev_stop));
         rx->last_demod_ms = rx->last_ms;
         if (sl.have_k) HIP_TRY(hipEventElapsedTime(&rx->last_demod_ms, sl.ev_k0, sl.ev_k1));
+        if (sl.overlapped && sl.prev_stop >= 0) {
+            float since = 0.0f;
+            HIP_TRY(hipEventElapsedTime(&since, rx->ev_stops[sl.prev_stop], sl.ev_stop));
+            rx->last_ms = std::min(rx->last_ms, since);
+            if (sl.have_k) {
+                HIP_TRY(hipEventElapsedTime(&since, rx->ev_stops[sl.prev_stop], sl.ev_k1));
+                rx->last_demod_ms = std::min(rx->last_demod_ms, since);
+            } else {
+                rx->last_demod_ms = rx->last_ms;
+            }
+        }
         rx->have_timing = true;
     }
     auto t_waited = std::chrono::steady_clock::now();
@@ -518,32 +536,36 @@
     tp.Pv = same::wide_params(rx->P, columns, same::is_fastmath(tp.family), same::tp_more_than_one_round(columns));
     if (columns > tp.cap_columns) {
         tp.cap_columns = 0;
-        HIP_TRY(tp.blob.reset());
+        for (auto &b : tp.blob) HIP_TRY(b.reset());
         HIP_TRY(tp.blob_fresh.reset());
-        const size_t bytes = carve_state(tp.Pv, nullptr, tp.Sv);
-        HIP_TRY(tp.blob.ensure(bytes));
-        HIP_TRY(hipMemset(tp.blob, 0, bytes));
+        const size_t bytes = carve_state(tp.Pv, nullptr, tp.Sv[0]);
+        for (auto &b : tp.blob) {
+            HIP_TRY(b.ensure(bytes));
+            HIP_TRY(hipMemset(b, 0, bytes));
+        }
         HIP_TRY(tp.blob_fresh.ensure(bytes));
         tp.cap_columns = columns;
     }
-    const size_t blob_bytes = carve_state(tp.Pv, (char *)tp.blob.get(), tp.Sv);
+    size_t blob_bytes = 0;
+    for (int w = 0; w < 2; ++w) blob_bytes = carve_state(tp.Pv, (char *)tp.blob[w].get(), tp.Sv[w]);
     {
-        same::State Sf{};
-        carve_state(tp.Pv, (char *)tp.blob_fresh.get(), Sf);
+        carve_state(tp.Pv, (char *)tp.blob_fresh.get(), tp.Sf);
         HIP_TRY(hipMemset(tp.blob_fresh, 0, blob_bytes));
-        HIP_TRY(same::launch_init_state(tp.Pv, Sf, 0, nullptr, 0));
+        HIP_TRY(same::launch_init_state(tp.Pv, tp.Sf, 0, nullptr, 0));
         HIP_TRY(hipDeviceSynchronize());
-        tp.fresh_bytes = (size_t)(reinterpret_cast<char *>(tp.Sv.fr_msg) - static_cast<char *>(tp.blob.get()));
-    }
-    std::vector<same::StateArrayDesc> in, out;
-    list_state_arrays(rx->P, rx->S, tp.Sv, in);
-    list_state_arrays(rx->P, tp.Sv, rx->S, out);
-    tp.n_desc = (uint32_t)in.size();
-    HIP_TRY(tp.d_desc_in.ensure(in.size()));
-    HIP_TRY(tp.d_desc_out.ensure(out.size()));
+        tp.fresh_bytes = (size_t)(reinterpret_cast<char *>(tp.Sv[0].fr_msg) - static_cast<char *>(tp.blob[0].get()));
+    }
+    for (int w = 0; w < 2; ++w) {
+        std::vector<same::StateArrayDesc> in, out;
+        list_state_arrays(rx->P, rx->S, tp.Sv[w], in);
+        list_state_arrays(rx->P, tp.Sv[w], rx->S, out);
+        tp.n_desc = (uint32_t)in.size();
+        HIP_TRY(tp.d_desc_in[w].ensure(in.size()));
+        HIP_TRY(tp.d_desc_out[w].ensure(out.size()));
+        HIP_TRY(hipMemcpy(tp.d_desc_in[w], in.data(), in.size() * sizeof(same::StateArrayDesc), hipMemcpyHostToDevice));
+        HIP_TRY(hipMemcpy(tp.d_desc_out[w], out.data(), out.size() * sizeof(same::StateArrayDesc), hipMemcpyHostToDevice));
+    }
     HIP_TRY(tp.d_final_col.ensure(rx->P.n_channels));
-    HIP_TRY(hipMemcpy(tp.d_desc_in, in.data(), in.size() * sizeof(same::StateArrayDesc), hipMemcpyHostToDevice));
-    HIP_TRY(hipMemcpy(tp.d_desc_out, out.data(), out.size() * sizeof(same::StateArrayDesc), hipMemcpyHostToDevice));
     tp.carved_columns = columns;
     tp.carved_family = (int)tp.family;
     return SAME_OK;
@@ -576,22 +598,32 @@
     return SAME_OK;
 }
 
-int tp_start(same_batch *rx, same_batch::Slot &sl, uint32_t columns, const char *layout, hipStream_t stream, bool *sort_bins_empty)
+int tp_start(same_batch *rx, same_batch::Slot &sl, uint32_t columns, const char *layout, hipStream_t stream, bool *sort_bins_empty, bool self_start,
+             bool beside = false)
 {
     same_batch::TimePar &tp = rx->tp;
     const uint32_t C = rx->P.n_channels;
+    const same::State &Sv = tp.Sv[&sl - rx->slot];
     *sort_bins_empty = false;
+    if (self_start) {
+        HIP_TRY(same::launch_tp_prologue_slim(Sv.sq_hist, tp.Sf.sq_hist, beside ? nullptr : rx->S.sq_hist, same::kSquelchHist, C, sl.d_handover, sl.d_sort,
+                                              columns, sl.d_counters, stream));
+        *sort_bins_empty = sl.sort_bins == columns;
+        if (rx->debug) std::fprintf(stderr, "[same] time-parallel launch: %u columns (%s), start-up: the kernel loads its start state%s\n", columns, layout,
+                                    beside ? ", fresh pieces beside the launch before" : "");
+        return SAME_OK;
+    }
     if (tp.cfg.knob_prologue >= 0) {
-        HIP_TRY(same::launch_tp_prologue(tp.blob, tp.blob_fresh, tp.fresh_bytes, sl.d_handover, sl.d_sort, columns, sl.d_counters, stream));
+        HIP_TRY(same::launch_tp_prologue(tp.blob[&sl - rx->slot], tp.blob_fresh, tp.fresh_bytes, sl.d_handover, sl.d_sort, columns, sl.d_counters, stream));
         *sort_bins_empty = sl.sort_bins == columns;
     } else {
         HIP_TRY(same::launch_counters(sl.d_counters, sl.h_counters.dev(), 0, stream));
-        HIP_TRY(same::launch_init_state(tp.Pv, tp.Sv, 0, stream, C));
+        HIP_TRY(same::launch_init_state(tp.Pv, Sv, 0, stream, C));
         HIP_TRY(same::launch_fill_u64(sl.d_handover, columns, same::kNoHandover, stream));
     }
     if (rx->debug) std::fprintf(stderr, "[same] time-parallel launch: %u columns (%s), start-up: %s\n", columns, layout,
                                 tp.cfg.knob_prologue >= 0 ? "prologue kernel" : "separate launches");
-    HIP_TRY(same::launch_copy_state_columns(tp.d_desc_in, tp.n_desc, C, columns, nullptr, C, stream));
+    HIP_TRY(same::launch_copy_state_columns(tp.d_desc_in[&sl - rx->slot], tp.n_desc, C, columns, nullptr, C, stream));
     return SAME_OK;
 }
 
@@ -615,7 +647,7 @@
 }
 
 int tp_plan_boundaries(same_batch *rx, same_batch::Slot &sl, const same::TpCut &cut, const same::TpNative &np, const float *d_x,
-                       hipStream_t stream, same::PipeChunks &pc)
+                       hipStream_t stream, same::PipeChunks &pc, bool beside = false)
 {
     same_batch::TimePar &tp = rx->tp;
     const same::TpGeomWords &w = np.words;
@@ -627,16 +659,17 @@
     sl.plan_sorted = np.sort_mode != 0; sl.plan_lpt = np.lpt; sl.plan_pairs = np.pair_groups;
     uint32_t *g = sl.d_geom;
     const bool side = same::tp_plan_beside(tp.cfg, stream == rx->own_stream);
-    hipStream_t ps = side ? rx->plan_stream : stream;
+    hipStream_t ps = beside ? rx->copy_stream : (side ? rx->plan_stream : stream);
+    if (beside && rx->order_recorded) HIP_TRY(hipStreamWaitEvent(ps, rx->ev_order, 0));
     if (tp.plan_recorded) HIP_TRY(hipStreamWaitEvent(ps, tp.ev_plan_prev, 0));
     HIP_TRY(same::launch_tp_plan(d_x, plan, tp.d_energy, g + w.own_start, g + w.row0, g + w.nominal, g + w.perm, g + w.wg, np.sort_mode != 0, ps,
                                  np.lpt ? g + w.perm2 : nullptr, np.lpt ? g + w.wg2 : nullptr, np.pair_groups));
     HIP_TRY(tp.ev_plan_prev.ensure());
     HIP_TRY(hipEventRecord(tp.ev_plan_prev, ps));
     tp.plan_recorded = true;
-    if (side) {
+    if (side || beside) {
         HIP_TRY(hipEventRecord(sl.ev_planned, ps));
-        HIP_TRY(hipStreamWaitEvent(stream, sl.ev_planned, 0));
+        HIP_TRY(hipStreamWaitEvent(beside ? rx->plan_stream : stream, sl.ev_planned, 0));
     }
     pc.col_row0 = g + w.row0; pc.col_nominal = g + w.nominal;
     pc.wg_blocks = g + (np.lpt ? w.wg2 : w.wg); pc.col_perm = np.lpt ? g + w.perm2 : nullptr;
@@ -670,22 +703,55 @@
         if (np->need_hist) HIP_TRY(tp.d_hist.ensure(np->hist_floats));
         sl.words = np->words;
     }
-    rc = begin_timing(rx, sl, stream);
+    const int w = (int)(&sl - rx->slot);
+    const same::State &Sv = tp.Sv[w];
+    const bool self_start = same::tp_self_start(tp.cfg, np, tp.family, stream == rx->own_stream, C);
+    const bool beside = same::tp_overlap(tp.cfg, self_start);
+    const same_batch::Slot &other = rx->slot[w ^ 1];
+    sl.overlapped = beside;
+    sl.prev_stop = other.in_flight && other.timed ? other.stop_idx : -1;
+    rc = begin_timing(rx, sl, beside ? rx->copy_stream : stream);
     if (rc) return rc;
     const float *xf = nullptr;
     if constexpr (std::is_same_v<SampleT, float>) xf = x;
-    if (np && (rc = tp_plan_boundaries(rx, sl, cut, *np, xf, stream, pc)) != SAME_OK) return rc;
-    rc = tp_start(rx, sl, columns, np ? "channel-major" : "time-major", stream, sort_bins_empty);
-    if (rc) return rc;
+    if (np && (rc = tp_plan_boundaries(rx, sl, cut, *np, xf, stream, pc, beside)) != SAME_OK) return rc;
     sl.have_k = np && sl.timed;
-    if (sl.have_k) HIP_TRY(hipEventRecord(sl.ev_k0, stream));
-    const hipError_t e = launch_family(tp.family, tp.Pv, tp.Sv, O, rx->d_taps, x, total_blocks, rx->counter, stream, pc);
+    hipError_t e = hipSuccess;
+    if (beside) {
+        hipStream_t fs = rx->plan_stream;
+        if (sl.seq != 0) HIP_TRY(hipStreamWaitEvent(fs, sl.ev_done, 0));
+        rc = tp_start(rx, sl, columns, "channel-major", fs, sort_bins_empty, true, true);
+        if (rc) return rc;
+        HIP_TRY(hipEventRecord(sl.ev_prologue, fs));
+        if (sl.have_k) HIP_TRY(hipEventRecord(sl.ev_k0, fs));
+        const same::TpGroups gf = same::tp_groups(C, cut.n_chunks, true), g0 = same::tp_groups(C, cut.n_chunks, false);
+        same::SymStart start{rx->S, tp.Sf};
+        start.first_group = gf.first; start.n_groups = gf.count;
+        e = same::launch_demod_sym(tp.Pv, Sv, O, rx->d_taps, xf, total_blocks, rx->counter, fs, pc, &start);
+        if (e == hipSuccess) {
+            HIP_TRY(hipEventRecord(sl.ev_fresh, fs));
+            HIP_TRY(hipStreamWaitEvent(stream, sl.ev_prologue, 0));
+            start.first_group = g0.first; start.n_groups = g0.count; start.copy_hist = true;
+            e = same::launch_demod_sym(tp.Pv, Sv, O, rx->d_taps, xf, total_blocks, rx->counter, stream, pc, &start);
+            HIP_TRY(hipStreamWaitEvent(stream, sl.ev_fresh, 0));
+        }
+    } else {
+        rc = tp_start(rx, sl, columns, np ? "channel-major" : "time-major", stream, sort_bins_empty, self_start);
+        if (rc) return rc;
+        if (sl.have_k) HIP_TRY(hipEventRecord(sl.ev_k0, stream));
+        if (self_start) {
+            const same::SymStart start{rx->S, tp.Sf};
+            e = same::launch_demod_sym(tp.Pv, Sv, O, rx->d_taps, xf, total_blocks, rx->counter, stream, pc, &start);
+        } else {
+            e = launch_family(tp.family, tp.Pv, Sv, O, rx->d_taps, x, total_blocks, rx->counter, stream, pc);
+        }
+    }
     rx->last_family = tp.family;
     if (e != hipSuccess) return fail(SAME_EHIP, "time-parallel demod kernel launch failed: %s", hipGetErrorString(e));
     if (sl.have_k) HIP_TRY(hipEventRecord(sl.ev_k1, stream));
     if (np) HIP_TRY(same::launch_chunk_final_column_pc(sl.d_handover, sl.d_geom + np->words.own_start, C, geom.n_chunks, rx->counter, tp.d_final_col, stream));
     else HIP_TRY(same::launch_chunk_final_column(sl.d_handover, C, geom, tp.d_final_col, stream));
-    HIP_TRY(same::launch_copy_state_columns(tp.d_desc_out, tp.n_desc, columns, C, tp.d_final_col, C, stream));
+    HIP_TRY(same::launch_copy_state_columns(tp.d_desc_out[w], tp.n_desc, columns, C, tp.d_final_col, C, stream));
     if (n_whole < n_call) {
         rc = np ? demod_tail_corner(rx, O, xf + n_whole, n_call, n_call - n_whole, rx->counter + n_whole, stream)
                 : demod_tail(rx, O, x + n_whole * C, n_call - n_whole, rx->counter + n_whole, stream);
@@ -702,7 +768,11 @@
 int end_launch(same_batch *rx, same_batch::Slot &sl, same_batch::Slot &prev, hipStream_t stream, const SampleT *rows, size_t n,
                bool sort_bins_empty, const RaggedLaunch *rl = nullptr)
 {
-    if (sl.timed) HIP_TRY(hipEventRecord(sl.ev_stop, stream));
+    if (sl.timed) {
+        HIP_TRY(hipEventRecord(sl.ev_stop, stream));
+        sl.stop_idx = (int)(rx->launch_seq & 3);
+        HIP_TRY(hipEventRecord(rx->ev_stops[sl.stop_idx], stream));
+    }
     HIP_TRY(same::launch_event_sort(sl.d_events, sl.d_counters, sl.event_cap(), sl.sort_bins, sl.d_sort, sl.d_sort + sl.sort_bins,
                                     sl.d_sorted, stream, sort_bins_empty));
     sl.dev_transport = rx->dev_transport && !sl.chunked;
@@ -1154,6 +1224,7 @@
     TRY_OR_CLEAN(hipStreamCreateWithFlags(&rx->copy_stream, hipStreamNonBlocking));
     TRY_OR_CLEAN(hipStreamCreateWithFlags(&rx->plan_stream, hipStreamNonBlocking));
     TRY_OR_CLEAN(rx->ev_order.ensure());
+    for (auto &ev : rx->ev_stops) TRY_OR_CLEAN(ev.ensure(hipEventDefault));
     for (auto &sl : rx->slot) {
         TRY_OR_CLEAN(sl.ev_start.ensure(hipEventDefault));
         TRY_OR_CLEAN(sl.ev_stop.ensure(hipEventDefault));
@@ -1161,6 +1232,8 @@
         TRY_OR_CLEAN(sl.ev_k1.ensure(hipEventDefault));
         TRY_OR_CLEAN(sl.ev_done.ensure());
         TRY_OR_CLEAN(sl.ev_planned.ensure());
+        TRY_OR_CLEAN(sl.ev_prologue.ensure());
+        TRY_OR_CLEAN(sl.ev_fresh.ensure());
         TRY_OR_CLEAN(sl.d_counters.ensure(4));
         TRY_OR_CLEAN(sl.h_counters.ensure(4));
     }
@@ -1320,6 +1393,7 @@
     HIP_TRY(hipEventRecord(rx->ev_order, (hipStream_t)producer_stream));
     HIP_TRY(hipStreamWaitEvent(rx->own_stream, rx->ev_order, 0));
     HIP_TRY(hipStreamWaitEvent(rx->plan_stream, rx->ev_order, 0));
+    rx->order_recorded = true;
     return SAME_OK;
 }
 
diff --git a/sameold_amd/csrc/same_device.h b/sameold_amd/csrc/same_device.h
--- a/sameold_amd/csrc/same_device.h
+++ b/sameold_amd/csrc/same_device.h
@@ -110,6 +110,12 @@
     uint32_t whole_samples;
 };
 
+struct SymStart {
+    State own, fresh;
+    uint32_t first_group = 0, n_groups = 0;
+    bool copy_hist = false;
+};
+
 struct ChunkGeom {
     uint64_t counter0;
     uint32_t n_chunks, block_len, stride_blocks, warmup_blocks;
diff --git a/sameold_amd/csrc/same_kernels.hip b/sameold_amd/csrc/same_kernels.hip
--- a/sameold_amd/csrc/same_kernels.hip
+++ b/sameold_amd/csrc/same_kernels.hip
@@ -729,6 +729,33 @@
                        reinterpret_cast<const uint4 *>(fresh), n16, handover, sort_cnt, n_cols, counters);
     return hipGetLastError();
 }
+__global__ __launch_bounds__(256) void tp_prologue_slim_kernel(uint4 *__restrict__ hist, const uint4 *__restrict__ fresh_hist,
+                                                               const uint4 *__restrict__ own_hist, uint32_t hist_rows, uint32_t own_cols4,
+                                                               uint64_t *__restrict__ handover, uint32_t *__restrict__ sort_cnt,
+                                                               uint32_t n_cols, uint32_t *__restrict__ counters)
+{
+    const size_t t = (size_t)blockIdx.x * blockDim.x + threadIdx.x, stride = (size_t)gridDim.x * blockDim.x;
+    const uint32_t cols4 = n_cols / 4u;
+    const size_t n16 = (size_t)hist_rows * cols4;
+    for (size_t i = t; i < n16; i += stride) {
+        const uint32_t row = (uint32_t)(i / cols4), col4 = (uint32_t)(i - (size_t)row * cols4);
+        if (col4 >= own_cols4) hist[i] = fresh_hist[i];
+        else if (own_hist) hist[i] = own_hist[(size_t)row * own_cols4 + col4];
+    }
+    for (size_t i = t; i < n_cols; i += stride) { handover[i] = kNoHandover; if (sort_cnt) sort_cnt[i] = 0u; }
+    if (t < 3 && counters) counters[t] = 0u;
+}
+hipError_t launch_tp_prologue_slim(float *hist, const float *fresh_hist, const float *own_hist, uint32_t hist_rows, uint32_t own_cols,
+                                   uint64_t *handover, uint32_t *sort_cnt, uint32_t n_cols, uint32_t *counters, hipStream_t stream)
+{
+    if ((n_cols & 3u) != 0u || (own_cols & 3u) != 0u || own_cols > n_cols) return hipErrorInvalidValue;
+    const size_t n16 = (size_t)hist_rows * (n_cols / 4u);
+    const unsigned grid = (unsigned)std::min<size_t>((std::max<size_t>(n16, n_cols) + 255) / 256, 256 * 16);
+    hipLaunchKernelGGL(tp_prologue_slim_kernel, dim3(grid ? grid : 1u), dim3(256), 0, stream, reinterpret_cast<uint4 *>(hist),
+                       reinterpret_cast<const uint4 *>(fresh_hist), reinterpret_cast<const uint4 *>(own_hist), hist_rows, own_cols / 4u,
+                       handover, sort_cnt, n_cols, counters);
+    return hipGetLastError();
+}
 __global__ void cast_i16_f32_kernel(const int16_t *__restrict__ in, float *__restrict__ out, size_t n)
 {
     for (size_t i = (size_t)blockIdx.x * blockDim.x + threadIdx.x; i < n; i += (size_t)gridDim.x * blockDim.x) out[i] = (float)in[i];
diff --git a/sameold_amd/csrc/same_kernels_sym.hip b/sameold_amd/csrc/same_kernels_sym.hip
--- a/sameold_amd/csrc/same_kernels_sym.hip
+++ b/sameold_amd/csrc/same_kernels_sym.hip
@@ -881,7 +881,8 @@
     return fmaxf(floorf(s - 0.5f) + 1.0f, 1.0f);
 }
 
-struct SymKernArgs { Params P; State S; Output O; const float4 *taps; const void *x; uint32_t n_blocks; uint64_t counter0; PipeChunks K; };
+struct SymKernArgs { Params P; State S; Output O; const float4 *taps; const void *x; uint32_t n_blocks; uint64_t counter0; PipeChunks K;
+                     State own; State fresh; uint32_t self_start; uint32_t first_group; uint32_t n_groups; };
 typedef const __attribute__((address_space(4))) char *sym_kernarg_ptr;
 template <typename T> __device__ __forceinline__ T sym_fresh_arg(sym_kernarg_ptr ka, size_t off)
 {
@@ -896,9 +897,10 @@
 template <int NT, int NFF, int NFB, typename SampleT, int CMODE>
 __global__ __launch_bounds__(SymGeom<NT>::HALVES * kSymRoles * kWave, NT == 42 ? 3 : 2) void demod_sym_kernel(Params P, State S_arg_, Output O_arg_, const float4 *__restrict__ taps,
                                                                          const SampleT *__restrict__ x, uint32_t n_blocks, uint64_t counter0,
-                                                                         PipeChunks K)
+                                                                         PipeChunks K, State own_arg_, State fresh_arg_, uint32_t self_start,
+                                                                         uint32_t first_group, uint32_t n_groups)
 {
-    (void)S_arg_; (void)O_arg_;
+    (void)S_arg_; (void)O_arg_; (void)own_arg_; (void)fresh_arg_;
     const sym_kernarg_ptr ka = (sym_kernarg_ptr)__builtin_amdgcn_kernarg_segment_ptr();
     auto fresh_state = [&]() __attribute__((always_inline)) -> State { return sym_fresh_arg<State>(ka, offsetof(SymKernArgs, S)); };
     auto fresh_output = [&]() __attribute__((always_inline)) -> Output { return sym_fresh_arg<Output>(ka, offsetof(SymKernArgs, O)); };
@@ -925,11 +927,13 @@
     const uint32_t half = LY::HALVES == 2 ? hr >> 3 : 0u;
     const uint32_t role = hr & 7u;
     const uint32_t C = P.n_channels;
-    const uint32_t vwg = blockIdx.x * kSymHalves + half;
-    if (vwg * kWave >= C) return;
+    const uint32_t wg_group = blockIdx.x * kSymHalves + half;
+    const uint32_t vwg = first_group + wg_group;
+    if (wg_group >= n_groups || vwg * kWave >= C) return;
     float *lds = lds_all + half * (uint32_t)(LY::lds_bytes / sizeof(float));
     const uint32_t c = (K.n_chunks > 1u && K.col_perm) ? K.col_perm[vwg * kWave + lane] : vwg * kWave + lane;
     uint32_t cin = c, Cin = C, n_nominal = n_blocks;
+    uint32_t piece = 0;
     bool may_leave = false;
     int32_t row_l = 0;
     const SampleT *xl = nullptr;
@@ -939,7 +943,8 @@
         if (K.col_row0) {
             const uint32_t chunk_l = c / Cin;
             cin = c - chunk_l * Cin;
-            may_leave = (uint32_t)__builtin_amdgcn_readfirstlane((int)chunk_l) + 1u < K.n_chunks;
+            piece = (uint32_t)__builtin_amdgcn_readfirstlane((int)chunk_l);
+            may_leave = piece + 1u < K.n_chunks;
             const uint32_t row_abs = K.col_row0[c];
             xl = x + (size_t)cin * K.in_samples + row_abs;
             avail_l = (K.whole_samples - row_abs) / (uint32_t)kSB;
@@ -960,6 +965,11 @@
             n_nominal = may_leave ? K.nominal_blocks : n_blocks;
         }
     }
+    const bool self = CMODE == 1 && self_start != 0u && K.n_chunks > 1u;
+    const bool own_piece = self && piece == 0u;
+    const size_t start_off = !self ? offsetof(SymKernArgs, S) : (own_piece ? offsetof(SymKernArgs, own) : offsetof(SymKernArgs, fresh));
+    const uint32_t cl = own_piece ? cin : c, Cl = own_piece ? Cin : C;
+    auto start_state = [&]() __attribute__((always_inline)) -> State { return sym_fresh_arg<State>(ka, start_off); };
     lds_u32 *mail = (lds_u32 *)(lds + LY::tap_floats);
     lds_u32 *symbox = mail;
     lds_u32 *ybox = symbox + 2u * LY::sym_words;
@@ -1030,7 +1040,7 @@
     if (role == 0u) {
         sym_setprio<sym_prio<NT>(0)>(P);
         SymAgc<NT> M;
-        { const State S = fresh_state(); M.load(P, S, c, C, counter0, wcol); }
+        { const State S = start_state(); M.load(P, S, cl, Cl, counter0, wcol); }
         lds_barrier();
         P3_T0();
         uint32_t stop_at = 0xffffffffu;
@@ -1075,7 +1085,7 @@
             static_assert(CMODE == 0 && kNSUB == 2, "time-major rows, two sub-blocks a step");
             SymDcRot<SampleT, NT> D;
             const uint32_t n_sub = n_blocks * (uint32_t)kNSUB;
-            { const State S = fresh_state(); D.load(S, x, c, C, cin, Cin, counter0, n_sub); }
+            { const State S = start_state(); D.load(S, x, cl, Cl, cin, Cin, counter0, n_sub); }
             donebox[lane] = 0u;
             D.template sub<0>(P, wcol, x, 0u, n_sub, cin, Cin);
             D.template sub<1>(P, wcol, x, 1u, n_sub, cin, Cin);
@@ -1118,7 +1128,7 @@
         Dc D;
         D.xl = xl; D.avail = avail_l;
         const uint32_t n_sub = n_blocks * (uint32_t)kNSUB;
-        { const State S = fresh_state(); D.load(S, x, c, C, cin, Cin, counter0, n_sub); }
+        { const State S = start_state(); D.load(S, x, cl, Cl, cin, Cin, counter0, n_sub); }
         donebox[lane] = 0u;
         auto sub_tm = [&](uint32_t q, auto pb_) __attribute__((always_inline)) {
             typename Dc::Pairs X;
@@ -1192,9 +1202,19 @@
         X.pending_slot = 0xffffffffu;
         X.tk = tkbox + lane;
         {
-            const State S = fresh_state();
-            lane_load(L, S, c);
-            X.ring_load(P, S, c);
+            const State S = start_state();
+            lane_load(L, S, cl);
+            X.ring_load(P, S, Cl, cl);
+            if (self) {
+                const State W = fresh_state();
+                W.wake_sample[c] = L.wake_sample;
+                if (!P.ticks) {
+                    const TickRingGlobal G;
+#pragma unroll
+                    for (uint32_t i = 0; i < (uint32_t)kTickRing; ++i) G.tk_set(W, C, c, i, G.tk_at(S, Cl, cl, i));
+                    G.tk_set_count(W, c, G.tk_count(S, cl));
+                }
+            }
         }
         const State Snone{};
         Output O{};
@@ -1271,7 +1291,7 @@
         std::conditional_t<NT == 42, SymTaps<42>, SymHalfTaps<NT, NT / 4, NT / 2>> TP;
         TP.load(taps);
         Lane L;
-        { const State S = fresh_state(); lane_load(L, S, c); }
+        { const State S = start_state(); lane_load(L, S, cl); }
         const float inv_spt = 1.0f / P.samples_per_ted;
         int cstar = next_fire_count(L.until_next_ted, L.ted_clock);
         int rel = cstar - (int)L.ted_clock - 1;
@@ -1429,26 +1449,27 @@
         uint64_t symbols0;
         const bool hist_copy = K.n_chunks > 1u && K.col_perm != nullptr && K.hist_scratch != nullptr;
         {
-            const State S = fresh_state();
-            lane_load(Q.L, S, c);
+            const State S = start_state(), W = fresh_state();
+            const bool hist_in = hist_copy || (own_piece && (self_start & 2u) != 0u);
+            lane_load(Q.L, S, cl);
             symbols0 = Q.L.sq_symbols;
             Q.nsym = (uint32_t)symbols0;
-            Q.hbase = reinterpret_cast<char *>(hist_copy ? K.hist_scratch : S.sq_hist);
+            Q.hbase = reinterpret_cast<char *>(hist_copy ? K.hist_scratch : W.sq_hist);
             Q.hcol4 = (hist_copy ? vwg * kWave + lane : c) * 4u;
             Q.hrow4 = C * 4u;
-            if (hist_copy) {
+            if (hist_in) {
 #pragma unroll 4
-                for (int i = 0; i < kSquelchHist; ++i) *Q.hptr((uint32_t)i) = S.sq_hist[(size_t)i * C + c];
+                for (int i = 0; i < kSquelchHist; ++i) *Q.hptr((uint32_t)i) = S.sq_hist[(size_t)i * Cl + cl];
             }
 #pragma unroll
             for (int i = 0; i < NFF; ++i) {
-                Q.ffc[i] = S.eq_ffc[i * C + c]; Q.ffw[i] = S.eq_ffw[i * C + c];
-                Q.sffc[i] = S.eq_snap_ffc[i * C + c]; Q.sffw[i] = S.eq_snap_ffw[i * C + c];
+                Q.ffc[i] = S.eq_ffc[i * Cl + cl]; Q.ffw[i] = S.eq_ffw[i * Cl + cl];
+                Q.sffc[i] = S.eq_snap_ffc[i * Cl + cl]; Q.sffw[i] = S.eq_snap_ffw[i * Cl + cl];
             }
 #pragma unroll
             for (int i = 0; i < NFB; ++i) {
-                Q.fbc[i] = S.eq_fbc[i * C + c]; Q.fbw[i] = S.eq_fbw[i * C + c];
-                Q.sfbc[i] = S.eq_snap_fbc[i * C + c]; Q.sfbw[i] = S.eq_snap_fbw[i * C + c];
+                Q.fbc[i] = S.eq_fbc[i * Cl + cl]; Q.fbw[i] = S.eq_fbw[i * Cl + cl];
+                Q.sfbc[i] = S.eq_snap_fbc[i * Cl + cl]; Q.sfbw[i] = S.eq_snap_fbw[i * Cl + cl];
             }
             const uint32_t pslot = (2u * Q.nsym) & 63u;
             Q.nxt0 = *Q.hptr((pslot + 16u) & 63u); Q.nxt1 = *Q.hptr((pslot + 17u) & 63u);
@@ -1560,10 +1581,12 @@
         Lane L;
         SymFramer F;
         uint8_t *fr_rows;
-        { const State S0 = fresh_state(); lane_load(L, S0, c); fr_rows = S0.fr_msg; }
+        const uint8_t *start_rows;
+        { const State S0 = start_state(); lane_load(L, S0, cl); start_rows = S0.fr_msg; fr_rows = fresh_state().fr_msg; }
         F.st = fr_state(L); F.last = (L.flags & F_LINK_MASK) >> F_LINK_SHIFT;
         F.word = L.fr_word; F.count = L.fr_count; F.invalid = L.fr_invalid; F.len = L.fr_len;
         uint8_t *const row = fr_rows + (size_t)c * kBurstCap;
+        if (self && L.fr_len != 0u) copy_burst_row(row, start_rows + (size_t)cl * kBurstCap);
         Output O{};
         { const Output Of = fresh_output(); O.n_events = Of.n_events; O.bursts = Of.bursts; O.burst_cap = Of.burst_cap; }
         lds_barrier();
@@ -1658,7 +1681,7 @@
 
 template <int NT, int NFF, int NFB, typename SampleT>
 static hipError_t launch_sym_one(const Params &P, const State &S, const Output &O, const float4 *taps, const SampleT *x,
-                                 uint32_t n_blocks, uint64_t counter0, hipStream_t stream, const PipeChunks &K)
+                                 uint32_t n_blocks, uint64_t counter0, hipStream_t stream, const PipeChunks &K, const SymStart *start = nullptr)
 {
     constexpr uint32_t kSymHalves = (uint32_t)SymLayout<NT>::HALVES;
     constexpr size_t lds = (size_t)kSymHalves * SymLayout<NT>::lds_bytes;
@@ -1666,6 +1689,7 @@
     const bool cm = K.n_chunks > 1u && K.col_row0 != nullptr;
     if (cm && (!std::is_same<SampleT, float>::value || NT != 42)) return hipErrorInvalidValue;
     if (K.n_chunks > 1u && (K.in_channels % kWave) != 0u) return hipErrorInvalidValue;
+    if (start && (!cm || K.col_perm != nullptr)) return hipErrorInvalidValue;
     if (n_blocks == 0u) return hipSuccess;
     auto go = [&](auto kernel) -> hipError_t {
         if (lds > 64u * 1024u) {
@@ -1681,7 +1705,11 @@
                 opted_in.insert(key);
             }
         }
-        hipLaunchKernelGGL(kernel, dim3((P.n_channels / kWave + kSymHalves - 1u) / kSymHalves), dim3(kSymHalves * kSymRoles * kWave), lds, stream, P, S, O, taps, x, n_blocks, counter0, K);
+        const uint32_t all = P.n_channels / kWave;
+        const uint32_t g0 = start && start->n_groups ? start->first_group : 0u, ng = start && start->n_groups ? start->n_groups : all;
+        if (g0 > all || ng > all - g0) return hipErrorInvalidValue;
+        hipLaunchKernelGGL(kernel, dim3((ng + kSymHalves - 1u) / kSymHalves), dim3(kSymHalves * kSymRoles * kWave), lds, stream, P, S, O, taps, x, n_blocks, counter0, K,
+                           start ? start->own : S, start ? start->fresh : S, start ? (1u | (start->copy_hist ? 2u : 0u)) : 0u, g0, ng);
         return hipGetLastError();
     };
     if constexpr (std::is_same<SampleT, float>::value && NT == 42) {
@@ -1722,20 +1750,21 @@
 #endif
 template <typename SampleT>
 static hipError_t launch_sym_t(const Params &P, const State &S, const Output &O, const float4 *taps, const SampleT *x,
-                               uint32_t n_blocks, uint64_t counter0, hipStream_t stream, const PipeChunks &K)
+                               uint32_t n_blocks, uint64_t counter0, hipStream_t stream, const PipeChunks &K, const SymStart *start)
 {
     if (!sym_kernel_supported(P)) return hipErrorInvalidValue;
     const bool eq = P.eq_nff == 6u && P.eq_nfb == 4u;
     if (standard_rate_taps(P) == 42u)
-        return eq ? launch_sym_one<42, 6, 4, SampleT>(P, S, O, taps, x, n_blocks, counter0, stream, K) : launch_sym_one<42, 1, 1, SampleT>(P, S, O, taps, x, n_blocks, counter0, stream, K);
+        return eq ? launch_sym_one<42, 6, 4, SampleT>(P, S, O, taps, x, n_blocks, counter0, stream, K, start) : launch_sym_one<42, 1, 1, SampleT>(P, S, O, taps, x, n_blocks, counter0, stream, K, start);
+    if (start) return hipErrorInvalidValue;
     return launch_demod_sym_hi(P, S, O, taps, x, n_blocks, counter0, stream, K);
 }
 hipError_t launch_demod_sym(const Params &P, const State &S, const Output &O, const float4 *taps, const float *x,
-                            uint32_t n_blocks, uint64_t counter0, hipStream_t stream, const PipeChunks &K)
-{ return launch_sym_t<float>(P, S, O, taps, x, n_blocks, counter0, stream, K); }
+                            uint32_t n_blocks, uint64_t counter0, hipStream_t stream, const PipeChunks &K, const SymStart *start)
+{ return launch_sym_t<float>(P, S, O, taps, x, n_blocks, counter0, stream, K, start); }
 hipError_t launch_demod_sym(const Params &P, const State &S, const Output &O, const float4 *taps, const int16_t *x,
                             uint32_t n_blocks, uint64_t counter0, hipStream_t stream, const PipeChunks &K)
-{ return launch_sym_t<int16_t>(P, S, O, taps, x, n_blocks, counter0, stream, K); }
+{ return launch_sym_t<int16_t>(P, S, O, taps, x, n_blocks, counter0, stream, K, nullptr); }
 #endif
 
 }
diff --git a/sameold_amd/csrc/same_launch.h b/sameold_amd/csrc/same_launch.h
--- a/sameold_amd/csrc/same_launch.h
+++ b/sameold_amd/csrc/same_launch.h
@@ -24,7 +24,7 @@
                              const PipeChunks &chunks = PipeChunks{}, bool relaxed = false);
 hipError_t launch_demod_sym(const Params &P, const State &S, const Output &O, const float4 *taps,
                             const float *x, uint32_t n_blocks, uint64_t counter0, hipStream_t stream,
-                            const PipeChunks &chunks = PipeChunks{});
+                            const PipeChunks &chunks = PipeChunks{}, const SymStart *start = nullptr);
 hipError_t launch_demod_sym(const Params &P, const State &S, const Output &O, const float4 *taps,
                             const int16_t *x, uint32_t n_blocks, uint64_t counter0, hipStream_t stream,
                             const PipeChunks &chunks = PipeChunks{});
@@ -54,6 +54,8 @@
 hipError_t launch_cast_i16_f32(const int16_t *in, float *out, size_t n, hipStream_t stream);
 hipError_t launch_tp_prologue(void *blob, const void *fresh, size_t bytes, uint64_t *handover, uint32_t *sort_cnt, uint32_t n_cols,
                               uint32_t *counters, hipStream_t stream);
+hipError_t launch_tp_prologue_slim(float *hist, const float *fresh_hist, const float *own_hist, uint32_t hist_rows, uint32_t own_cols,
+                                   uint64_t *handover, uint32_t *sort_cnt, uint32_t n_cols, uint32_t *counters, hipStream_t stream);
 struct TpPlan {
     uint32_t channels, n_chunks, block_len, warmup_samples, whole_samples;
     uint64_t in_samples;
diff --git a/sameold_amd/csrc/same_pipe_common.h b/sameold_amd/csrc/same_pipe_common.h
--- a/sameold_amd/csrc/same_pipe_common.h
+++ b/sameold_amd/csrc/same_pipe_common.h
@@ -75,14 +75,15 @@
     {
         tk[2u * i * kWave] = (uint32_t)v; tk[(2u * i + 1u) * kWave] = (uint32_t)(v >> 32);
     }
-    __device__ __forceinline__ void ring_load(const Params &P, const State &S, uint32_t c)
+    __device__ __forceinline__ void ring_load(const Params &P, const State &S, uint32_t C, uint32_t c)
     {
         if (!P.ticks) return;
         const TickRingGlobal G;
 #pragma unroll
-        for (uint32_t i = 0; i < (uint32_t)kTickRing; ++i) tk_set(S, P.n_channels, c, i, G.tk_at(S, P.n_channels, c, i));
+        for (uint32_t i = 0; i < (uint32_t)kTickRing; ++i) tk_set(S, C, c, i, G.tk_at(S, C, c, i));
         tk_set_count(S, c, G.tk_count(S, c));
     }
+    __device__ __forceinline__ void ring_load(const Params &P, const State &S, uint32_t c) { ring_load(P, S, P.n_channels, c); }
     __device__ __forceinline__ void ring_store(const Params &P, const State &S, uint32_t c) const
     {
         if (!P.ticks) return;
diff --git a/sameold_amd/csrc/same_tp_plan.h b/sameold_amd/csrc/same_tp_plan.h
--- a/sameold_amd/csrc/same_tp_plan.h
+++ b/sameold_amd/csrc/same_tp_plan.h
@@ -24,6 +24,7 @@
     int sort_mode = -1;
     int knob_plan_stream = 0;
     int knob_prologue = 0;
+    int overlap = 2;
 };
 
 struct TpCut {
@@ -55,6 +56,23 @@
 };
 TpNative tp_native_plan(const Params &P, const TpConfig &cfg, const TpCut &cut, size_t n_call, uintptr_t base);
 inline bool tp_plan_beside(const TpConfig &cfg, bool own_stream) { return own_stream && cfg.knob_plan_stream >= 0; }
+inline bool tp_self_start(const TpConfig &cfg, const TpNative *np, Family family, bool own_stream, uint32_t channels)
+{
+    if (!np || !np->qualifies || family != Family::kSym || !own_stream) return false;
+    if (np->sort_mode != 0 || np->lpt || np->pair_groups || np->need_hist) return false;
+    if (channels == 0u || channels % 64u != 0u) return false;
+    return cfg.overlap >= 1 && cfg.knob_plan_stream >= 0 && cfg.knob_prologue >= 0;
+}
+inline bool tp_overlap(const TpConfig &cfg, bool self_start) { return self_start && cfg.overlap >= 2; }
+struct TpGroups { uint32_t first = 0, count = 0; };
+inline TpGroups tp_groups(uint32_t channels, uint32_t n_chunks, bool fresh)
+{
+    const uint32_t per_piece = channels / 64u;
+    TpGroups g;
+    g.first = fresh ? per_piece : 0u;
+    g.count = fresh ? (n_chunks > 1u ? (n_chunks - 1u) * per_piece : 0u) : per_piece;
+    return g;
+}
 
 constexpr size_t kSpanBytes = 32;
 struct OutputCaps {
```

New measurement: 448,700. 4.3% lower.
